# ramanakumars/patchGAN

Hardware: AMD Instinct MI355X
Metric: train images/sec (G+D step) at 256x256 bs=16 per GPU (higher is better)
Workload: dtype f32 (fp32 tensors and accumulation; polyphase Winograd GEMMs in bf16x3 split form: six bf16 MFMA products per fp32 product); 1 GPU; cfg2: 256x256x3->1 masks, bs 16/GPU, UNet nf=64 leakyrelu/sigmoid + PatchGAN ndf=64 n_layers=3, focal-Tversky*200 + BCE, Adam 1e-3, dropout off; global_batch=16, parallelism=dp1

## Files before the change

### include/patchgan_hip.h

```cpp
#ifndef PATCHGAN_HIP_H
#define PATCHGAN_HIP_H

#include <stddef.h>
#include <stdint.h>

#ifdef __cplusplus
extern "C" {
#endif

#define PG_OK 0
#define PG_EINVAL (-1)
#define PG_EWORKSPACE (-2)
#define PG_ELAUNCH (-3)

#define PG_ACT_NONE 0
#define PG_ACT_LEAKY 1
#define PG_ACT_RELU 2
#define PG_ACT_TANH 3
#define PG_ACT_SIGMOID 4

#define PG_ALGO_AUTO 0
#define PG_ALGO_DIRECT 1
#define PG_ALGO_MFMA 2
#define PG_ALGO_BF16 3

#define PG_ALGO_MASK 0xF
#define PG_TUNE_WINO2_ALL 0x010
#define PG_TUNE_WINO2_OFF 0x020
#define PG_TUNE_WINO2W_ALL 0x040
#define PG_TUNE_WINO2W_OFF 0x080
#define PG_TUNE_WINO_OFF 0x100
#define PG_TUNE_WINOW_OFF 0x200
#define PG_TUNE_WINO1_F2 0x400
#define PG_TUNE_WINO1_F3 0x800
#define PG_TUNE_WINO_DMA 0x1000
#define PG_TUNE_BF16X_OFF 0x2000
#define PG_TUNE_BF16X_RING 0x4000
#define PG_TUNE_BF16X_FLAT 0x8000
#define PG_TUNE_S3_OFF 0x40000

#define PG_IO_BIG_BF16 0x10000
#define PG_IO_SMALL_BF16 0x20000
#define PG_IO_MASK 0x30000

typedef struct pg_conv_geom {
    int N;
    int Hb, Wb;
    int Hs, Ws;
    int Ca;
    int Cb;
    int stride;
} pg_conv_geom;

int pg_version(void);

size_t pg_conv_max_tensor_bytes(void);

size_t pg_conv_workspace_bytes(const pg_conv_geom* g, int op);

int pg_conv_describe(const pg_conv_geom* g, int op, size_t ws_bytes, int* tile_id, int* split, long* workgroups);

int pg_conv_kernel(const pg_conv_geom* g, int op, size_t ws_bytes, char* name, size_t name_len, int* split, double* mfma_flops);

int pg_conv_kernel_flops(const pg_conv_geom* g, int op, size_t ws_bytes, double* executed, double* useful);

int pg_conv_time_next(void* ev_start, void* ev_stop);

int pg_conv4x4_big2small(const float* big, int ld_big, const float* P, const float* bias,
                         float* small, int ld_small, const pg_conv_geom* g, int act, int algo,
                         void* ws, size_t ws_bytes, void* stream);

int pg_conv4x4_small2big(const float* small, int ld_small, const float* P, const float* bias,
                         float* big, int ld_big, const pg_conv_geom* g, int act, int algo,
                         void* ws, size_t ws_bytes, void* stream);

int pg_conv4x4_wgrad(const float* small, int ld_small, const float* big, int ld_big,
                     float* dP, float* dbias, const pg_conv_geom* g, int algo,
                     void* ws, size_t ws_bytes, void* stream);

typedef struct pg_conv_extras {
    double* part;
    float* v_keep;
    const float* v_pre;
    float* u_cache;
    int u_valid;
    const void* mul_t;
    int mul_ld;
    int mul_act;
    long long v_stride;
    long long v_tile0;
} pg_conv_extras;
int pg_conv_batch_halves_same(const pg_conv_geom* g, int algo, size_t ws_bytes_n, size_t ws_bytes_2n);
int pg_conv_mul_ok(const pg_conv_geom* g, int algo, size_t ws_bytes);
int pg_conv_stats_chunks(const pg_conv_geom* g, int op, int algo, size_t ws_bytes);
size_t pg_conv_u_bytes(const pg_conv_geom* g, int op, int algo, size_t ws_bytes);
size_t pg_conv_v_bytes(const pg_conv_geom* g, int algo, size_t ws_bytes);
int pg_conv4x4_big2small_x(const float* big, int ld_big, const float* P, const float* bias, float* small, int ld_small,
                           const pg_conv_geom* g, int act, int algo, void* ws, size_t ws_bytes, void* stream,
                           const pg_conv_extras* x);
int pg_conv4x4_small2big_x(const float* small, int ld_small, const float* P, const float* bias, float* big, int ld_big,
                           const pg_conv_geom* g, int act, int algo, void* ws, size_t ws_bytes, void* stream,
                           const pg_conv_extras* x);
int pg_conv4x4_wgrad_x(const float* small, int ld_small, const float* big, int ld_big, float* dP, float* dbias,
                       const pg_conv_geom* g, int algo, void* ws, size_t ws_bytes, void* stream, const pg_conv_extras* x);
typedef struct pg_conv_prep_item {
    pg_conv_geom g;
    int op;
    int algo;
    size_t ws_bytes;
    const float* P;
    void* u;
} pg_conv_prep_item;
int pg_conv_prep_batch(int n, const pg_conv_prep_item* items, void* stream);
int pg_instnorm_act_fwd_parts(const float* y, int ld_y, float* out, int ld_out, float* stats, const double* part, int chunks,
                              int N, int HW, int C, int act, float eps, float drop_p, uint64_t seed, void* stream);

int pg_instnorm_act_fwd_t(const void* y, int ld_y, void* out, int ld_out, float* stats, int N, int HW, int C, int act, float eps,
                          float drop_p, uint64_t seed, void* ws, size_t ws_bytes, void* stream, int dt);
int pg_instnorm_act_fwd_parts_t(const void* y, int ld_y, void* out, int ld_out, float* stats, const double* part, int chunks,
                                int N, int HW, int C, int act, float eps, float drop_p, uint64_t seed, void* stream, int dt);
int pg_instnorm_act_bwd_t(const void* g1, int ld_g1, const void* g2, int ld_g2, const void* y, int ld_y, const float* stats,
                          void* dy, int ld_dy, int N, int HW, int C, int act, float drop_p, uint64_t seed, void* ws,
                          size_t ws_bytes, void* stream, int dt);
size_t pg_instnorm_affine_workspace_bytes(int N, int HW, int C);
int pg_instnorm_affine_act_fwd_t(const void* y, int ld_y, void* out, int ld_out, const float* gamma, const float* beta, float* stats,
                                 int N, int HW, int C, int act, float eps, float drop_p, uint64_t seed, void* ws, size_t ws_bytes,
                                 void* stream, int dt);
int pg_instnorm_affine_act_fwd_parts_t(const void* y, int ld_y, void* out, int ld_out, const float* gamma, const float* beta,
                                       float* stats, const double* part, int chunks, int N, int HW, int C, int act, float eps,
                                       float drop_p, uint64_t seed, void* stream, int dt);
int pg_instnorm_affine_act_bwd_t(const void* g1, int ld_g1, const void* g2, int ld_g2, const void* y, int ld_y, const float* gamma,
                                 const float* beta, const float* stats, void* dy, int ld_dy, float* dgamma, float* dbeta, int N,
                                 int HW, int C, int act, float drop_p, uint64_t seed, void* ws, size_t ws_bytes, void* stream,
                                 int dt);
int pg_act_fwd_t(const void* y, int ld_y, void* out, int ld_out, long npix, int C, int act, float drop_p, uint64_t seed,
                 void* stream, int dt);
int pg_act_bwd_t(const void* g1, int ld_g1, const void* g2, int ld_g2, const void* a, int ld_a, void* dy, int ld_dy, long npix,
                 int C, int act, float drop_p, uint64_t seed, void* stream, int dt);

int pg_conv4x4_bwd_big(const float* small, int ld_small, const float* big, int ld_big, const float* P, float* dP,
                       float* dsmall, int ld_dsmall, const pg_conv_geom* g, int algo, void* ws, size_t ws_bytes, void* stream);
int pg_conv4x4_bwd_big_x(const float* small, int ld_small, const float* big, int ld_big, const float* P, float* dP,
                         float* dsmall, int ld_dsmall, const pg_conv_geom* g, int algo, void* ws, size_t ws_bytes, void* stream,
                         const pg_conv_extras* x);

int pg_conv_time_next2(void* ev_start, void* ev_stop, void* ev_start2, void* ev_stop2);

int pg_instnorm_act_fwd(const float* y, int ld_y, float* out, int ld_out, float* stats,
                        int N, int HW, int C, int act, float eps,
                        float drop_p, uint64_t seed, void* ws, size_t ws_bytes, void* stream);

size_t pg_instnorm_workspace_bytes(int N, int HW, int C);

int pg_instnorm_act_bwd(const float* g1, int ld_g1, const float* g2, int ld_g2,
                        const float* y, int ld_y, const float* stats, float* dy, int ld_dy,
                        int N, int HW, int C, int act, float drop_p, uint64_t seed,
                        void* ws, size_t ws_bytes, void* stream);

int pg_act_bwd(const float* g1, int ld_g1, const float* g2, int ld_g2, const float* a, int ld_a,
               float* dy, int ld_dy, long npix, int C, int act, float drop_p, uint64_t seed, void* stream);

int pg_act_fwd(const float* y, int ld_y, float* out, int ld_out, long npix, int C, int act,
               float drop_p, uint64_t seed, void* stream);

int pg_softmax_fwd(const float* y, int ld_y, float* out, int ld_out, long npix, int C, void* stream);
int pg_softmax_bwd(const float* g1, int ld_g1, const float* g2, int ld_g2, const float* out, int ld_out,
                   float* dy, int ld_dy, long npix, int C, void* stream);

int pg_dropout_mask(float* mask, long nelem, float drop_p, uint64_t seed, void* stream);

size_t pg_batchnorm_workspace_bytes(int N, int HW, int C, int nseg);
int pg_batchnorm_act_fwd(const float* y, int ld_y, float* out, int ld_out, const float* weight, const float* bias, float* coef,
                         double* bstat, int N, int HW, int C, int nseg, int act, float eps, float drop_p, uint64_t seed, void* ws,
                         size_t ws_bytes, void* stream);
int pg_batchnorm_stats(const float* y, int ld_y, const double* part, int chunks, const float* weight, const float* bias, float* coef,
                       double* bstat, int N, int HW, int C, int nseg, float eps, void* ws, size_t ws_bytes, void* stream);
int pg_batchnorm_act_apply(const float* y, int ld_y, float* out, int ld_out, const float* coef, int N, int HW, int C, int nseg,
                           int act, float drop_p, uint64_t seed, void* stream);
int pg_batchnorm_eval_coef(const float* running_mean, const float* running_var, const float* weight, const float* bias, int C,
                           float eps, float* coef, void* stream);
int pg_batchnorm_act_bwd(const float* g1, int ld_g1, const float* g2, int ld_g2, const float* y, int ld_y, const float* coef,
                         float* dy, int ld_dy, float* dweight, float* dbias, int N, int HW, int C, int nseg, int train, int act,
                         float drop_p, uint64_t seed, void* ws, size_t ws_bytes, void* stream);
int pg_batchnorm_moments_fwd(const float* y, int ld_y, const double* part, int chunks, double* mom, int N, int HW, int C, int nseg,
                             void* ws, size_t ws_bytes, void* stream);
int pg_batchnorm_coef_from_moments(const double* mom, double count, const float* weight, const float* bias, float eps, float* coef,
                                   double* bstat, int C, int nseg, void* stream);
// ... 165 lines not shown
```

### patchgan_amd/_lib.py

```python
import ctypes
import os

_HERE = os.path.dirname(os.path.abspath(__file__))
LIB_PATH = os.environ.get('PATCHGAN_LIB') or os.path.join(_HERE, 'libpatchgan_hip.so')

ACT_NONE, ACT_LEAKY, ACT_RELU, ACT_TANH, ACT_SIGMOID = 0, 1, 2, 3, 4
ACT_CODES = {None: ACT_NONE, 'none': ACT_NONE, 'leakyrelu': ACT_LEAKY, 'relu': ACT_RELU, 'tanh': ACT_TANH,
             'sigmoid': ACT_SIGMOID}
ALGO_AUTO, ALGO_DIRECT, ALGO_MFMA, ALGO_BF16 = 0, 1, 2, 3
ALGO_MASK = 0xF
IO_BIG_BF16, IO_SMALL_BF16, IO_MASK = 0x10000, 0x20000, 0x30000
TUNE_WINO2_ALL, TUNE_WINO2_OFF, TUNE_WINO2W_ALL, TUNE_WINO2W_OFF = 0x010, 0x020, 0x040, 0x080
TUNE_WINO_OFF, TUNE_WINOW_OFF, TUNE_WINO1_F2, TUNE_WINO1_F3, TUNE_WINO_DMA = 0x100, 0x200, 0x400, 0x800, 0x1000
TUNE_BF16X_OFF, TUNE_BF16X_RING, TUNE_BF16X_FLAT = 0x2000, 0x4000, 0x8000
TUNE_S3_OFF = 0x40000
LOSS_TVERSKY, LOSS_WBCE, LOSS_MAE, LOSS_BCE = 0, 1, 2, 3
OP_BIG2SMALL, OP_SMALL2BIG, OP_WGRAD = 0, 1, 2
AUG_FLIP, AUG_TRANSLATION, AUG_CUTOUT = 1, 2, 4
ACC_BEGIN, ACC_ADD, ACC_CLOSE, ACC_CLOSE_ONLY = 0, 1, 2, 3
GAN_LSGAN, GAN_HINGE_D, GAN_HINGE_G, GAN_BCE_LOGITS = 0, 1, 2, 3
SEG_CE, SEG_FOCAL, SEG_DICE = 1, 2, 4
SEG_FOCAL_GAMMA_MAX, SEG_FOCAL_ALPHA_NONE = 8, -1.0

_ERR = {-1: 'PG_EINVAL (bad shape / null or misaligned pointer)', -2: 'PG_EWORKSPACE (workspace too small)',
        -3: 'PG_ELAUNCH (HIP launch failed)'}


class ConvGeom(ctypes.Structure):
    _fields_ = [('N', ctypes.c_int), ('Hb', ctypes.c_int), ('Wb', ctypes.c_int), ('Hs', ctypes.c_int),
                ('Ws', ctypes.c_int), ('Ca', ctypes.c_int), ('Cb', ctypes.c_int), ('stride', ctypes.c_int)]

    def key(self):
        return (self.N, self.Hb, self.Wb, self.Hs, self.Ws, self.Ca, self.Cb, self.stride)


_p = ctypes.c_void_p
_i = ctypes.c_int
_l = ctypes.c_long
_f = ctypes.c_float
_d = ctypes.c_double
_sz = ctypes.c_size_t
_u64 = ctypes.c_uint64
_G = ctypes.POINTER(ConvGeom)


class ConvExtras(ctypes.Structure):
    _fields_ = [('part', ctypes.c_void_p), ('v_keep', ctypes.c_void_p), ('v_pre', ctypes.c_void_p), ('u_cache', ctypes.c_void_p),
                ('u_valid', ctypes.c_int), ('mul_t', ctypes.c_void_p), ('mul_ld', ctypes.c_int), ('mul_act', ctypes.c_int),
                ('v_stride', ctypes.c_longlong), ('v_tile0', ctypes.c_longlong)]


_X = ctypes.POINTER(ConvExtras)


class BnUpdateItem(ctypes.Structure):
    _fields_ = [('bstat', ctypes.c_void_p), ('running_mean', ctypes.c_void_p), ('running_var', ctypes.c_void_p),
                ('num_batches_tracked', ctypes.c_void_p), ('C', ctypes.c_int)]


BN_MAX_LAYERS = 16


class ConvPrepItem(ctypes.Structure):
    _fields_ = [('g', ConvGeom), ('op', ctypes.c_int), ('algo', ctypes.c_int), ('ws_bytes', ctypes.c_size_t), ('P', ctypes.c_void_p),
                ('u', ctypes.c_void_p)]


class SpectralItem(ctypes.Structure):
    _fields_ = [('W', ctypes.c_void_p), ('w_hat', ctypes.c_void_p), ('u', ctypes.c_void_p), ('v', ctypes.c_void_p),
                ('sigma', ctypes.c_void_p), ('g_off', ctypes.c_long), ('Cout', ctypes.c_int), ('Cin', ctypes.c_int),
                ('iterate', ctypes.c_int)]


SN_MAX_LAYERS = 16


class GanTerm(ctypes.Structure):
    _fields_ = [('d', ctypes.c_void_p), ('g', ctypes.c_void_p), ('value', ctypes.c_void_p), ('scale', ctypes.c_double),
                ('n', ctypes.c_long), ('ld', ctypes.c_int), ('ld_g', ctypes.c_int), ('kind', ctypes.c_int), ('target', ctypes.c_float)]


GAN_MAX_TERMS = 4


SIGNATURES = {
    'pg_version': (_i, []),
    'pg_conv_max_tensor_bytes': (_sz, []),
    'pg_conv_workspace_bytes': (_sz, [_G, _i]),
    'pg_conv_describe': (_i, [_G, _i, _sz, ctypes.POINTER(_i), ctypes.POINTER(_i), ctypes.POINTER(_l)]),
    'pg_conv_mul_ok': (_i, [_G, _i, _sz]),
    'pg_conv_kernel': (_i, [_G, _i, _sz, ctypes.c_char_p, _sz, ctypes.POINTER(_i), ctypes.POINTER(ctypes.c_double)]),
    'pg_conv_kernel_flops': (_i, [_G, _i, _sz, ctypes.POINTER(ctypes.c_double), ctypes.POINTER(ctypes.c_double)]),
    'pg_conv_time_next': (_i, [_p, _p]),
    'pg_conv_time_next2': (_i, [_p, _p, _p, _p]),
    'pg_conv4x4_bwd_big': (_i, [_p, _i, _p, _i, _p, _p, _p, _i, _G, _i, _p, _sz, _p]),
    'pg_conv4x4_bwd_big_x': (_i, [_p, _i, _p, _i, _p, _p, _p, _i, _G, _i, _p, _sz, _p, _X]),
    'pg_conv4x4_big2small': (_i, [_p, _i, _p, _p, _p, _i, _G, _i, _i, _p, _sz, _p]),
    'pg_conv4x4_small2big': (_i, [_p, _i, _p, _p, _p, _i, _G, _i, _i, _p, _sz, _p]),
    'pg_conv4x4_wgrad': (_i, [_p, _i, _p, _i, _p, _p, _G, _i, _p, _sz, _p]),
    'pg_conv_stats_chunks': (_i, [_G, _i, _i, _sz]),
    'pg_conv_u_bytes': (_sz, [_G, _i, _i, _sz]),
    'pg_conv_v_bytes': (_sz, [_G, _i, _sz]),
    'pg_conv_batch_halves_same': (_i, [_G, _i, _sz, _sz]),
    'pg_conv4x4_big2small_x': (_i, [_p, _i, _p, _p, _p, _i, _G, _i, _i, _p, _sz, _p, _X]),
    'pg_conv4x4_small2big_x': (_i, [_p, _i, _p, _p, _p, _i, _G, _i, _i, _p, _sz, _p, _X]),
    'pg_conv4x4_wgrad_x': (_i, [_p, _i, _p, _i, _p, _p, _G, _i, _p, _sz, _p, _X]),
    'pg_conv_prep_batch': (_i, [_i, ctypes.POINTER(ConvPrepItem), _p]),
    'pg_instnorm_act_fwd_parts': (_i, [_p, _i, _p, _i, _p, _p, _i, _i, _i, _i, _i, _f, _f, _u64, _p]),
    'pg_instnorm_workspace_bytes': (_sz, [_i, _i, _i]),
    'pg_instnorm_act_fwd': (_i, [_p, _i, _p, _i, _p, _i, _i, _i, _i, _f, _f, _u64, _p, _sz, _p]),
    'pg_instnorm_act_bwd': (_i, [_p, _i, _p, _i, _p, _i, _p, _p, _i, _i, _i, _i, _i, _f, _u64, _p, _sz, _p]),
    'pg_act_bwd': (_i, [_p, _i, _p, _i, _p, _i, _p, _i, _l, _i, _i, _f, _u64, _p]),
    'pg_act_fwd': (_i, [_p, _i, _p, _i, _l, _i, _i, _f, _u64, _p]),
    'pg_instnorm_act_fwd_t': (_i, [_p, _i, _p, _i, _p, _i, _i, _i, _i, _f, _f, _u64, _p, _sz, _p, _i]),
    'pg_instnorm_act_fwd_parts_t': (_i, [_p, _i, _p, _i, _p, _p, _i, _i, _i, _i, _i, _f, _f, _u64, _p, _i]),
    'pg_instnorm_act_bwd_t': (_i, [_p, _i, _p, _i, _p, _i, _p, _p, _i, _i, _i, _i, _i, _f, _u64, _p, _sz, _p, _i]),
    'pg_instnorm_affine_workspace_bytes': (_sz, [_i, _i, _i]),
    'pg_instnorm_affine_act_fwd_t': (_i, [_p, _i, _p, _i, _p, _p, _p, _i, _i, _i, _i, _f, _f, _u64, _p, _sz, _p, _i]),
    'pg_instnorm_affine_act_fwd_parts_t': (_i, [_p, _i, _p, _i, _p, _p, _p, _p, _i, _i, _i, _i, _i, _f, _f, _u64, _p, _i]),
    'pg_instnorm_affine_act_bwd_t': (_i, [_p, _i, _p, _i, _p, _i, _p, _p, _p, _p, _i, _p, _p, _i, _i, _i, _i, _f, _u64, _p, _sz, _p,
                                          _i]),
    'pg_act_fwd_t': (_i, [_p, _i, _p, _i, _l, _i, _i, _f, _u64, _p, _i]),
    'pg_act_bwd_t': (_i, [_p, _i, _p, _i, _p, _i, _p, _i, _l, _i, _i, _f, _u64, _p, _i]),
    'pg_softmax_fwd': (_i, [_p, _i, _p, _i, _l, _i, _p]),
    'pg_softmax_bwd': (_i, [_p, _i, _p, _i, _p, _i, _p, _i, _l, _i, _p]),
    'pg_dropout_mask': (_i, [_p, _l, _f, _u64, _p]),
    'pg_batchnorm_workspace_bytes': (_sz, [_i, _i, _i, _i]),
    'pg_batchnorm_act_fwd': (_i, [_p, _i, _p, _i, _p, _p, _p, _p, _i, _i, _i, _i, _i, _f, _f, _u64, _p, _sz, _p]),
    'pg_batchnorm_stats': (_i, [_p, _i, _p, _i, _p, _p, _p, _p, _i, _i, _i, _i, _f, _p, _sz, _p]),
    'pg_batchnorm_act_apply': (_i, [_p, _i, _p, _i, _p, _i, _i, _i, _i, _i, _f, _u64, _p]),
    'pg_batchnorm_eval_coef': (_i, [_p, _p, _p, _p, _i, _f, _p, _p]),
    'pg_batchnorm_act_bwd': (_i, [_p, _i, _p, _i, _p, _i, _p, _p, _i, _p, _p, _i, _i, _i, _i, _i, _i, _f, _u64, _p, _sz, _p]),
    'pg_batchnorm_moments_fwd': (_i, [_p, _i, _p, _i, _p, _i, _i, _i, _i, _p, _sz, _p]),
    'pg_batchnorm_coef_from_moments': (_i, [_p, _d, _p, _p, _f, _p, _p, _i, _i, _p]),
    'pg_batchnorm_moments_bwd': (_i, [_p, _i, _p, _i, _p, _i, _p, _p, _p, _p, _i, _i, _i, _i, _i, _f, _u64, _p, _sz, _p]),
    'pg_batchnorm_bwd_apply': (_i, [_p, _i, _p, _i, _p, _i, _p, _p, _d, _p, _i, _i, _i, _i, _i, _i, _f, _u64, _p, _sz, _p]),
    'pg_batchnorm_update_running': (_i, [_i, ctypes.POINTER(BnUpdateItem), _i, _f, _p]),
    'pg_loss_reduce_doubles': (_l, [_i, _i, _i]),
    'pg_loss_fused_max_nc': (_i, []),
    'pg_loss_reduce': (_i, [_p, _i, _p, _i, _f, _i, _i, _i, _p, _p]),
    'pg_loss_prepare': (_i, [_p, _i, _i, _f, _p, _p]),
    'pg_loss_finalize': (_i, [_p, _p, _i, _i, _i, _i, _i, _f, _f, _f, _p, _p, _p]),
    'pg_loss_grad': (_i, [_p, _i, _p, _i, _f, _p, _p, _i, _i, _i, _i, _i, _p]),
    'pg_loss_reduce_parts': (_i, [_p, _i, _p, _i, _f, _i, _i, _i, _p, _p]),
    'pg_loss_value_grad': (_i, [_p, _i, _p, _p, _i, _i, _i, _i, _i, _f, _f, _f, _p, _i, _p, _i, _f, _p, _i, _p, _p]),
    'pg_seg_confusion_max_c': (_i, []),
    'pg_seg_confusion': (_i, [_p, _i, _p, _i, _i, _i, _i, _f, _p, _p]),
    'pg_seg_hist_max_words': (_i, []),
    'pg_seg_hist': (_i, [_p, _i, _p, _i, _i, _i, _i, _i, _p, _p]),
    'pg_adam_step': (_i, [_p, _p, _p, _p, _l, _f, _f, _f, _f, _f, _f, _p]),
    'pg_adam_step_dev': (_i, [_p, _p, _p, _p, _l, _f, _f, _f, _p, _p]),
    'pg_adam_ema_step': (_i, [_p, _p, _p, _p, _p, _l, _f, _f, _f, _f, _f, _f, _f, _p]),
    'pg_adam_ema_step_dev': (_i, [_p, _p, _p, _p, _p, _l, _f, _f, _f, _p, _f, _p]),
    'pg_grad_norm_workspace_bytes': (_l, [_l]),
    'pg_grad_norm': (_i, [_p, _l, _d, _p, _l, _p, _p]),
    'pg_adam_clip_step': (_i, [_p, _p, _p, _p, _p, _l, _f, _f, _f, _f, _f, _f, _f, _p, _p]),
    'pg_adam_clip_step_dev': (_i, [_p, _p, _p, _p, _p, _l, _f, _f, _f, _p, _f, _p, _p]),
    'pg_adamw_step': (_i, [_p, _p, _p, _p, _p, _l, _f, _f, _f, _f, _f, _f, _f, _f, _p, _p]),
    'pg_adamw_step_dev': (_i, [_p, _p, _p, _p, _p, _l, _f, _f, _f, _p, _f, _p, _p]),
    'pg_grad_accum': (_i, [_p, _p, _l, _i, _f, _p]),
    'pg_spectral_workspace_bytes': (_l, [_i, ctypes.POINTER(SpectralItem)]),
    'pg_spectral_fwd': (_i, [_i, ctypes.POINTER(SpectralItem), _p, _p, _l, _p, _l, _p]),
    'pg_spectral_bwd': (_i, [_i, ctypes.POINTER(SpectralItem), _p, _l, _p, _l, _p]),
    'pg_nchw_to_nhwc': (_i, [_p, _p, _i, _i, _i, _i, _i, _p]),
    'pg_nhwc_to_nchw': (_i, [_p, _i, _p, _i, _i, _i, _i, _p]),
    'pg_copy_channels': (_i, [_p, _i, _p, _i, _l, _i, _p]),
    'pg_fill': (_i, [_p, _l, _f, _p]),
    'pg_pad8_bf16': (_i, [_p, _i, _p, _l, _i, _p]),
    'pg_din_fill': (_i, [_p, _p, _p, _p, _i, _i, _i, _i, _i, _i, _p]),
    'pg_u8_to_f32': (_i, [_p, _p, _i, _l, _i, _f, _p]),
    'pg_labels_to_onehot': (_i, [_p, _p, _i, _l, _p, _i, _i, _p]),
    'pg_tiles_count': (_i, [_i, _i, _i]),
    'pg_tiles_gather': (_i, [_p, _i, _i, _i, _i, _i, _p, _i, _p]),
    'pg_tiles_blend': (_i, [_p, _i, _i, _i, _i, _i, _i, ctypes.c_double, _p, _p, _p]),
    'pg_tiles_tta_max': (_i, []),
    'pg_tiles_gather_tta': (_i, [_p, _i, _i, _i, _i, _i, _i, _p, _i, _p]),
    'pg_tiles_blend_win': (_i, [_p, _i, _i, _i, _i, _i, _i, _i, _p, ctypes.c_double, _p, _p, _p]),
    'pg_diffaug_params': (_i, [_u64, _p, _u64, _i, _l, _i, _i, _i, _p, _p]),
    'pg_diffaug_fwd': (_i, [_p, _i, _p, _i, _p, _i, _i, _i, _i, _p]),
    'pg_diffaug_bwd': (_i, [_p, _i, _p, _i, _p, _i, _i, _i, _i, _p]),
    'pg_gan_loss_max_terms': (_i, []),
    'pg_gan_loss_single_max': (_l, []),
    'pg_gan_loss_workspace_bytes': (_l, [_i, ctypes.POINTER(GanTerm)]),
    'pg_gan_loss': (_i, [_i, ctypes.POINTER(GanTerm), _p, _l, _p]),
    'pg_seg_loss_workspace_bytes': (_l, [_i, _i, _i]),
    'pg_seg_loss_slabs': (_i, [_i, _i]),
    'pg_seg_loss_reduce': (_i, [_p, _i, _p, _i, _i, _i, _i, _i, _i, _f, _p, _l, _p]),
    'pg_seg_loss_value_grad': (_i, [_p, _l, _p, _i, _p, _i, _i, _i, _i, _i, _i, _f, _f, _d, _d, _d, _p, _i, _p, _p]),
    'pg_seg_loss_value_grad_w': (_i, [_p, _l, _p, _i, _p, _i, _i, _i, _i, _i, _i, _f, _f, _d, _d, _d, _p, _p, _i, _p, _p]),
    'pg_seg_label_count': (_i, [_p, _i, _i, _i, _i, _p, _p]),
# ... 39 lines not shown
```

### patchgan_amd/csrc/conv_gemm.hip

```cpp
#include <hip/hip_runtime.h>
#include <stdio.h>
#include <stdint.h>
#include <stdlib.h>
#include <string.h>
#include <type_traits>
#include <vector>
#include "patchgan_hip.h"
#include "pg_common.h"
#include "conv_wino.h"
#include "conv_bf16.h"

namespace {

typedef float f32x4 __attribute__((ext_vector_type(4)));
typedef float f32x16 __attribute__((ext_vector_type(16)));

struct Geom {
    int N, Hb, Wb, Hs, Ws, Ca, Cb, s;
};

constexpr int KC = 32;
constexpr int LDK = KC + 4;

__device__ __forceinline__ f32x4 ld4(const float* p, bool ok) {
// ... 4234 lines not shown
                    hipLaunchKernelGGL((k_wgrad_tapn<PG_TILE(T), 2>), grid, dim3(256), 0, st, big, ld_big, small, ld_small, dst, q.out_elems, g, q.cps, q.tiles_n,
                                       p.vecn, 0);
            });
        }
    }
    if (hipGetLastError() != hipSuccess) return PG_ELAUNCH;
    return q.split == 1 ? PG_OK : reduce(dst, q.split);
}

int refusal(int rc, int op, const Views& v, const pg_conv_geom* gg, int algo_full, size_t ws_bytes) {
    if (rc != PG_EINVAL || !(algo_full & PG_IO_MASK)) return rc;
    const size_t full = pg_conv_workspace_bytes(gg, op);
    if (v.ws && ws_bytes >= full) return rc;
    Views w = v;
    if (!w.ws) w.ws = reinterpret_cast<void*>(uintptr_t(256));
    return plan_conv(gg, op, algo_full, tune_of(algo_full), full, &w).rc == PG_OK ? PG_EWORKSPACE : rc;
}

int run_conv(int op, const Views& v, const pg_conv_geom* gg, int algo_full, size_t ws_bytes, void* stream) {
    if (!v.ws) ws_bytes = 0;
    Call c{ConvPlan{}, v, to_geom(gg), algo_full & PG_ALGO_MASK, algo_full & PG_IO_MASK, tune_of(algo_full), ws_bytes, (hipStream_t)stream};
    c.p = plan_conv(gg, op, algo_full, c.tune, ws_bytes, &c.v);
    if (c.p.rc != PG_OK) return refusal(c.p.rc, op, v, gg, algo_full, ws_bytes);
    return op == 0 ? launch_b2s(c) : op == 1 ? launch_s2b(c) : launch_wgrad(c);
}

}

static bool hand_overs_sized(const pg_conv_geom* gg, int op, int algo, const void* ws, size_t ws_bytes, const pg_conv_extras& x) {
    const size_t wb = ws ? ws_bytes : 0;
    if (x.part && (op > 1 || pg_conv_stats_chunks(gg, op, algo, wb) == 0)) return false;
    if (x.u_cache && (op > 1 || pg_conv_u_bytes(gg, op, algo, wb) == 0)) return false;
    if ((x.v_keep || x.v_pre) && pg_conv_v_bytes(gg, algo, wb) == 0) return false;
    return true;
}

extern "C" {

int pg_conv4x4_big2small_x(const float* big, int ld_big, const float* P, const float* bias, float* small, int ld_small,
                           const pg_conv_geom* gg, int act, int algo, void* ws, size_t ws_bytes, void* stream, const pg_conv_extras* xp) {
    const pg_conv_extras& x = xp ? *xp : NO_EXTRAS;
    if ((x.u_cache && !aligned16(x.u_cache)) || (x.v_keep && !aligned16(x.v_keep)) || x.v_pre) return PG_EINVAL;
    if (!geom_ok(gg) || !big || !P || !small || ld_big < gg->Cb || ld_small < gg->Ca) return PG_EINVAL;
    if (act < PG_ACT_NONE || act > PG_ACT_SIGMOID) return PG_EINVAL;
    if ((algo & PG_IO_MASK) && (algo & PG_ALGO_MASK) != PG_ALGO_BF16) return PG_EINVAL;
    if (!hand_overs_sized(gg, 0, algo, ws, ws_bytes, x)) return PG_EINVAL;
    if (x.v_stride || x.v_tile0) {
        ConvPlan f;
        if (!x.v_keep || x.v_stride < 0 || x.v_tile0 < 0 || !query_plan(gg, 0, algo, ws ? ws_bytes : 0, OFFER_V, &f)) return PG_EINVAL;
        if (f.path != Path::Wino1 && f.path != Path::Wino2) return PG_EINVAL;
        const bool w1 = f.path == Path::Wino1;
        const long X = w1 ? 36 : 16, K = w1 ? gg->Cb : 4L * gg->Cb;
        const long T = w1 ? (long)gg->N * ((gg->Hs + 2) / 3) * ((gg->Ws + 2) / 3) : pg_wino2_tiles_b2s(gg->N, gg->Hs, gg->Ws);
        const long zs = x.v_stride ? (long)x.v_stride : T * K;
        if ((zs & 3) || (x.v_tile0 + T) * K > zs || (double)X * zs * 4 >= 1.5e9) return PG_EINVAL;
    }
    return run_conv(0, Views{small, big, ld_small, ld_big, P, bias, act, ws, &x}, gg, algo, ws_bytes, stream);
}

int pg_conv4x4_big2small(const float* big, int ld_big, const float* P, const float* bias, float* small,
                         int ld_small, const pg_conv_geom* gg, int act, int algo, void* ws, size_t ws_bytes,
                         void* stream) {
    return pg_conv4x4_big2small_x(big, ld_big, P, bias, small, ld_small, gg, act, algo, ws, ws_bytes, stream, nullptr);
}

int pg_conv4x4_small2big_x(const float* small, int ld_small, const float* P, const float* bias, float* big, int ld_big,
                           const pg_conv_geom* gg, int act, int algo, void* ws, size_t ws_bytes, void* stream, const pg_conv_extras* xp) {
    const pg_conv_extras& x = xp ? *xp : NO_EXTRAS;
    if ((x.u_cache && !aligned16(x.u_cache)) || x.v_keep || x.v_pre || x.v_stride || x.v_tile0) return PG_EINVAL;
    if (x.mul_t && (x.mul_ld < gg->Cb || x.mul_act < PG_ACT_NONE || x.mul_act > PG_ACT_SIGMOID || x.part)) return PG_EINVAL;
    if (!geom_ok(gg) || !big || !P || !small || ld_big < gg->Cb || ld_small < gg->Ca) return PG_EINVAL;
    if (act < PG_ACT_NONE || act > PG_ACT_SIGMOID) return PG_EINVAL;
    if ((algo & PG_IO_MASK) && (algo & PG_ALGO_MASK) != PG_ALGO_BF16) return PG_EINVAL;
    if (!hand_overs_sized(gg, 1, algo, ws, ws_bytes, x)) return PG_EINVAL;
    return run_conv(1, Views{small, big, ld_small, ld_big, P, bias, act, ws, &x}, gg, algo, ws_bytes, stream);
}

int pg_conv4x4_small2big(const float* small, int ld_small, const float* P, const float* bias, float* big,
                         int ld_big, const pg_conv_geom* gg, int act, int algo, void* ws, size_t ws_bytes,
                         void* stream) {
    return pg_conv4x4_small2big_x(small, ld_small, P, bias, big, ld_big, gg, act, algo, ws, ws_bytes, stream, nullptr);
}

static int wgrad_impl(const float* small, int ld_small, const float* big, int ld_big, float* dP, float* dbias,
                      const pg_conv_geom* gg, int algo, void* ws, size_t ws_bytes, void* stream, const float* v_pre) {
    if (!geom_ok(gg) || !big || !dP || !small || ld_big < gg->Cb || ld_small < gg->Ca) return PG_EINVAL;
    if (v_pre && !aligned16(v_pre)) return PG_EINVAL;
    hipStream_t st = (hipStream_t)stream;
    const Geom g = to_geom(gg);
    const int io = algo & PG_IO_MASK;
    if (io && ((algo & PG_ALGO_MASK) != PG_ALGO_BF16 || io != PG_IO_MASK)) return PG_EINVAL;
    if (io && dbias && !((g.Ca % 4 == 0) && (ld_small % 4 == 0) && aligned_io(small, true))) return PG_EINVAL;
    if (!ws) ws_bytes = 0;
    pg_conv_extras x = NO_EXTRAS;
    x.v_pre = v_pre;
    if (!hand_overs_sized(gg, 2, algo, ws, ws_bytes, x)) return PG_EINVAL;
    if (dbias) {
        if (ws_bytes < colsum_bytes(g.Ca)) return PG_EWORKSPACE;
        const Views vw{small, big, ld_small, ld_big, dP, dbias, PG_ACT_NONE, ws, &x};
        const int prc = plan_conv(gg, 2, algo, tune_of(algo), ws_bytes, &vw).rc;
        if (prc != PG_OK) return refusal(prc, 2, vw, gg, algo, ws_bytes);
        const long Kp = (long)g.N * g.Hs * g.Ws;
        float* part = (float*)ws;
        int chunks = (int)std::min<long>(COLSUM_CHUNKS, Kp);
        long rpc = (Kp + chunks - 1) / chunks;
        chunks = (int)((Kp + rpc - 1) / rpc);
        if (io)
            hipLaunchKernelGGL(k_colsum_partial4<true>, dim3(chunks, (g.Ca + 63) / 64), dim3(256), 0, st, small, ld_small, Kp, g.Ca,
                               rpc, part);
        else if ((g.Ca % 4 == 0) && (ld_small % 4 == 0) && aligned16(small) && aligned16(part))
            hipLaunchKernelGGL(k_colsum_partial4<false>, dim3(chunks, (g.Ca + 63) / 64), dim3(256), 0, st, small, ld_small, Kp, g.Ca,
                               rpc, part);
        else
            hipLaunchKernelGGL(k_colsum_partial, dim3(chunks, (g.Ca + 63) / 64), dim3(256), 0, st, small, ld_small, Kp, g.Ca,
                               rpc, part);
        if (hipGetLastError() != hipSuccess) return PG_ELAUNCH;
        int rc = launch_reduce(part, g.Ca, chunks, dbias, g.Ca, 1, g.Ca, nullptr, 0, st);
        if (rc != PG_OK) return rc;
    }
    return run_conv(2, Views{small, big, ld_small, ld_big, dP, dbias, PG_ACT_NONE, ws, &x}, gg, algo, ws_bytes, stream);
}

int pg_conv4x4_wgrad(const float* small, int ld_small, const float* big, int ld_big, float* dP, float* dbias,
                     const pg_conv_geom* gg, int algo, void* ws, size_t ws_bytes, void* stream) {
    return wgrad_impl(small, ld_small, big, ld_big, dP, dbias, gg, algo, ws, ws_bytes, stream, nullptr);
}

int pg_conv4x4_wgrad_x(const float* small, int ld_small, const float* big, int ld_big, float* dP, float* dbias,
                       const pg_conv_geom* gg, int algo, void* ws, size_t ws_bytes, void* stream, const pg_conv_extras* x) {
    if (x && (x->part || x->v_keep || x->u_cache || x->v_stride || x->v_tile0)) return PG_EINVAL;
    return wgrad_impl(small, ld_small, big, ld_big, dP, dbias, gg, algo, ws, ws_bytes, stream, x ? x->v_pre : nullptr);
}

int pg_conv4x4_bwd_big(const float* small, int ld_small, const float* big, int ld_big, const float* P, float* dP,
                       float* dsmall, int ld_dsmall, const pg_conv_geom* gg, int algo, void* ws, size_t ws_bytes, void* stream) {
    return pg_conv4x4_bwd_big_x(small, ld_small, big, ld_big, P, dP, dsmall, ld_dsmall, gg, algo, ws, ws_bytes, stream, nullptr);
}

int pg_conv4x4_bwd_big_x(const float* small, int ld_small, const float* big, int ld_big, const float* P, float* dP,
                         float* dsmall, int ld_dsmall, const pg_conv_geom* gg, int algo, void* ws, size_t ws_bytes, void* stream,
                         const pg_conv_extras* x) {
    if (!geom_ok(gg) || !small || !big || !P || !dP || !dsmall) return PG_EINVAL;
    if (x && (x->part || x->v_keep || x->v_pre || x->mul_t || x->v_stride || x->v_tile0)) return PG_EINVAL;
    float* const Uext = x ? x->u_cache : nullptr;
    const int u_valid = x ? x->u_valid : 0;
    if (Uext && !aligned16(Uext)) return PG_EINVAL;
    if (ld_small < gg->Ca || ld_big < gg->Cb || ld_dsmall < gg->Ca) return PG_EINVAL;
    if (Uext && pg_conv_u_bytes(gg, 0, algo, ws ? ws_bytes : 0) == 0) return PG_EINVAL;
    hipStream_t st = (hipStream_t)stream;
    const Geom g = to_geom(gg);
    const Tune tune = tune_of(algo);
    if (!ws) ws_bytes = 0;
    const bool views_ok = (ld_small % 4 == 0) && (ld_big % 4 == 0) && (ld_dsmall % 4 == 0) && aligned16(small) && aligned16(big) &&
                          aligned16(P) && aligned16(dP) && aligned16(dsmall) && aligned16(ws);
    hipEvent_t e0 = t_ev0, e1 = t_ev1, e2 = t_ev2, e3 = t_ev3;
    if (!plan_share_v(g, algo, tune, ws_bytes, views_ok, nullptr)) {
        t_ev2 = t_ev3 = nullptr;
        int rc = pg_conv4x4_wgrad(small, ld_small, big, ld_big, dP, nullptr, gg, algo, ws, ws_bytes, stream);
        if (rc != PG_OK) return rc;
        t_ev0 = e2;
        t_ev1 = e3;
        if (Uext) {
            pg_conv_extras xu{};
            xu.u_cache = Uext;
            xu.u_valid = u_valid;
            return pg_conv4x4_big2small_x(big, ld_big, P, nullptr, dsmall, ld_dsmall, gg, PG_ACT_NONE, algo, ws, ws_bytes, stream, &xu);
        }
        return pg_conv4x4_big2small(big, ld_big, P, nullptr, dsmall, ld_dsmall, gg, PG_ACT_NONE, algo, ws, ws_bytes, stream);
    }
    t_ev0 = t_ev1 = t_ev2 = t_ev3 = nullptr;
    float* V = (float*)ws;
    void* rest = (char*)ws + pg_wino2_v_bytes(g.N, g.Hs, g.Ws, g.Cb);
    int rc = pg_wino2_v(big, ld_big, V, g.N, g.Hb, g.Wb, g.Hs, g.Ws, g.Cb, st);
    if (rc != PG_OK) return rc;
    rc = pg_wino2_wgrad(small, ld_small, big, ld_big, dP, g.N, g.Hb, g.Wb, g.Hs, g.Ws, g.Ca, g.Cb, rest, st, e0, e1, V, tune.s3w);
    if (rc != PG_OK) return rc;
    return pg_wino2_b2s(big, ld_big, P, nullptr, dsmall, ld_dsmall, g.N, g.Hb, g.Wb, g.Hs, g.Ws, g.Ca, g.Cb, PG_ACT_NONE, rest, st, e2,
                        e3, V, nullptr, nullptr, Uext, u_valid, tune.s3);
}

}
```

### patchgan_amd/csrc/conv_wino.h

```cpp
#pragma once
#include <hip/hip_runtime.h>
#include <stddef.h>
#include "pg_common.h"


bool pg_wino_eligible(int N, int Hin, int Win, int Cin, int Hout, int Wout, int Cout, int ld_in, const void* in, int mo_forced);
bool pg_wino_geom_ok(int N, int Hout, int Wout, int Cin, int Cout, int mo_forced);
int pg_wino_mo(int N, int Hout, int Wout, int Cin, int Cout, int mo_forced);
bool pg_wino_small_tile(int N, int Hout, int Wout, int Cin, int Cout, int mo_forced);
size_t pg_wino_ws_bytes(int N, int Hout, int Wout, int Cin, int Cout, int mo_forced);
int pg_wino_prepare(const float* in, int ld_in, const float* P, int flip, int N, int Hin, int Win, int Cin, int Hout,
                    int Wout, int Cout, int pad, void* ws, hipStream_t st, int mo_forced, float* Uext, int u_valid, float* Vext = nullptr,
                    long v_stride = 0, long v_tile0 = 0);
size_t pg_wino_u_bytes(int N, int Hout, int Wout, int Cin, int Cout, int mo_forced);
size_t pg_wino2_u_bytes(int Ca, int Cb);
#define PG_WINO_PREP_MAX 24
struct pg_wino_prep {
    const float* P;
    float* U;
    int Ca, Cb, kind, mo, flip;
};
int pg_wino_prep_batch(int n, const pg_wino_prep* items, hipStream_t st);
int pg_wino_gemm_slices(int N, int Hout, int Wout, int Cin, int Cout, int mo_forced);
bool pg_wino_gemm_rows(int N, int Hout, int Wout, int Cin, int Cout, int mo_forced, int dma_mode, const float* out, int ld_out,
                       const float* bias, pg_epi_mul mul);
bool pg_wino_row_on();
float* pg_wino_gemm_slabs(void* ws, int N, int Hout, int Wout, int Cin, int Cout, int mo_forced);
int pg_wino_dma_mode();
int pg_wino_gemm(const float* bias, float* out, int ld_out, int N, int Cin, int Hout, int Wout, int Cout, int act,
                 void* ws, hipStream_t st, int mo_forced, int dma_mode, const float* Uext, pg_epi_mul mul = pg_epi_mul{nullptr, 0, 0},
                 const float* Vext = nullptr, int s3 = 0, long v_stride = 0, long v_tile0 = 0);

bool pg_wino_wgrad_geom_ok(int N, int Hs, int Ws, int Ca, int Cb);
int pg_wino_wgrad_r(int N, int Hs, int Ws);
double pg_wino_wgrad_flops(int N, int Hs, int Ws, int Ca, int Cb);
int pg_wino_wgrad_slices(int N, int Hs, int Ws, int Ca, int Cb, int s3);
bool pg_wino_wgrad_tile64(int Ca, int Cb, int s3);
size_t pg_wino_wgrad_ws_bytes(int N, int Hs, int Ws, int Ca, int Cb);
int pg_wino_wgrad(const float* small, int ld_small, const float* big, int ld_big, float* dP, int N, int Hb, int Wb, int Hs,
                  int Ws, int Ca, int Cb, void* ws, hipStream_t st, hipEvent_t ev0, hipEvent_t ev1, const float* Vpre = nullptr, int s3 = 0);
size_t pg_wino_wgrad_v_bytes(int N, int Hs, int Ws, int Ca, int Cb, int fwd_mo_forced);

int pg_wino2_mo();
long pg_wino2_tiles_b2s(int N, int Hs, int Ws);
long pg_wino2_tiles_s2b(int N, int Hb, int Wb);
int pg_wino2_b2s_zb(int N, int Hs, int Ws, int Ca);
int pg_wino2_s2b_zb(int N, int Hb, int Wb, int Cb);
bool pg_wino2_geom_ok(int N, int Hs, int Ws, int Ca, int Cb);
size_t pg_wino2_ws_bytes(int N, int Hs, int Ws, int Ca, int Cb);
int pg_wino2_b2s(const float* big, int ld_big, const float* P, const float* bias, float* small, int ld_small, int N, int Hb,
                 int Wb, int Hs, int Ws, int Ca, int Cb, int act, void* ws, hipStream_t st, hipEvent_t ev0, hipEvent_t ev1,
                 const float* Vpre, double* part, float* Vkeep, float* Uext, int u_valid, int s3, long v_stride = 0, long v_tile0 = 0);
int pg_wino2_b2s_stats_chunks(int N, int Hs, int Ws, int Ca);
int pg_wino2_s2b_stats_chunks(int N, int Hb, int Wb, int Cb);
size_t pg_wino2_v_bytes(int N, int Hs, int Ws, int Cb);
int pg_wino2_v(const float* big, int ld_big, float* V, int N, int Hb, int Wb, int Hs, int Ws, int Cb, hipStream_t st);

bool pg_wino2c_geom_ok(int N, int Hb, int Wb, int Ca, int Cb);
size_t pg_wino2c_ws_bytes(int N, int Hb, int Wb, int Ca, int Cb);
int pg_wino2_s2b(const float* small, int ld_small, const float* P, const float* bias, float* big, int ld_big, int N, int Hb,
                 int Wb, int Hs, int Ws, int Ca, int Cb, int act, void* ws, hipStream_t st, hipEvent_t ev0, hipEvent_t ev1,
                 double* part, float* Uext, int u_valid, pg_epi_mul mul, int s3);

bool pg_wino2_wgrad_geom_ok(int N, int Hs, int Ws, int Ca, int Cb);
int pg_wino2_wgrad_slices(int N, int Hs, int Ws, int Ca, int Cb, int s3);
bool pg_wino2_wgrad_tile64(int Ca, int Cb, int s3);
size_t pg_wino2_wgrad_ws_bytes(int N, int Hs, int Ws, int Ca, int Cb);
int pg_wino2_wgrad(const float* small, int ld_small, const float* big, int ld_big, float* dP, int N, int Hb, int Wb, int Hs,
                   int Ws, int Ca, int Cb, void* ws, hipStream_t st, hipEvent_t ev0, hipEvent_t ev1, const float* Vpre, int s3 = 0);
```

### patchgan_amd/csrc/conv_wino.hip

```cpp
#include <hip/hip_runtime.h>
#include <stdint.h>
#include <stdlib.h>
#include "patchgan_hip.h"
#include "pg_common.h"
#include "conv_wino.h"

namespace {

typedef float f32x4 __attribute__((ext_vector_type(4)));
typedef float f32x16 __attribute__((ext_vector_type(16)));
typedef unsigned int u32x4 __attribute__((ext_vector_type(4)));

constexpr int KC = 32;
constexpr int LDK = KC + 4;


__device__ __constant__ float c_BT[5][5] = {{2, -1, -2, 1, 0}, {0, -2, -1, 1, 0}, {0, 2, -3, 1, 0}, {0, -1, 0, 1, 0},
                                            {0, 2, -1, -2, 1}};
__device__ __constant__ float c_G[5][4] = {{0.5f, 0, 0, 0},
                                           {-0.5f, -0.5f, -0.5f, -0.5f},
                                           {-1.f / 6, 1.f / 6, -1.f / 6, 1.f / 6},
                                           {1.f / 6, 1.f / 3, 2.f / 3, 4.f / 3},
                                           {0, 0, 0, 1}};

// ... 1104 lines not shown
            for (int j = 0; j < NR; ++j)
#pragma unroll
                for (int p = 0; p < 3; ++p)
                    fb[j][p] = *reinterpret_cast<const s3_bf16x8*>(&buf[(BM + (wn * NR + j) * 32 + lrow) * S3_LDR + p * S3_KC + lh * 8]);
#pragma unroll
            for (int i = 0; i < MR; ++i)
#pragma unroll
                for (int p = 0; p < 3; ++p)
                    fa[i][p] = *reinterpret_cast<const s3_bf16x8*>(&buf[((wm * MR + i) * 32 + lrow) * S3_LDR + p * S3_KC + lh * 8]);
        };
        auto mm = [&](const s3_bf16x8 (&fa)[MR][3], const s3_bf16x8 (&fb)[NR][3]) {
#define S3_MM(pa, pb)                                                                       \
    _Pragma("unroll") for (int i = 0; i < MR; ++i) _Pragma("unroll") for (int j = 0; j < NR; ++j) \
        acc[i][j] = __builtin_amdgcn_mfma_f32_32x32x16_bf16(fa[i][pa], fb[j][pb], acc[i][j], 0, 0, 0)
            S3_MM(0, 0); S3_MM(0, 1); S3_MM(1, 0); S3_MM(1, 1); S3_MM(0, 2); S3_MM(2, 0);
#undef S3_MM
        };
        auto mix = [&]() {
            constexpr int NM = 6 * MR * NR, NRD = 3 * (MR + NR), NWR = 3 * (AI + BI), NLD = AI + BI;
#pragma unroll
            for (int t = 0; t < NM; ++t) {
                __builtin_amdgcn_sched_group_barrier(0x008, 1, 0);
                if (t < NLD) __builtin_amdgcn_sched_group_barrier(0x020, 1, 0);
                if (t < NRD) __builtin_amdgcn_sched_group_barrier(0x100, 1, 0);
                __builtin_amdgcn_sched_group_barrier(0x002, 4, 0);
                if (t >= NM - NWR) __builtin_amdgcn_sched_group_barrier(0x200, 1, 0);
            }
        };
        issue_loads(ra0, rb0, 0);
        issue_loads(ra1, rb1, 1);
        stage(ra0, rb0, buf0);
        issue_loads(ra0, rb0, 2);
        __syncthreads();
        rd(fa0, fb0, buf0);
        stage(ra1, rb1, buf1);
        issue_loads(ra1, rb1, 3);
        __syncthreads();
        for (int c = 0; c < nch; c += 2) {
            mm(fa0, fb0);
            rd(fa1, fb1, buf1);
            stage(ra0, rb0, buf0);
            issue_loads(ra0, rb0, c + 4);
            mix();
            __syncthreads();
            mm(fa1, fb1);
            rd(fa0, fb0, buf0);
            stage(ra1, rb1, buf1);
            issue_loads(ra1, rb1, c + 5);
            mix();
            __syncthreads();
        }
    } else {
    issue_loads(ra0, rb0, 0);
    issue_loads(ra1, rb1, 1);
    stage(ra0, rb0, buf0);
    issue_loads(ra0, rb0, 2);
    __syncthreads();
    for (int c = 0; c < nch; c += 2) {
        stage(ra1, rb1, buf1);
        compute(buf0);
        issue_loads(ra1, rb1, c + 3);
        __syncthreads();
        stage(ra0, rb0, buf0);
        compute(buf1);
        issue_loads(ra0, rb0, c + 4);
        __syncthreads();
    }
    }
    float* o = C + (long)z * Mrows * Ncols;
#pragma unroll
    for (int i = 0; i < MR; ++i)
#pragma unroll
        for (int j = 0; j < NR; ++j) {
            const int col = n0 + (wn * NR + j) * 32 + lrow;
#pragma unroll
            for (int r = 0; r < 16; ++r) {
                const int row = (r & 3) + 8 * (r >> 2) + 4 * lh;
                const int m = m0 + (wm * MR + i) * 32 + row;
                if (m < Mrows && col < Ncols) o[(long)m * Ncols + col] = acc[i][j][r];
            }
        }
}

template <int MR, int NR, int WM, int WN, int KS, int WPE>
__global__ __launch_bounds__(256) __attribute__((amdgpu_waves_per_eu(WPE, WPE))) void k_wino_wgrad_gemm_s3(const float* __restrict__ DY, const float* __restrict__ V,
                                                         float* __restrict__ S, int T, int Ca, int Cb, int chunks_per_slice,
                                                         int tilesA, int tilesB, int NX, int dy_bytes, int v_bytes) {
    constexpr int BM = WM * MR * 32, BN = WN * NR * 32, KCH = 16 * KS, ROW = KS * 48 + 8, BUF = (BM + BN) * ROW;
    static_assert((BM + BN) * KS == 256, "one 4 x 4 block per staging thread");
    __shared__ __attribute__((aligned(16))) __bf16 smem[2 * BUF];
    const int tid = threadIdx.x, lane = tid & 63, wave = tid >> 6;
    const int wm = wave / WN, wn = wave % WN;
    const int lrow = lane & 31, lh = lane >> 5;
    int w = pg_xcd_remap(blockIdx.x, gridDim.x);
    const int tile_b = w % tilesB;
    w /= tilesB;
    const int tile_a = w % tilesA;
    w /= tilesA;
    const int xi = w % NX, slice = w / NX;
    const int m0 = tile_a * BM, n0 = tile_b * BN;
    const int k_begin = slice * chunks_per_slice * KC, k_end = min(T, k_begin + chunks_per_slice * KC);
    const int nch = (max(k_end - k_begin, 0) + KCH - 1) / KCH;
    const bool is_a = __builtin_amdgcn_readfirstlane(tid >> 6) < BM * KS / 64;
    const int it = is_a ? tid : tid - BM * KS, BX = is_a ? BM : BN;
    const int kg = it & 3, mq = (it >> 2) % (BX / 4), ks = it / BX;
    const int ld = is_a ? Ca : Cb, c0 = (is_a ? m0 : n0) + mq * 4;
    const bool c_in = c0 < ld;
    const __amdgpu_buffer_rsrc_t rS = is_a ? __builtin_amdgcn_make_buffer_rsrc((void*)DY, 0, dy_bytes, 0x00020000)
                                           : __builtin_amdgcn_make_buffer_rsrc((void*)V, 0, v_bytes, 0x00020000);
    const int base = xi * T * ld + c0;
    const int krow = ks * 16 + kg * 4;
    const int wr_off = ((is_a ? 0 : BM) + mq * 4) * ROW + ks * 48 + kg * 4;
    auto issue_loads = [&](f32x4 (&r)[4], int c) {
#pragma unroll
        for (int j = 0; j < 4; ++j) {
            const int k = k_begin + c * KCH + krow + j;
            r[j] = bload4(rS, voff(base + k * ld, c < nch && c_in && k < k_end));
        }
    };
    auto stage = [&](const f32x4 (&r)[4], __bf16* buf) {
#pragma unroll
        for (int e = 0; e < 4; ++e) {
            const f32x4 v = {r[0][e], r[1][e], r[2][e], r[3][e]};
            s3_bf16x4 h, m, l;
            s3_split(v, h, m, l);
            __bf16* row = &buf[wr_off + e * ROW];
            *reinterpret_cast<s3_bf16x4*>(row) = h;
            *reinterpret_cast<s3_bf16x4*>(row + 16) = m;
            *reinterpret_cast<s3_bf16x4*>(row + 32) = l;
        }
    };
    f32x16 acc[MR][NR];
#pragma unroll
    for (int i = 0; i < MR; ++i)
#pragma unroll
        for (int j = 0; j < NR; ++j)
#pragma unroll
            for (int r = 0; r < 16; ++r) acc[i][j][r] = 0.f;
    auto compute = [&](const __bf16* buf) {
#pragma unroll
        for (int s = 0; s < KS; ++s) {
            s3_bf16x8 bf[NR][3], af[MR][3];
#pragma unroll
            for (int j = 0; j < NR; ++j)
#pragma unroll
                for (int p = 0; p < 3; ++p)
                    bf[j][p] = *reinterpret_cast<const s3_bf16x8*>(&buf[(BM + (wn * NR + j) * 32 + lrow) * ROW + s * 48 + p * 16 + lh * 8]);
#pragma unroll
            for (int i = 0; i < MR; ++i)
#pragma unroll
                for (int p = 0; p < 3; ++p)
                    af[i][p] = *reinterpret_cast<const s3_bf16x8*>(&buf[((wm * MR + i) * 32 + lrow) * ROW + s * 48 + p * 16 + lh * 8]);
#pragma unroll
            for (int i = 0; i < MR; ++i)
#pragma unroll
                for (int j = 0; j < NR; ++j) {
#define S3_MM(pa, pb) acc[i][j] = __builtin_amdgcn_mfma_f32_32x32x16_bf16(af[i][pa], bf[j][pb], acc[i][j], 0, 0, 0)
                    S3_MM(0, 0); S3_MM(0, 1); S3_MM(1, 0); S3_MM(1, 1); S3_MM(0, 2); S3_MM(2, 0);
#undef S3_MM
                }
        }
    };
    __bf16* const buf0 = smem;
    __bf16* const buf1 = smem + BUF;
    f32x4 r0[4], r1[4];
    issue_loads(r0, 0);
    issue_loads(r1, 1);
    stage(r0, buf0);
    issue_loads(r0, 2);
    __syncthreads();
    for (int c = 0; c < nch; c += 2) {
        stage(r1, buf1);
        compute(buf0);
        issue_loads(r1, c + 3);
        __syncthreads();
        stage(r0, buf0);
        compute(buf1);
        issue_loads(r0, c + 4);
        __syncthreads();
    }
    float* o = S + ((long)slice * NX + xi) * Ca * Cb;
#pragma unroll
    for (int i = 0; i < MR; ++i)
#pragma unroll
        for (int j = 0; j < NR; ++j) {
            const int col = n0 + (wn * NR + j) * 32 + lrow;
#pragma unroll
            for (int r = 0; r < 16; ++r) {
                const int row = (r & 3) + 8 * (r >> 2) + 4 * lh;
                const int a = m0 + (wm * MR + i) * 32 + row;
                if (a < Ca && col < Cb) o[(long)a * Cb + col] = acc[i][j][r];
            }
        }
}

template <int WPE>
__global__ __launch_bounds__(256) __attribute__((amdgpu_waves_per_eu(WPE, WPE))) void k_wino_gemm_row_s3(
    const float* __restrict__ V, const float* __restrict__ U, float* __restrict__ Tout, int T, int Ci, int Co, int v_bytes, int u_bytes,
    int tiles_n, int v_xi) {
    constexpr int NP = 6, BM = 128, BN = 64, MR = 2, BUF = (BM + BN) * S3_LDR;
    __shared__ __attribute__((aligned(16))) __bf16 smem[2 * BUF];
    const __amdgpu_buffer_rsrc_t rV = __builtin_amdgcn_make_buffer_rsrc((void*)V, 0, v_bytes, 0x00020000);
    const __amdgpu_buffer_rsrc_t rU = __builtin_amdgcn_make_buffer_rsrc((void*)U, 0, u_bytes, 0x00020000);
    const int tid = threadIdx.x, lane = tid & 63, wave = tid >> 6;
    const int wm = wave >> 1, wn = wave & 1;
    const int lrow = lane & 31, lh = lane >> 5;
    int w = pg_xcd_remap(blockIdx.x, gridDim.x);
    const int n0 = (w % tiles_n) * BN;
    w /= tiles_n;
    const int tiles_m = (T + BM - 1) / BM;
    const int xrow = w / tiles_m;
    const int m0 = (w % tiles_m) * BM;
    const int nch = Ci / S3_KC, total = NP * nch;
    const int kq = tid & 3, r0 = tid >> 2;
    int a_off[2], b_off;
    bool a_ok[2];
#pragma unroll
    for (int i = 0; i < 2; ++i) {
        const int m = m0 + r0 + 64 * i;
        a_ok[i] = m < T;
        a_off[i] = min(m, T - 1) * Ci + kq * 4;
    }
    {
        const int co = n0 + r0;
        b_off = (co < Co) ? co * Ci + kq * 4 : 0x10000000;
    }
    const int u_xi = Co * Ci;
    int ld_j = 0, ld_ch = 0;
    auto issue_loads = [&](f32x4 (&ra)[2], f32x4& rb) {
        const bool on = ld_j < NP;
        const int xi = xrow * NP + ld_j;
        const int av = xi * v_xi + ld_ch * S3_KC, bu = xi * u_xi + ld_ch * S3_KC;
#pragma unroll
        for (int i = 0; i < 2; ++i) ra[i] = bload4(rV, voff(a_off[i] + av, on && a_ok[i]));
        rb = bload4(rU, voff(b_off + bu, on));
        const bool wrap = ld_ch + 1 >= nch;
        ld_ch = wrap ? 0 : ld_ch + 1;
        ld_j = wrap ? ld_j + 1 : ld_j;
    };
    auto stage = [&](const f32x4 (&ra)[2], const f32x4& rb, __bf16* buf) {
#pragma unroll
        for (int i = 0; i < 2; ++i) {
            s3_bf16x4 h, m, l;
            s3_split(ra[i], h, m, l);
            __bf16* row = &buf[(r0 + 64 * i) * S3_LDR + kq * 4];
            *reinterpret_cast<s3_bf16x4*>(row) = h;
            *reinterpret_cast<s3_bf16x4*>(row + S3_KC) = m;
            *reinterpret_cast<s3_bf16x4*>(row + 2 * S3_KC) = l;
        }
        s3_bf16x4 h, m, l;
        s3_split(rb, h, m, l);
        __bf16* row = &buf[(BM + r0) * S3_LDR + kq * 4];
        *reinterpret_cast<s3_bf16x4*>(row) = h;
        *reinterpret_cast<s3_bf16x4*>(row + S3_KC) = m;
        *reinterpret_cast<s3_bf16x4*>(row + 2 * S3_KC) = l;
    };
    f32x16 accm[MR], acct[3][MR];
#pragma unroll
    for (int i = 0; i < MR; ++i)
#pragma unroll
        for (int r = 0; r < 16; ++r) {
            accm[i][r] = 0.f;
#pragma unroll
            for (int c = 0; c < 3; ++c) acct[c][i][r] = 0.f;
        }
    int j = 0, ch = 0;
    auto compute = [&](const __bf16* buf) {
        s3_bf16x8 bf[3], af[MR][3];
#pragma unroll
        for (int p = 0; p < 3; ++p) bf[p] = *reinterpret_cast<const s3_bf16x8*>(&buf[(BM + wn * 32 + lrow) * S3_LDR + p * S3_KC + lh * 8]);
#pragma unroll
        for (int i = 0; i < MR; ++i)
#pragma unroll
            for (int p = 0; p < 3; ++p)
                af[i][p] = *reinterpret_cast<const s3_bf16x8*>(&buf[((wm * MR + i) * 32 + lrow) * S3_LDR + p * S3_KC + lh * 8]);
#pragma unroll
// ... 664 lines not shown
                           TW, Hout, Wout, act, v_bytes, u_bytes, tn, mul, 1, 0L);
    } else if (small_tile && dma_mode == 2) {
        dim3 grid((unsigned)(((T + 63) / 64) * tn));
        hipLaunchKernelGGL((k_wino_gemm_dma<2, 3, 3>), grid, dim3(256), 0, st, V, U, bias, out, ld_out, (int)T, Cin, Cout, TH, TW,
                           Hout, Wout, act, v_bytes, u_bytes, tn);
    } else if (small_tile) {
        dim3 grid((unsigned)(((T + 63) / 64) * tn));
        hipLaunchKernelGGL((k_wino_gemm<1, 1, 2, 2, 4, 2>), grid, dim3(256), 0, st, V, U, bias, out, ld_out, (int)T, Cin, Cout, TH,
                           TW, Hout, Wout, act, v_bytes, u_bytes, tn, mul, 1, 0L);
    } else {
        dim3 grid((unsigned)(((T + 127) / 128) * tn));
        hipLaunchKernelGGL((k_wino_gemm<2, 1, 2, 2, 2, 2>), grid, dim3(256), 0, st, V, U, bias, out, ld_out, (int)T, Cin, Cout, TH,
                           TW, Hout, Wout, act, v_bytes, u_bytes, tn, mul, 1, 0L);
    }
    return hipGetLastError() == hipSuccess ? PG_OK : PG_ELAUNCH;
}

static long wgrad_s3_fill(int s3, int tile) {
    static const int forced = [] {
        const char* e = pg_exp_env("PATCHGAN_S3W_FILL");
        return e ? atoi(e) : 0;
    }();
    if (s3 && tile == 128) return forced ? forced : 128;
    return 768;
}
int pg_wino_wgrad_r(int N, int Hs, int Ws) {
    static const int forced = [] {
        const char* e = pg_exp_env("PATCHGAN_WINOW_R");
        return e ? atoi(e) : 0;
    }();
    if (forced == 2 || forced == 3) return forced;
    return (long)N * ((Hs + 2) / 3) * ((Ws + 2) / 3) >= 1024 ? 3 : 2;
}
static long wgrad_tiles(int N, int Hs, int Ws) {
    const int r = pg_wino_wgrad_r(N, Hs, Ws);
    return (long)N * ((Hs + r - 1) / r) * ((Ws + r - 1) / r);
}
static int wgrad_nxi(int N, int Hs, int Ws) {
    const int np = pg_wino_wgrad_r(N, Hs, Ws) + 3;
    return np * np;
}
double pg_wino_wgrad_flops(int N, int Hs, int Ws, int Ca, int Cb) {
    return 2.0 * wgrad_nxi(N, Hs, Ws) * wgrad_tiles(N, Hs, Ws) * Ca * Cb;
}
bool pg_wino_wgrad_geom_ok(int N, int Hs, int Ws, int Ca, int Cb) {
    if (Ca % 4 != 0 || Cb % 4 != 0 || Ca < 64 || Cb < 64) return false;
    if ((long)N * ((Hs + 1) / 2) * ((Ws + 1) / 2) < 2048) return false;
    const double xt = (double)wgrad_nxi(N, Hs, Ws) * wgrad_tiles(N, Hs, Ws);
    if (xt * Ca * 4 >= 1.5e9 || xt * Cb * 4 >= 1.5e9) return false;
    return true;
}

bool pg_wino_wgrad_tile64(int Ca, int Cb, int s3) {
    static const int forced = [] {
        const char* e = pg_exp_env("PATCHGAN_WINOW_TILE");
        return e ? atoi(e) : 0;
    }();
    if (forced) return forced == 64;
    if (s3 && Ca % 128 == 0 && Cb % 128 == 0) return false;
    return 25L * ((Ca + 127) / 128) * ((Cb + 127) / 128) < 768;
}
int pg_wino_wgrad_slices(int N, int Hs, int Ws, int Ca, int Cb, int s3) {
    const long T = wgrad_tiles(N, Hs, Ws);
    const int tt = pg_wino_wgrad_tile64(Ca, Cb, s3) ? 64 : 128;
    const long wgs = (long)wgrad_nxi(N, Hs, Ws) * ((Ca + tt - 1) / tt) * ((Cb + tt - 1) / tt);
    const long fill = wgrad_s3_fill(s3, tt);
    long s = (fill + wgs - 1) / wgs;
    const long nchunks = (T + KC - 1) / KC;
    if (s > nchunks / 16) s = nchunks / 16;
    return (int)(s < 1 ? 1 : s);
}

size_t pg_wino_wgrad_ws_bytes(int N, int Hs, int Ws, int Ca, int Cb) {
    const long T = wgrad_tiles(N, Hs, Ws), X = wgrad_nxi(N, Hs, Ws);
    const int sl = std::max(pg_wino_wgrad_slices(N, Hs, Ws, Ca, Cb, 0), pg_wino_wgrad_slices(N, Hs, Ws, Ca, Cb, 1));
    return align256((size_t)X * T * Cb * 4) + align256((size_t)X * T * Ca * 4) + align256((size_t)sl * X * Ca * Cb * 4);
}

size_t pg_wino_wgrad_v_bytes(int N, int Hs, int Ws, int Ca, int Cb, int fwd_forced) {
    if (pg_wino_wgrad_r(N, Hs, Ws) != 3 || pg_wino_mo(N, Hs, Ws, Cb, Ca, fwd_forced) != 3) return 0;
    return align256((size_t)36 * wgrad_tiles(N, Hs, Ws) * Cb * 4);
}

int pg_wino_wgrad(const float* small, int ld_small, const float* big, int ld_big, float* dP, int N, int Hb, int Wb, int Hs,
                  int Ws, int Ca, int Cb, void* ws, hipStream_t st, hipEvent_t ev0, hipEvent_t ev1, const float* Vpre, int s3) {
    const int R = pg_wino_wgrad_r(N, Hs, Ws), X = (R + 3) * (R + 3);
    const int TH = (Hs + R - 1) / R, TW = (Ws + R - 1) / R;
    const long T = (long)N * TH * TW;
    if (Vpre && R != 3) return PG_EINVAL;
    const float* V = Vpre ? Vpre : (const float*)ws;
    float* DY = (float*)((char*)ws + align256((size_t)X * T * Cb * 4));
    float* S = (float*)((char*)DY + align256((size_t)X * T * Ca * 4));
    const dim3 gv((unsigned)((T * (Cb / 4) + 255) / 256)), gd((unsigned)((T * (Ca / 4) + 255) / 256));
    if (R == 3) {
        if (!Vpre) hipLaunchKernelGGL(k_wino_v<3>, gv, dim3(256), 0, st, big, ld_big, (float*)ws, N, Hb, Wb, Cb, TH, TW, 1, T * Cb, 0L);
        if (hipGetLastError() != hipSuccess) return PG_ELAUNCH;
        hipLaunchKernelGGL(k_wino_dy<3>, gd, dim3(256), 0, st, small, ld_small, DY, N, Hs, Ws, Ca, TH, TW);
    } else {
        hipLaunchKernelGGL(k_wino_v<2>, gv, dim3(256), 0, st, big, ld_big, (float*)ws, N, Hb, Wb, Cb, TH, TW, 1, T * Cb, 0L);
        if (hipGetLastError() != hipSuccess) return PG_ELAUNCH;
        hipLaunchKernelGGL(k_wino_dy<2>, gd, dim3(256), 0, st, small, ld_small, DY, N, Hs, Ws, Ca, TH, TW);
    }
    if (hipGetLastError() != hipSuccess) return PG_ELAUNCH;
    const int slices = pg_wino_wgrad_slices(N, Hs, Ws, Ca, Cb, s3);
    const int nchunks = (int)((T + KC - 1) / KC);
    const int cps = (nchunks + slices - 1) / slices;
    if (ev0) (void)hipEventRecord(ev0, st);
    if (pg_wino_wgrad_tile64(Ca, Cb, s3)) {
        const int tilesA = (Ca + 63) / 64, tilesB = (Cb + 63) / 64;
        if (s3)
            hipLaunchKernelGGL((k_wino_wgrad_gemm_s3<1, 1, 2, 2, 2, 3>), dim3(tilesA * tilesB * X * slices), dim3(256), 0, st, DY, V, S, (int)T,
                               Ca, Cb, cps, tilesA, tilesB, X, (int)((long)X * T * Ca * 4), (int)((long)X * T * Cb * 4));
        else
            hipLaunchKernelGGL((k_wino_wgrad_gemm<1, 1, 2, 2>), dim3(tilesA * tilesB * X * slices), dim3(256), 0, st, DY, V, S, (int)T, Ca,
                               Cb, cps, tilesA, tilesB, X, (int)((long)X * T * Ca * 4), (int)((long)X * T * Cb * 4));
    } else {
        const int tilesA = (Ca + 127) / 128, tilesB = (Cb + 127) / 128;
        if (s3)
            hipLaunchKernelGGL((k_wino_wgrad_gemm_s3<2, 2, 2, 2, 1, 2>), dim3(tilesA * tilesB * X * slices), dim3(256), 0, st, DY, V, S, (int)T,
                               Ca, Cb, cps, tilesA, tilesB, X, (int)((long)X * T * Ca * 4), (int)((long)X * T * Cb * 4));
        else
            hipLaunchKernelGGL((k_wino_wgrad_gemm<2, 2, 2, 2>), dim3(tilesA * tilesB * X * slices), dim3(256), 0, st, DY, V, S, (int)T, Ca,
                               Cb, cps, tilesA, tilesB, X, (int)((long)X * T * Ca * 4), (int)((long)X * T * Cb * 4));
    }
    if (ev1) (void)hipEventRecord(ev1, st);
    if (hipGetLastError() != hipSuccess) return PG_ELAUNCH;
    const dim3 go((unsigned)(((long)Ca * Cb + 255) / 256));
    if (R == 3)
        hipLaunchKernelGGL(k_wino_wgrad_out<3>, go, dim3(256), 0, st, S, slices, dP, Ca, Cb);
    else
        hipLaunchKernelGGL(k_wino_wgrad_out<2>, go, dim3(256), 0, st, S, slices, dP, Ca, Cb);
    return hipGetLastError() == hipSuccess ? PG_OK : PG_ELAUNCH;
}

static void bgemm_s3_launch(int big_rows, dim3 grid, hipStream_t st, const float* A, const float* B, float* C, int Mrows, int Ncols, int K,
                            int a_bytes, int b_bytes, int tm, int tn, int a_zs) {
    static const int var = [] {
        const char* e = pg_exp_env("PATCHGAN_S3_VAR");
        return e ? atoi(e) : 1;
    }();
    static const int pipe = [] {
        const char* e = pg_exp_env("PATCHGAN_S3_PIPE");
        return e ? atoi(e) : 0;
    }();
    static const int big = [] {
        const char* e = pg_exp_env("PATCHGAN_S3_BIG");
        return e ? atoi(e) : 0;
    }();
    if (var == 1 && big && big_rows && Mrows >= big) {
        const int X = (int)grid.x / (tm * tn), tm2 = (Mrows + 255) / 256;
        hipLaunchKernelGGL((k_wino_bgemm_s3<2, 2, 4, 2, 2, 1, false>), dim3(tm2 * tn * X), dim3(512), 0, st, A, B, C, Mrows, Ncols, K, a_bytes, b_bytes,
                           tm2, tn, a_zs);
        return;
    }
    if (var == 1 && pipe) {
        if (big_rows)
            hipLaunchKernelGGL((k_wino_bgemm_s3<2, 2, 2, 2, 2, 1, true>), grid, dim3(256), 0, st, A, B, C, Mrows, Ncols, K, a_bytes, b_bytes, tm, tn, a_zs);
        else
            hipLaunchKernelGGL((k_wino_bgemm_s3<1, 2, 2, 2, 3, 1, true>), grid, dim3(256), 0, st, A, B, C, Mrows, Ncols, K, a_bytes, b_bytes, tm, tn, a_zs);
        return;
    }
#define S3_GO(MR, WPE, VAR) hipLaunchKernelGGL((k_wino_bgemm_s3<MR, 2, 2, 2, WPE, VAR>), grid, dim3(256), 0, st, A, B, C, Mrows, Ncols, K, a_bytes, b_bytes, tm, tn, a_zs)
    if (var == 0) { if (big_rows) S3_GO(2, 2, 0); else S3_GO(1, 3, 0); }
    else if (var == 2) { if (big_rows) S3_GO(2, 2, 2); else S3_GO(1, 3, 2); }
    else if (var == 3) { if (big_rows) S3_GO(2, 2, 3); else S3_GO(1, 3, 3); }
    else if (big_rows) S3_GO(2, 2, 1);
    else S3_GO(1, 3, 1);
#undef S3_GO
}
static int bgemm_zb(long tiles_mn, int X) {
    static const bool on = [] {
        const char* e = pg_exp_env("PATCHGAN_BGEMM_MZ");
        return e && e[0] == '1';
    }();
    if (!on) return 1;
    int zb = 1;
    for (int d = 2; d <= X; ++d)
        if (X % d == 0 && tiles_mn * (X / d) >= 768) zb = d;
    return zb;
}

int pg_wino2_mo() {
    static const int mo = [] {
        const char* e = pg_exp_env("PATCHGAN_WINO2_TILE");
        return (e && atoi(e) == 4) ? 4 : 3;
    }();
    return mo;
}
static long wino2_tiles(int N, int H, int W) {
    const int mo = pg_wino2_mo();
    return (long)N * ((H + mo - 1) / mo) * ((W + mo - 1) / mo);
}
static long wino2_nxi() { return (long)(pg_wino2_mo() + 1) * (pg_wino2_mo() + 1); }

long pg_wino2_tiles_b2s(int N, int Hs, int Ws) { return wino2_tiles(N, Hs, Ws); }
long pg_wino2_tiles_s2b(int N, int Hb, int Wb) { return wino2_tiles(N, (Hb + 1) / 2 + 1, (Wb + 1) / 2 + 1); }

bool pg_wino2_geom_ok(int N, int Hs, int Ws, int Ca, int Cb) {
    if (Cb % 8 != 0 || Ca % 4 != 0 || Cb < 32 || Ca < 64) return false;
    const long T = wino2_tiles(N, Hs, Ws), X = wino2_nxi();
    if (T < 64) return false;
    if ((double)X * T * 4 * Cb * 4 >= 1.5e9 || (double)X * Ca * 4 * Cb * 4 >= 1.5e9 || (double)X * T * Ca * 4 >= 1.5e9) return false;
    return true;
}

size_t pg_wino2_ws_bytes(int N, int Hs, int Ws, int Ca, int Cb) {
    const long T = wino2_tiles(N, Hs, Ws), X = wino2_nxi();
    return align256((size_t)X * Ca * 4 * Cb * 4) + align256((size_t)X * T * 4 * Cb * 4) + align256((size_t)X * T * Ca * 4);
}

template <int MO>
static int wino2_b2s_run(const float* big, int ld_big, const float* P, const float* bias, float* small, int ld_small, int N,
                         int Hb, int Wb, int Hs, int Ws, int Ca, int Cb, int act, void* ws, hipStream_t st, hipEvent_t ev0,
                         hipEvent_t ev1, const float* Vpre, double* part, float* Vkeep, float* Uext, int u_valid, int s3, long v_stride,
                         long v_tile0) {
// ... 148 lines not shown
    float* M = (float*)((char*)V + align256((size_t)X * T * Ca * 4));
    if (!(Uext && u_valid)) {
        hipLaunchKernelGGL(k_wino2c_u<MO>, dim3((Cb + 15) / 16, (Ca + 15) / 16), dim3(256), 0, st, P, U, Ca, Cb);
        if (hipGetLastError() != hipSuccess) return PG_ELAUNCH;
    }
    hipLaunchKernelGGL(k_wino2c_v<MO>, dim3((unsigned)((T * (Ca / 4) + 255) / 256)), dim3(256), 0, st, small, ld_small, V, N, Hs, Ws,
                       Ca, TH, TW);
    if (hipGetLastError() != hipSuccess) return PG_ELAUNCH;
    if (ev0) (void)hipEventRecord(ev0, st);
    const int a_bytes = (int)((long)X * T * Ca * 4), b_bytes = (int)((long)X * NC * Ca * 4);
    {
        const int big_rows = T >= 1024;
        const int tm = (int)(big_rows ? (T + 127) / 128 : (T + 63) / 64), tn = (NC + 127) / 128;
        const int zb = s3 ? 1 : bgemm_zb((long)tm * tn, X);
        const dim3 grid((unsigned)(tm * tn * (X / zb)));
        if (s3)
            bgemm_s3_launch(big_rows, grid, st, V, U, M, (int)T, NC, Ca, a_bytes, b_bytes, tm, tn, (int)T * Ca);
        else if (big_rows && zb > 1)
            hipLaunchKernelGGL((k_wino_bgemm_mz<2, 2, 2, 2>), grid, dim3(256), 0, st, V, U, M, (int)T, NC, Ca, zb, a_bytes, b_bytes, tm, tn, (int)T * Ca);
        else if (big_rows)
            hipLaunchKernelGGL((k_wino_bgemm<2, 2, 2, 2>), grid, dim3(256), 0, st, V, U, M, (int)T, NC, Ca, a_bytes, b_bytes, tm, tn, (int)T * Ca);
        else if (zb > 1)
            hipLaunchKernelGGL((k_wino_bgemm_mz<1, 2, 2, 2>), grid, dim3(256), 0, st, V, U, M, (int)T, NC, Ca, zb, a_bytes, b_bytes, tm, tn, (int)T * Ca);
        else
            hipLaunchKernelGGL((k_wino_bgemm<1, 2, 2, 2>), grid, dim3(256), 0, st, V, U, M, (int)T, NC, Ca, a_bytes, b_bytes, tm, tn, (int)T * Ca);
    }
    if (ev1) (void)hipEventRecord(ev1, st);
    if (hipGetLastError() != hipSuccess) return PG_ELAUNCH;
    if (part)
        hipLaunchKernelGGL(k_wino2c_out_stats<MO>, dim3((unsigned)pg_wino2_s2b_stats_chunks(N, Hb, Wb, Cb), N), dim3(256), 0, st, M, bias,
                           big, ld_big, N, Hb, Wb, Cb, TH, TW, act, part);
    else
        hipLaunchKernelGGL(k_wino2c_out<MO>, dim3((unsigned)((T * Cb + 255) / 256)), dim3(256), 0, st, M, bias, big, ld_big, N, Hb,
                           Wb, Cb, TH, TW, act, mul);
    return hipGetLastError() == hipSuccess ? PG_OK : PG_ELAUNCH;
}

int pg_wino2_s2b(const float* small, int ld_small, const float* P, const float* bias, float* big, int ld_big, int N, int Hb,
                 int Wb, int Hs, int Ws, int Ca, int Cb, int act, void* ws, hipStream_t st, hipEvent_t ev0, hipEvent_t ev1,
                 double* part, float* Uext, int u_valid, pg_epi_mul mul, int s3) {
    if (part && mul.t) return PG_EINVAL;
    if (pg_wino2_mo() == 4)
        return wino2_s2b_run<4>(small, ld_small, P, bias, big, ld_big, N, Hb, Wb, Hs, Ws, Ca, Cb, act, ws, st, ev0, ev1, part, Uext, u_valid, mul, s3);
    return wino2_s2b_run<3>(small, ld_small, P, bias, big, ld_big, N, Hb, Wb, Hs, Ws, Ca, Cb, act, ws, st, ev0, ev1, part, Uext, u_valid, mul, s3);
}

static long wino2w_tiles(int N, int Hs, int Ws) { return (long)N * ((Hs + 2) / 3) * ((Ws + 2) / 3); }

bool pg_wino2_wgrad_geom_ok(int N, int Hs, int Ws, int Ca, int Cb) {
    if (Ca % 4 != 0 || Cb % 4 != 0 || Ca < 64 || Cb < 32) return false;
    const long T = wino2w_tiles(N, Hs, Ws);
    if (T < 512) return false;
    if (16.0 * T * Ca * 4 >= 1.5e9 || 16.0 * T * 4 * Cb * 4 >= 1.5e9) return false;
    return true;
}

bool pg_wino2_wgrad_tile64(int Ca, int Cb, int s3) {
    static const int forced = [] {
        const char* e = pg_exp_env("PATCHGAN_WINO2W_TILE");
        return e ? atoi(e) : 0;
    }();
    if (forced) return forced == 64;
    if (s3 && Ca % 128 == 0 && (4 * Cb) % 128 == 0) return false;
    return 16L * ((Ca + 127) / 128) * ((4 * Cb + 127) / 128) < 768;
}

int pg_wino2_wgrad_slices(int N, int Hs, int Ws, int Ca, int Cb, int s3) {
    const long T = wino2w_tiles(N, Hs, Ws);
    const int t = pg_wino2_wgrad_tile64(Ca, Cb, s3) ? 64 : 128;
    const long wgs = 16L * ((Ca + t - 1) / t) * ((4 * Cb + t - 1) / t);
    const long fill = wgrad_s3_fill(s3, t);
    long s = (fill + wgs - 1) / wgs;
    const long nchunks = (T + KC - 1) / KC;
    if (s > nchunks / 8) s = nchunks / 8;
    return (int)(s < 1 ? 1 : s);
}

size_t pg_wino2_wgrad_ws_bytes(int N, int Hs, int Ws, int Ca, int Cb) {
    const long T = wino2w_tiles(N, Hs, Ws);
    const int sl = std::max(pg_wino2_wgrad_slices(N, Hs, Ws, Ca, Cb, 0), pg_wino2_wgrad_slices(N, Hs, Ws, Ca, Cb, 1));
    return align256((size_t)16 * T * 4 * Cb * 4) + align256((size_t)16 * T * Ca * 4) + align256((size_t)sl * 16 * Ca * 4 * Cb * 4);
}

int pg_wino2_wgrad(const float* small, int ld_small, const float* big, int ld_big, float* dP, int N, int Hb, int Wb, int Hs,
                   int Ws, int Ca, int Cb, void* ws, hipStream_t st, hipEvent_t ev0, hipEvent_t ev1, const float* Vpre, int s3) {
    const int TH = (Hs + 2) / 3, TW = (Ws + 2) / 3, K = 4 * Cb;
    const long T = (long)N * TH * TW;
    float* Vown = (float*)ws;
    float* DY = Vpre ? Vown : (float*)((char*)ws + align256((size_t)16 * T * K * 4));
    float* S = (float*)((char*)DY + align256((size_t)16 * T * Ca * 4));
    const float* V = Vpre ? Vpre : Vown;
    if (!Vpre) {
        hipLaunchKernelGGL(k_wino2_v<3>, dim3((unsigned)((T * Cb + 255) / 256)), dim3(256), 0, st, big, ld_big, Vown, N, Hb, Wb, Cb, TH,
                           TW, T * K, 0L);
        if (hipGetLastError() != hipSuccess) return PG_ELAUNCH;
    }
    hipLaunchKernelGGL(k_wino2_dy, dim3((unsigned)((T * (Ca / 4) + 255) / 256)), dim3(256), 0, st, small, ld_small, DY, N, Hs, Ws,
                       Ca, TH, TW);
    if (hipGetLastError() != hipSuccess) return PG_ELAUNCH;
    const int slices = pg_wino2_wgrad_slices(N, Hs, Ws, Ca, Cb, s3);
    const int nchunks = (int)((T + KC - 1) / KC);
    const int cps = (nchunks + slices - 1) / slices;
    if (ev0) (void)hipEventRecord(ev0, st);
    if (pg_wino2_wgrad_tile64(Ca, Cb, s3)) {
        const int tilesA = (Ca + 63) / 64, tilesB = (K + 63) / 64;
        if (s3)
            hipLaunchKernelGGL((k_wino_wgrad_gemm_s3<1, 1, 2, 2, 2, 3>), dim3(tilesA * tilesB * 16 * slices), dim3(256), 0, st, DY, V, S, (int)T,
                               Ca, K, cps, tilesA, tilesB, 16, (int)(16L * T * Ca * 4), (int)(16L * T * K * 4));
        else
            hipLaunchKernelGGL((k_wino_wgrad_gemm<1, 1, 2, 2>), dim3(tilesA * tilesB * 16 * slices), dim3(256), 0, st, DY, V, S, (int)T, Ca,
                               K, cps, tilesA, tilesB, 16, (int)(16L * T * Ca * 4), (int)(16L * T * K * 4));
    } else {
        const int tilesA = (Ca + 127) / 128, tilesB = (K + 127) / 128;
        if (s3)
            hipLaunchKernelGGL((k_wino_wgrad_gemm_s3<2, 2, 2, 2, 1, 2>), dim3(tilesA * tilesB * 16 * slices), dim3(256), 0, st, DY, V, S, (int)T,
                               Ca, K, cps, tilesA, tilesB, 16, (int)(16L * T * Ca * 4), (int)(16L * T * K * 4));
        else
            hipLaunchKernelGGL((k_wino_wgrad_gemm<2, 2, 2, 2>), dim3(tilesA * tilesB * 16 * slices), dim3(256), 0, st, DY, V, S, (int)T, Ca,
                               K, cps, tilesA, tilesB, 16, (int)(16L * T * Ca * 4), (int)(16L * T * K * 4));
    }
    if (ev1) (void)hipEventRecord(ev1, st);
    if (hipGetLastError() != hipSuccess) return PG_ELAUNCH;
    hipLaunchKernelGGL(k_wino2_wgrad_out, dim3((unsigned)(((long)Ca * Cb + 255) / 256)), dim3(256), 0, st, S, slices, dP, Ca, Cb);
    return hipGetLastError() == hipSuccess ? PG_OK : PG_ELAUNCH;
}

int pg_wino2_b2s_zb(int N, int Hs, int Ws, int Ca) {
    const long T = wino2_tiles(N, Hs, Ws);
    const long tm = (T >= 1024) ? (T + 127) / 128 : (T + 63) / 64;
    return bgemm_zb(tm * ((Ca + 127) / 128), (int)wino2_nxi());
}
int pg_wino2_s2b_zb(int N, int Hb, int Wb, int Cb) {
    const long T = pg_wino2_tiles_s2b(N, Hb, Wb);
    const long tm = (T >= 1024) ? (T + 127) / 128 : (T + 63) / 64;
    return bgemm_zb(tm * ((4 * Cb + 127) / 128), (int)wino2_nxi());
}

#ifdef PG_TRACE_R
extern "C" int pg_debug_trace_set_w(void* buf) {
    unsigned long long* p = (unsigned long long*)buf;
    return hipMemcpyToSymbol(HIP_SYMBOL(pg_trace_buf_w), &p, sizeof(p)) == hipSuccess ? 0 : -1;
}
#endif
```

### patchgan_amd/engine.py

```python
import ctypes
import os
import functools
import math
import threading

import numpy as np

import torch
from torch import nn

from . import _lib as L

_MASK64 = (1 << 64) - 1
DEFAULT_ALGO = {'direct': L.ALGO_DIRECT, 'mfma': L.ALGO_MFMA, 'bf16': L.ALGO_BF16}.get(__import__('os').environ.get('PATCHGAN_ALGO', ''), L.ALGO_AUTO)


_raw_stream = getattr(torch._C, '_cuda_getCurrentRawStream', None)


def _stream():
    if _raw_stream is not None:
        return _raw_stream(torch.cuda.current_device())
    return torch.cuda.current_stream().cuda_stream

# ... 16 lines not shown
        assert not self.bf and self.C <= 8
        t = torch.empty(self.npix * 8, dtype=torch.bfloat16, device=self.t.device)
        L.check(L.load().pg_pad8_bf16(self.ptr(), self.ld, t.data_ptr(), self.npix, self.C, _stream()), 'pg_pad8_bf16')
        return View(t, 0, 8, self.N, self.H, self.W, self.C, True)

    def channels(self, c0, c):
        assert 0 <= c0 and c0 + c <= self.C
        return View(self.t, self.off + c0, self.ld, self.N, self.H, self.W, c, self.bf)

    def samples(self, n0, n):
        assert 0 <= n0 and n0 + n <= self.N
        return View(self.t, self.off + n0 * self.H * self.W * self.ld, self.ld, n, self.H, self.W, self.C, self.bf)

    def converted(self, bf):
        if self.bf == bf:
            return self
        out = View.alloc(self.N, self.H, self.W, self.C, self.t.device, bf=bf)
        L.check(L.load().pg_act_fwd_t(self.ptr(), self.ld, out.ptr(), out.ld, self.npix, self.C, L.ACT_NONE, 0.0, 0, _stream(),
                                      (1 if self.bf else 0) | (2 if bf else 0)), 'pg_act_fwd_t')
        return out

    @property
    def HW(self):
        return self.H * self.W

    @property
    def extent_bytes(self):
        return self.npix * self.ld * (2 if self.bf else 4)

    @property
    def npix(self):
        return self.N * self.H * self.W

    def to_nchw(self):
        if self.bf:
            return self.converted(False).to_nchw()
        out = torch.empty(self.N, self.C, self.H, self.W, dtype=torch.float32, device=self.t.device)
        L.check(L.load().pg_nhwc_to_nchw(self.ptr(), self.ld, out.data_ptr(), self.N, self.C, self.H, self.W,
                                         _stream()), 'pg_nhwc_to_nchw')
        return out

    def from_nchw(self, src):
        assert tuple(src.shape) == (self.N, self.C, self.H, self.W), (tuple(src.shape), (self.N, self.C, self.H, self.W))
        assert not self.bf, 'API-edge layout kernels write fp32 views'
        src = src.contiguous()
        L.check(L.load().pg_nchw_to_nhwc(src.data_ptr(), self.ptr(), self.ld, self.N, self.C, self.H, self.W,
                                         _stream()), 'pg_nchw_to_nhwc')
        return self

    def from_u8(self, src, div=255.0):
        assert src.dtype == torch.uint8 and tuple(src.shape) == (self.N, self.H, self.W, self.C), tuple(src.shape)
        src = src.contiguous()
        L.check(L.load().pg_u8_to_f32(src.data_ptr(), self.ptr(), self.ld, self.npix, self.C, div, _stream()), 'pg_u8_to_f32')
        return self

    def from_labels(self, src, labels, add=1):
        assert src.dtype == torch.uint8 and tuple(src.shape) == (self.N, self.H, self.W), tuple(src.shape)
        assert len(labels) == self.C, (len(labels), self.C)
        src = src.contiguous()
        arr = (ctypes.c_int * len(labels))(*[int(v) for v in labels])
        L.check(L.load().pg_labels_to_onehot(src.data_ptr(), self.ptr(), self.ld, self.npix, arr, len(labels), add, _stream()),
                'pg_labels_to_onehot')
        return self


def din_fill(x, y, real, fake):
    N, Cx, H, W = x.shape
    Cy = y.shape[1]
    assert tuple(y.shape) == (N, Cy, H, W) and (real.N, real.H, real.W, real.C) == (N, H, W, Cx + Cy) == (fake.N, fake.H, fake.W, fake.C)
    assert real.ld == fake.ld and not real.bf and not fake.bf
    x, y = x.contiguous(), y.contiguous()
    L.check(L.load().pg_din_fill(x.data_ptr(), y.data_ptr(), real.ptr(), fake.ptr(), real.ld, N, Cx, Cy, H, W, _stream()), 'pg_din_fill')




class Exec:

    def __init__(self, device=None):
        self.device = torch.device(device) if device is not None else None
        self.enabled = self.allow = self.inside = self.pending = False
        self.stream = None
        self.keep = []
        self.keep_ptrs = set()
        self.keep_bytes = 0
        self.ws = {}
        self.ws_gen = 0
        self._prev = []

    def side_stream(self):
        if self.stream is None:
            dev = self.device if self.device is not None else torch.device('cuda', torch.cuda.current_device())
            st = _SECOND_STREAMS.get(dev.index)
            if st is None:
                st = _SECOND_STREAMS[dev.index] = torch.cuda.Stream(device=dev)
            self.stream = st
        return self.stream

    def workspace(self, nbytes, device):
        if self.device is not None and device != self.device:
            raise RuntimeError(f'patchgan_amd: engine call on {device} under an execution state bound to {self.device}')
        ws = self.ws.get(self.inside)
        if ws is None or ws.numel() < nbytes:
            ws = self.ws[self.inside] = torch.empty(max(nbytes, 1 << 20), dtype=torch.uint8, device=device)
            self.ws_gen += 1
        return ws

    def buffers(self):
        return list(self.ws.values())

    def release(self):
        if self.stream is not None and (self.keep or self.pending):
            torch.cuda.current_stream(self.device).wait_stream(self.stream)
        self.keep.clear()
        self.keep_ptrs.clear()
        self.keep_bytes = 0
        self.pending = self.allow = self.inside = False
        self.ws.clear()
        self.ws_gen += 1

    def __enter__(self):
        self._prev.append(getattr(_TLS, 'cur', None))
        _TLS.cur = self
        return self

    def __exit__(self, *exc):
        _TLS.cur = self._prev.pop()
        return False


_TLS = threading.local()
_SECOND_STREAMS = {}
_DEFAULT_EXEC = {}


def cur_exec(device=None):
    ex = getattr(_TLS, 'cur', None)
    if ex is not None:
        return ex
    if device is None:
        device = torch.device('cuda', torch.cuda.current_device())
    ex = _DEFAULT_EXEC.get(device.index)
    if ex is None:
        ex = _DEFAULT_EXEC[device.index] = Exec(device)
    return ex


def release_workspaces():
    for ex in _DEFAULT_EXEC.values():
        ex.release()
    _DEFAULT_EXEC.clear()


KEEP_LIMIT_BYTES = 3 << 30


class on_side:
    def __enter__(self):
        ex = self._ex = cur_exec()
        side = ex.side_stream()
        side.wait_stream(torch.cuda.current_stream())
        self._ctx = torch.cuda.stream(side)
        self._ctx.__enter__()
        self._was = ex.inside
        ex.inside = ex.pending = True
        return side

    def __exit__(self, *exc):
        self._ex.inside = self._was
        return self._ctx.__exit__(*exc)


def _side_begin(allow):
    ex = cur_exec()
    ex.allow = (bool(allow) and ex.enabled and not ex.inside and WGRAD_SIDE and PROFILER is None
                and not torch.cuda.is_current_stream_capturing())


def side_join():
    _side_join(True)


def _side_join(explicit=False):
    ex = cur_exec()
    ex.allow = False
    if ex.keep or (explicit and ex.pending):
        torch.cuda.current_stream().wait_stream(ex.stream)
        ex.keep.clear()
        ex.keep_ptrs.clear()
        ex.keep_bytes = 0
        ex.pending = False


def side_producers():
    ex = cur_exec()
    return [ex.stream] if (ex.stream is not None and (ex.keep or ex.pending)) else []


def _workspace(nbytes, device):
    return cur_exec(device).workspace(nbytes, device)


class LaunchProfiler:
    def __init__(self, only=None):
        self.records = []
        self.only = only
        self.limit = None
        self._pool = []

    def reserve(self, n):
        for _ in range(n):
            self._pool.append(self._new_event())

    def _new_event(self):
        e = torch.cuda.Event(enable_timing=True)
        e.record()
        return e

    def launch(self, op, opcode, fn, io=0):
        if op.algo & L.ALGO_MASK == L.ALGO_DIRECT:
            return fn()
        sym, split = op.describe(opcode, io)
        if (self.only is not None and sym != self.only) or (self.limit is not None and len(self.records) >= self.limit):
            return fn()
        e0, e1 = self._event(), self._event()
        L.check(L.load().pg_conv_time_next(e0.cuda_event, e1.cuda_event), 'pg_conv_time_next')
        fn()
        self.records.append((sym, split, op.flops, op.kernel_flops(opcode, io), op.useful_flops(opcode, io), e0, e1))

    def launch2(self, op, opcodes, fn, io=0):
        if op.algo & L.ALGO_MASK == L.ALGO_DIRECT:
            return fn()
        syms = [op.describe(oc, io)[0] for oc in opcodes]
        if (self.only is not None and self.only not in syms) or (self.limit is not None and len(self.records) >= self.limit):
            return fn()
        ev = [self._event() for _ in range(4)]
        L.check(L.load().pg_conv_time_next2(*[e.cuda_event for e in ev]), 'pg_conv_time_next2')
        fn()
        for i, oc in enumerate(opcodes):
            if self.only is None or syms[i] == self.only:
                self.records.append((syms[i], op.describe(oc, io)[1], op.flops, op.kernel_flops(oc, io), op.useful_flops(oc, io), ev[2 * i], ev[2 * i + 1]))

    def _event(self):
        if self._pool:
            return self._pool.pop()
        return self._new_event()

    def summary(self):
        out = {}
        for sym, split, flops, kflops, uflops, e0, e1 in self.records:
            ms = e0.elapsed_time(e1)
            d = out.setdefault(sym, dict(launches=0, ms=0.0, flops=0.0, kflops=0.0, uflops=0.0))
            d['launches'] += 1
            d['ms'] += ms
            d['flops'] += flops
            d['kflops'] += kflops
            d['uflops'] += uflops
        return out


PROFILER = None
_MAX_TENSOR_BYTES = None


class ConvOp:

    def __init__(self, N, Hb, Wb, Ca, Cb, stride, algo=L.ALGO_AUTO):
        Hs = (Hb - 2) // stride + 1
        Ws = (Wb - 2) // stride + 1
        if Hb < 2 or Wb < 2 or Hs < 1 or Ws < 1:
            raise RuntimeError(f"Kernel size can't be greater than actual input size ({Hb}x{Wb}, 4x4 kernel, pad 1)")
        self.g = L.ConvGeom(N, Hb, Wb, Hs, Ws, Ca, Cb, stride)
        self.N, self.Hb, self.Wb, self.Hs, self.Ws, self.Ca, self.Cb, self.stride = N, Hb, Wb, Hs, Ws, Ca, Cb, stride
        self.algo = algo
        lib = L.load()
        self.ws_bytes = max(int(lib.pg_conv_workspace_bytes(ctypes.byref(self.g), op)) for op in (0, 1, 2, 3))
        self._desc = {}

    @property
    def ws_arg(self):
        return max(self.ws_bytes, 1 << 20)

    def _ws(self, device):
        ws = _workspace(self.ws_bytes, device)
        return ws.data_ptr(), self.ws_arg

    @property
    def flops(self):
        return 2.0 * self.N * self.Hs * self.Ws * 16 * self.Ca * self.Cb

    def kernel_flops(self, opcode, io=0):
        return self._describe(opcode, io)[2]

    def useful_flops(self, opcode, io=0):
        ex, us = ctypes.c_double(0), ctypes.c_double(0)
        L.check(L.load().pg_conv_kernel_flops(ctypes.byref(self.g), opcode + 16 * (self.algo | io), self.ws_arg, ctypes.byref(ex),
                                              ctypes.byref(us)), 'pg_conv_kernel_flops')
        return us.value

    def describe(self, opcode, io=0):
        return self._describe(opcode, io)[:2]

    def _describe(self, opcode, io=0):
        key = (opcode, io)
        if key not in self._desc:
            name = ctypes.create_string_buffer(128)
            s, fl = ctypes.c_int(0), ctypes.c_double(0)
            L.check(L.load().pg_conv_kernel(ctypes.byref(self.g), opcode + 16 * (self.algo | io), self.ws_arg, name, 128,
                                            ctypes.byref(s), ctypes.byref(fl)), 'pg_conv_kernel')
            self._desc[key] = (name.value.decode(), s.value, fl.value)
        return self._desc[key]

    @staticmethod
    def _aligned(*views):
        return all(v.ld % 4 == 0 and v.ptr() % 16 == 0 and not v.bf for v in views)

    @staticmethod
    def fits(*views):
        global _MAX_TENSOR_BYTES
        if _MAX_TENSOR_BYTES is None:
            _MAX_TENSOR_BYTES = int(L.load().pg_conv_max_tensor_bytes())
        return all(v.extent_bytes < _MAX_TENSOR_BYTES for v in views)

    @staticmethod
    def _io(big, small):
        return (L.IO_BIG_BF16 if big.bf else 0) | (L.IO_SMALL_BF16 if small.bf else 0)

    def _query(self, key, fn):
        if key not in self._desc:
            self._desc[key] = int(fn())
        return self._desc[key]

    def stats_chunks(self, opcode, view_in, view_out):
        big, small = (view_in, view_out) if opcode == 0 else (view_out, view_in)
        io = self._io(big, small)
        if not self.fits(view_in, view_out):
            return 0
        if io:
            if io != L.IO_MASK or not all(v.ptr() % 16 == 0 and v.ld % 8 == 0 for v in (view_in, view_out)):
                return 0
        elif not self._aligned(view_out) or (not self._aligned(view_in) and not (opcode == 0 and self.Cb <= 3)):
            return 0
        return self._query(('chunks', opcode, io), lambda: L.load().pg_conv_stats_chunks(ctypes.byref(self.g), opcode, self.algo | io,
                                                                                        self.ws_arg))

    def u_bytes(self, opcode, io=0):
        return self._query(('u', opcode, io), lambda: L.load().pg_conv_u_bytes(ctypes.byref(self.g), opcode, self.algo | io,
                                                                               self.ws_arg))

    def v_bytes(self):
        return self._query(('v',), lambda: L.load().pg_conv_v_bytes(ctypes.byref(self.g), self.algo, self.ws_arg))

    def keep_v(self, want, *views):
        vb = self.v_bytes() if (want and KEEP_V and self._aligned(*views) and self.fits(*views)) else 0
        return torch.empty(vb, dtype=torch.uint8, device=views[0].t.device) if vb else None

    def halves_same(self, whole):
        assert whole.g.key()[1:] == self.g.key()[1:] and whole.N == 2 * self.N and whole.algo == self.algo
        return bool(self._query(('halves', whole.ws_arg), lambda: L.load().pg_conv_batch_halves_same(
            ctypes.byref(self.g), self.algo, self.ws_arg, whole.ws_arg)))

    def v_part(self, whole, n0):
        points, k = (16, 4 * self.Cb) if self.stride == 2 else (36, self.Cb)
        stride = whole.v_bytes() // (4 * points)
        return stride, n0 * (stride // k) // whole.N

    @staticmethod
    def _extras(part=None, v_keep=None, v_pre=None, u_cache=None, u_valid=False, mul=None, v_part=(0, 0)):
        if part is None and v_keep is None and v_pre is None and u_cache is None and mul is None:
            return None
        p = lambda t: t.data_ptr() if t is not None else None
        mt, ml, ma = (mul[0].ptr(), mul[0].ld, mul[1]) if mul is not None else (None, 0, 0)
        return L.ConvExtras(p(part), p(v_keep), p(v_pre), p(u_cache), 1 if u_valid else 0, mt, ml, ma, v_part[0], v_part[1])

    def mul_ok(self, small, big, t):
        if t.bf != big.bf or (t.N, t.H, t.W, t.C) != (big.N, big.H, big.W, big.C) or not self.fits(small, big, t):
            return False
        need = (big, t) if self.Ca == 1 else (small, big, t)
        if not all(v.ptr() % 16 == 0 and v.ld % (8 if v.bf else 4) == 0 for v in need):
            return False
        io = self._io(big, small)
        return bool(self._query(('mul', io), lambda: L.load().pg_conv_mul_ok(ctypes.byref(self.g), self.algo | io,
                                                                              self.ws_arg)))

    def big2small(self, big, P, p_off, bias, b_off, small, act=L.ACT_NONE, part=None, v_keep=None, u_cache=None, u_valid=False,
                  v_part=(0, 0)):
        assert (big.N, big.H, big.W, big.C) == (self.N, self.Hb, self.Wb, self.Cb), 'big view mismatch'
        assert (small.N, small.H, small.W, small.C) == (self.N, self.Hs, self.Ws, self.Ca), 'small view mismatch'
        wp, wn = self._ws(P.device)
        args = (big.ptr(), big.ld, L.ptr(P, p_off), L.ptr(bias, b_off) if bias is not None else None, small.ptr(), small.ld,
                ctypes.byref(self.g), act, self.algo | self._io(big, small), wp, wn, _stream())
        x = self._extras(part=part, v_keep=v_keep, u_cache=u_cache, u_valid=u_valid, v_part=v_part if v_keep is not None else (0, 0))

        def go():
            if x is None:
                L.check(L.load().pg_conv4x4_big2small(*args), 'pg_conv4x4_big2small')
            else:
                L.check(L.load().pg_conv4x4_big2small_x(*args, ctypes.byref(x)), 'pg_conv4x4_big2small_x')
        PROFILER.launch(self, 0, go, self._io(big, small)) if PROFILER is not None else go()

    def small2big(self, small, P, p_off, bias, b_off, big, act=L.ACT_NONE, part=None, u_cache=None, u_valid=False, mul=None):
        assert (big.N, big.H, big.W, big.C) == (self.N, self.Hb, self.Wb, self.Cb), 'big view mismatch'
        assert (small.N, small.H, small.W, small.C) == (self.N, self.Hs, self.Ws, self.Ca), 'small view mismatch'
        wp, wn = self._ws(P.device)
        args = (small.ptr(), small.ld, L.ptr(P, p_off), L.ptr(bias, b_off) if bias is not None else None, big.ptr(), big.ld,
                ctypes.byref(self.g), act, self.algo | self._io(big, small), wp, wn, _stream())
        x = self._extras(part=part, u_cache=u_cache, u_valid=u_valid, mul=mul)

        def go():
            if x is None:
                L.check(L.load().pg_conv4x4_small2big(*args), 'pg_conv4x4_small2big')
            else:
                L.check(L.load().pg_conv4x4_small2big_x(*args, ctypes.byref(x)), 'pg_conv4x4_small2big_x')
        PROFILER.launch(self, 1, go, self._io(big, small)) if PROFILER is not None else go()

    def wgrad(self, small, big, dP, p_off, dbias=None, b_off=0, v_pre=None):
        assert (big.N, big.H, big.W, big.C) == (self.N, self.Hb, self.Wb, self.Cb), 'big view mismatch'
        assert (small.N, small.H, small.W, small.C) == (self.N, self.Hs, self.Ws, self.Ca), 'small view mismatch'
        wp, wn = self._ws(dP.device)
        args = (small.ptr(), small.ld, big.ptr(), big.ld, L.ptr(dP, p_off), L.ptr(dbias, b_off) if dbias is not None else None,
                ctypes.byref(self.g), self.algo | self._io(big, small), wp, wn, _stream())
        x = self._extras(v_pre=v_pre)

        def go():
            if x is None:
                L.check(L.load().pg_conv4x4_wgrad(*args), 'pg_conv4x4_wgrad')
            else:
                L.check(L.load().pg_conv4x4_wgrad_x(*args, ctypes.byref(x)), 'pg_conv4x4_wgrad_x')
        ex = cur_exec(dP.device)
        if ex.allow:
            side = ex.side_stream()
            side.wait_stream(torch.cuda.current_stream())
            ex.keep.append((small.t, big.t, v_pre, dP))
            for t in (small.t, big.t, v_pre):
                if t is not None and t.data_ptr() not in ex.keep_ptrs:
                    ex.keep_ptrs.add(t.data_ptr())
                    ex.keep_bytes += t.numel() * t.element_size()
            was, ex.inside = ex.inside, True
            try:
                with torch.cuda.stream(side):
                    wp2, wn2 = self._ws(dP.device)
                    args = args[:8] + (wp2, wn2, _stream())
                    go()
            finally:
                ex.inside = was
            if ex.keep_bytes > KEEP_LIMIT_BYTES:
                torch.cuda.current_stream().wait_stream(side)
                ex.keep.clear()
                ex.keep_ptrs.clear()
                ex.keep_bytes = 0
            return
        PROFILER.launch(self, 2, go, self._io(big, small)) if PROFILER is not None else go()

    def bwd_big(self, small, big, P, dP, p_off, dsmall, u_cache=None, u_valid=False):
        assert (big.N, big.H, big.W, big.C) == (self.N, self.Hb, self.Wb, self.Cb), 'big view mismatch'
        assert (small.N, small.H, small.W, small.C) == (self.N, self.Hs, self.Ws, self.Ca), 'small view mismatch'
        assert (dsmall.N, dsmall.H, dsmall.W, dsmall.C) == (self.N, self.Hs, self.Ws, self.Ca), 'dsmall view mismatch'
        wp, wn = self._ws(P.device)

        def go():
            assert small.bf == big.bf == dsmall.bf, 'bwd_big: one storage type for the three activation tensors'
            args = (small.ptr(), small.ld, big.ptr(), big.ld, L.ptr(P, p_off), L.ptr(dP, p_off), dsmall.ptr(), dsmall.ld,
                    ctypes.byref(self.g), self.algo | self._io(big, small), wp, wn, _stream())
            if u_cache is None:
                L.check(L.load().pg_conv4x4_bwd_big(*args), 'pg_conv4x4_bwd_big')
            else:
                x = self._extras(u_cache=u_cache, u_valid=u_valid)
                L.check(L.load().pg_conv4x4_bwd_big_x(*args, ctypes.byref(x)), 'pg_conv4x4_bwd_big_x')
        PROFILER.launch2(self, (2, 0), go, self._io(big, small)) if PROFILER is not None else go()


def _bf16_tensors_ok(ops, ld_mult=1):
    if _MAX_TENSOR_BYTES is None:
        ConvOp.fits()
    for op in ops:
        if max(op.N * op.Hb * op.Wb * op.Cb, op.N * op.Hs * op.Ws * op.Ca) * ld_mult * 2 >= _MAX_TENSOR_BYTES:
            return False
    return all('bf16' in op.describe(oc, L.IO_MASK)[0] for op in ops for oc in (0, 1, 2))


class UCache(dict):

    def __init__(self, pool=None):
        super().__init__()
        self.log = []
        self.pool = pool if pool is not None else {}

    def buffer(self, key, nb, dev):
        buf = self.pool.get(key)
        if buf is None or buf.numel() != nb or buf.device != dev:
            buf = self.pool[key] = torch.empty(nb, dtype=torch.uint8, device=dev)
        return buf


def _ucache(ucache, li, opcode, op, dev, src, dst, p_off=None):
    if ucache is None or not CACHE_U or not ConvOp.fits(src, dst):
        return None, False
    big, small = (src, dst) if opcode == 0 else (dst, src)
    io = ConvOp._io(big, small)
    if io:
        if not all(v.ptr() % 16 == 0 and v.ld % (8 if v.bf else 4) == 0 for v in (src, dst)):
            return None, False
    elif not ConvOp._aligned(src, dst):
        return None, False
    nb = op.u_bytes(opcode, io)
    if not nb:
        return None, False
    shared = (io == L.IO_MASK and op.Cb > 8 and not (op.algo & L.TUNE_BF16X_RING)
              and not op.describe(0, io)[0].startswith('k_conv_bf16r') and not op.describe(1, io)[0].startswith('k_conv_bf16r'))
    key = (li, 'w', nb) if shared else (li, opcode, nb)
    if key in ucache:
        return ucache[key], True
    if isinstance(ucache, UCache):
        ucache[key] = ucache.buffer(key, nb, dev)
        if p_off is not None:
            ucache.log.append((key, op, opcode, io, p_off, nb))
    else:
        ucache[key] = torch.empty(nb, dtype=torch.uint8, device=dev)
    return ucache[key], False


def prefill_ucache(plan, flat, dev, pool=None):
    uc = UCache(pool)
    if not plan or not PREP_BATCH:
        return uc
    items = (L.ConvPrepItem * len(plan))()
    for it, (key, op, opcode, io, p_off, nb) in zip(items, plan):
        buf = uc[key] = uc.buffer(key, nb, dev)
        it.g, it.op, it.algo, it.ws_bytes = op.g, opcode, op.algo | io, op.ws_arg
        it.P, it.u = L.ptr(flat, p_off), buf.data_ptr()
    uc.log = list(plan)
    L.check(L.load().pg_conv_prep_batch(len(plan), items, _stream()), 'pg_conv_prep_batch')
    return uc


# ... 61 lines not shown
    bstat = L.ptr(bn.scratch, l.bs_off + bn.slot * y.C * 2)
    L.check(lib.pg_batchnorm_coef_from_moments(mom.data_ptr(), count, w, b, BN_EPS, coef.data_ptr(), bstat, y.C, bn.nseg, st),
            'pg_batchnorm_coef_from_moments')
    L.check(lib.pg_batchnorm_act_apply(y.ptr(), y.ld, out.ptr(), out.ld, coef.data_ptr(), y.N, y.HW, y.C, bn.nseg, act, drop_p,
                                       seed & _MASK64, st), 'pg_batchnorm_act_apply')
    return coef


def batchnorm_act_fwd(l, bn, flat, y, out, act, drop_p=0.0, seed=0, part=None, chunks=0):
    lib = L.load()
    coef = torch.empty(bn.nseg * y.C * 4, dtype=torch.float32, device=y.t.device)
    w, b = L.ptr(flat, l.g_off), L.ptr(flat, l.be_off)
    st = _stream()
    if not bn.train:
        L.check(lib.pg_batchnorm_eval_coef(L.ptr(bn.bufs, l.rm_off), L.ptr(bn.bufs, l.rv_off), w, b, y.C, BN_EPS, coef.data_ptr(), st),
                'pg_batchnorm_eval_coef')
        L.check(lib.pg_batchnorm_act_apply(y.ptr(), y.ld, out.ptr(), out.ld, coef.data_ptr(), y.N, y.HW, y.C, 1, act, drop_p,
                                           seed & _MASK64, st), 'pg_batchnorm_act_apply')
        return coef
    _bn_check(y, bn.nseg, bn.world)
    if bn.dist is not None:
        return _bn_sync_fwd(lib, l, bn, flat, y, out, act, drop_p, seed, part, chunks, coef, st)
    bstat = L.ptr(bn.scratch, l.bs_off + bn.slot * y.C * 2)
    if part is not None:
        L.check(lib.pg_batchnorm_stats(None, y.ld, part.data_ptr(), chunks, w, b, coef.data_ptr(), bstat, y.N, y.HW, y.C, bn.nseg,
                                       BN_EPS, None, 0, st), 'pg_batchnorm_stats')
        L.check(lib.pg_batchnorm_act_apply(y.ptr(), y.ld, out.ptr(), out.ld, coef.data_ptr(), y.N, y.HW, y.C, bn.nseg, act, drop_p,
                                           seed & _MASK64, st), 'pg_batchnorm_act_apply')
        return coef
    ws = _workspace(int(lib.pg_batchnorm_workspace_bytes(y.N, y.HW, y.C, bn.nseg)), y.t.device)
    L.check(lib.pg_batchnorm_act_fwd(y.ptr(), y.ld, out.ptr(), out.ld, w, b, coef.data_ptr(), bstat, y.N, y.HW, y.C, bn.nseg, act,
                                     BN_EPS, drop_p, seed & _MASK64, ws.data_ptr(), ws.numel(), st), 'pg_batchnorm_act_fwd')
    return coef


def batchnorm_act_bwd(l, train, nseg, gflat, g1, g2, y, coef, dy, act, drop_p=0.0, seed=0, dist=None):
    lib = L.load()
    nseg = nseg if train else 1
    ws = _workspace(int(lib.pg_batchnorm_workspace_bytes(y.N, y.HW, y.C, nseg)), y.t.device)
    dw, db = (L.ptr(gflat, l.g_off), L.ptr(gflat, l.be_off)) if gflat is not None else (None, None)
    if train and dist is not None:
        st = _stream()
        g2p, g2l = _pl(g2)
        mom = torch.empty(nseg * y.C * 2, dtype=torch.float64, device=y.t.device)
        L.check(lib.pg_batchnorm_moments_bwd(g1.ptr(), g1.ld, g2p, g2l, y.ptr(), y.ld, coef.data_ptr(), mom.data_ptr(), dw, db, y.N, y.HW,
                                             y.C, nseg, act, drop_p, seed & _MASK64, ws.data_ptr(), ws.numel(), st),
                'pg_batchnorm_moments_bwd')
        _bn_allreduce(dist, mom)
        count = float((y.N // nseg) * dist.world * y.HW)
        L.check(lib.pg_batchnorm_bwd_apply(g1.ptr(), g1.ld, g2p, g2l, y.ptr(), y.ld, coef.data_ptr(), mom.data_ptr(), count, dy.ptr(),
                                           dy.ld, y.N, y.HW, y.C, nseg, act, drop_p, seed & _MASK64, ws.data_ptr(), ws.numel(), st),
                'pg_batchnorm_bwd_apply')
        return
    L.check(lib.pg_batchnorm_act_bwd(g1.ptr(), g1.ld, *_pl(g2), y.ptr(), y.ld, coef.data_ptr(), dy.ptr(), dy.ld, dw, db, y.N, y.HW, y.C,
                                     nseg, 1 if train else 0, act, drop_p, seed & _MASK64, ws.data_ptr(), ws.numel(), _stream()),
            'pg_batchnorm_act_bwd')


def bn_update_running(layers, bufs, counters, scratch, nslots):
    bl = [l for l in layers if l.bn]
    if not bl:
        return
    items = (L.BnUpdateItem * len(bl))()
    for it, l in zip(items, bl):
        it.bstat, it.C = L.ptr(scratch, l.bs_off), l.cout
        it.running_mean, it.running_var = L.ptr(bufs, l.rm_off), L.ptr(bufs, l.rv_off)
        it.num_batches_tracked = L.ptr(counters, l.bn_idx)
    L.check(L.load().pg_batchnorm_update_running(len(bl), items, nslots, BN_MOMENTUM, _stream()), 'pg_batchnorm_update_running')


def _exp_env(name, default='1'):
    return os.environ.get(name, default) if 'PATCHGAN_EXPERIMENT' in os.environ else default


FUSE_IN_STATS = _exp_env('PATCHGAN_FUSE_IN_STATS') != '0'
KEEP_V = _exp_env('PATCHGAN_KEEP_V') != '0'
CACHE_U = _exp_env('PATCHGAN_CACHE_U') != '0'
PREP_BATCH = _exp_env('PATCHGAN_PREP_BATCH') != '0'
FUSE_ACT_BWD = _exp_env('PATCHGAN_FUSE_ACT_BWD') != '0'
SEAM8 = _exp_env('PATCHGAN_SEAM8') != '0'
WGRAD_SIDE = _exp_env('PATCHGAN_WGRAD_SIDE') != '0'
BF16_WGRAD_SIDE = _exp_env('PATCHGAN_BF16_WGRAD_SIDE') != '0'
SHARE_DY_V = _exp_env('PATCHGAN_SHARE_DY_V') != '0'
SPLIT_BWD_BIG = _exp_env('PATCHGAN_SPLIT_BWD_BIG') != '0'


def instnorm_act_bwd(g1, g2, y, stats, dy, act, drop_p=0.0, seed=0):
    ws = _workspace(int(L.load().pg_instnorm_workspace_bytes(y.N, y.HW, y.C)), y.t.device)
    L.check(L.load().pg_instnorm_act_bwd_t(g1.ptr(), g1.ld, *_pl(g2), y.ptr(), y.ld, stats.data_ptr(), dy.ptr(), dy.ld,
                                           y.N, y.HW, y.C, act, drop_p, seed & _MASK64, ws.data_ptr(), ws.numel(), _stream(),
                                           _dt(g1, g2, y, dy)), 'pg_instnorm_act_bwd')


def instnorm_affine_act_fwd(y, out, stats, flat, g_off, be_off, act, drop_p=0.0, seed=0, part=None, chunks=0):
    _in_check(y)
    lib = L.load()
    w, b = L.ptr(flat, g_off), L.ptr(flat, be_off)
    if part is not None:
        L.check(lib.pg_instnorm_affine_act_fwd_parts_t(y.ptr(), y.ld, out.ptr(), out.ld, w, b, stats.data_ptr(), part.data_ptr(), chunks,
                                                       y.N, y.HW, y.C, act, 1e-5, drop_p, seed & _MASK64, _stream(), _dt(y, out)),
                'pg_instnorm_affine_act_fwd_parts')
        return
    ws = _workspace(int(lib.pg_instnorm_affine_workspace_bytes(y.N, y.HW, y.C)), y.t.device)
    L.check(lib.pg_instnorm_affine_act_fwd_t(y.ptr(), y.ld, out.ptr(), out.ld, w, b, stats.data_ptr(), y.N, y.HW, y.C, act, 1e-5, drop_p,
                                             seed & _MASK64, ws.data_ptr(), ws.numel(), _stream(), _dt(y, out)),
            'pg_instnorm_affine_act_fwd')


def instnorm_affine_act_bwd(g1, g2, y, stats, dy, flat, gflat, g_off, be_off, act, drop_p=0.0, seed=0):
    lib = L.load()
    ws = _workspace(int(lib.pg_instnorm_affine_workspace_bytes(y.N, y.HW, y.C)), y.t.device)
    dw, db = (L.ptr(gflat, g_off), L.ptr(gflat, be_off)) if gflat is not None else (None, None)
    L.check(lib.pg_instnorm_affine_act_bwd_t(g1.ptr(), g1.ld, *_pl(g2), y.ptr(), y.ld, L.ptr(flat, g_off), L.ptr(flat, be_off),
                                             stats.data_ptr(), dy.ptr(), dy.ld, dw, db, y.N, y.HW, y.C, act, drop_p, seed & _MASK64,
                                             ws.data_ptr(), ws.numel(), _stream(), _dt(g1, g2, y, dy)), 'pg_instnorm_affine_act_bwd')


def act_bwd(g1, g2, a, dy, act):
    L.check(L.load().pg_act_bwd_t(g1.ptr(), g1.ld, *_pl(g2), *_pl(a), dy.ptr(), dy.ld, dy.npix, dy.C, act, 0.0, 0, _stream(),
                                  _dt(g1, g2, a, dy)), 'pg_act_bwd')


def softmax_fwd(y, out):
    L.check(L.load().pg_softmax_fwd(y.ptr(), y.ld, out.ptr(), out.ld, y.npix, y.C, _stream()), 'pg_softmax_fwd')


def softmax_bwd(g1, g2, out, dy):
    L.check(L.load().pg_softmax_bwd(g1.ptr(), g1.ld, *_pl(g2), out.ptr(), out.ld, dy.ptr(), dy.ld, dy.npix, dy.C, _stream()),
            'pg_softmax_bwd')


def adam_scalars(step, lr, beta1=0.9, beta2=0.999, weight_decay=None):
    bc1 = np.float32(1.0 - beta1 ** step)
    sc = np.float32(lr) / bc1, np.float32(math.sqrt(1.0 - beta2 ** step))
    return sc if weight_decay is None else sc + (np.float32(decay_mul(lr, weight_decay)),)


def _is_number(x):
    return not isinstance(x, bool) and isinstance(x, (int, float, np.floating, np.integer))


def _one_or_pair(value, one, msg):
    if value is None:
        return None, None
    if isinstance(value, (tuple, list)):
        if len(value) != 2:
            raise ValueError(msg)
        return tuple(None if x is None else one(x) for x in value)
    x = one(value)
    return x, x


def check_ema_decay(decay):
    if not _is_number(decay):
        raise ValueError(f"ema_decay must be None or a float in [0, 1), not {decay!r}")
    d = float(decay)
    if not (0.0 <= d < 1.0) or not (float(np.float32(d)) < 1.0):
        raise ValueError(f"ema_decay must be None or a float in [0, 1), not {decay!r}")
    return d


def check_clip_norm(value):
    msg = f"clip_grad_norm must be None, a positive float or a pair of them (members may be None), not {value!r}"

    def one(x):
        if not _is_number(x) or not float(x) > 0.0:
# ... 672 lines not shown
                    raise ValueError(f"Expected more than 1 spatial element when training, got input size "
                                     f"torch.Size([{N}, {l.a}, {h}, {w}])")
            sizes = [(op.Hs, op.Ws) for op in enc_ops]
            for i, l in enumerate(self.dec):
                op = ConvOp(N, 2 * h, 2 * w, l.a, l.b, 2, self.algo)
                assert (op.Hs, op.Ws) == (h, w)
                dec_ops.append(op)
                h, w = 2 * h, 2 * w
                if i < 6:
                    sh, sw = sizes[5 - i]
                    if (sh, sw) != (h, w):
                        raise RuntimeError(f"Sizes of tensors must match except in dimension 1. Expected size {h} but got "
                                           f"size {sh} for the skip connection of decoder block {i + 1} (input {H}x{W}: "
                                           "H and W must be multiples of 128)")
            self._ops[key] = (enc_ops, dec_ops)
        return self._ops[key]

    def forward(self, flat, xin, gen_out, train, seed=0, sample0=0, keep_v=False, ucache=None, bn=None):
        assert bn is not None or not self.has_bn, 'a BatchNorm generator pass needs its BNRun'
        N, H, W = xin.N, xin.H, xin.W
        dev = flat.device
        enc_ops, dec_ops = self.ops(N, H, W)
        F = [l.a for l in self.enc]
        c = GenContext()
        c.N, c.H, c.W, c.xin, c.gen_out = N, H, W, xin, gen_out
        norm = c.norm = norm_pass(bn, train=train, seed=seed, sample0=sample0)
        bf = c.bf = bool(self.act_bf) and self._storage_ok((N, H, W), enc_ops[1:] + dec_ops[:6])
        seam8 = c.seam8 = (bf and SEAM8 and self.nf % 64 == 0 and self.input_nc <= 8 and self.output_nc <= 8
                           and enc_ops[0].describe(0, L.IO_MASK)[0].startswith('k_conv_bf16x'))
        c.xin8 = xin.padded8() if seam8 else None
        c.cat = [None] * 7
        for i in range(1, 7):
            op = dec_ops[i]
            c.cat[i] = View.alloc(N, op.Hs, op.Ws, self.dec[i].a, dev, bf=bf)
        c.hidden = View.alloc(N, enc_ops[6].Hs, enc_ops[6].Ws, F[6], dev, bf=bf)
        c.y, c.stats, c.enc_out, c.v = [], [], [], []
        act = L.ACT_CODES[self.activation]
        src = c.xin8 if seam8 else xin
        for i, (l, op) in enumerate(zip(self.enc, enc_ops)):
            y = View.alloc(N, op.Hs, op.Ws, l.a, dev, bf=bf and (i > 0 or seam8))
            if i < 6:
                cat = c.cat[6 - i]
                out = cat.channels(cat.C - l.a, l.a)
            else:
                out = c.hidden
            vk = op.keep_v(keep_v, src, y)
            u, uv = _ucache(ucache, ('e', i), 0, op, dev, src, y, l.p_off)
            c.stats.append(norm.conv_norm_act(op, 0, src, flat, l, (1, i), y, out, act, v_keep=vk, u_cache=u, u_valid=uv))
            c.v.append(vk)
            c.y.append(y)
            c.enc_out.append(out)
            src = out
        c.yd, c.statsd = [None] * 7, [None] * 7
        src = c.hidden
        for i, (l, op) in enumerate(zip(self.dec, dec_ops)):
            if i == 6:
                src = c.cat6_f32 = src if seam8 else src.converted(False)
                if self.final_act == 'softmax':
                    c.gen_raw = View.alloc(N, op.Hb, op.Wb, l.b, dev)
                    op.small2big(src, flat, l.p_off, None, 0, c.gen_raw)
                    softmax_fwd(c.gen_raw, gen_out)
                else:
                    op.small2big(src, flat, l.p_off, None, 0, gen_out, L.ACT_CODES[self.final_act])
                break
            cat = c.cat[i + 1]
            out = cat.channels(0, l.b)
            if l.norm:
                yd = View.alloc(N, op.Hb, op.Wb, l.b, dev, bf=bf)
                u, uv = _ucache(ucache, ('d', i), 1, op, dev, src, yd, l.p_off)
                c.yd[i], c.statsd[i] = yd, norm.conv_norm_act(op, 1, src, flat, l, (2, i), yd, out, act, u_cache=u, u_valid=uv)
            else:
                op.small2big(src, flat, l.p_off, None, 0, out, act)
            src = cat
        return c

    def backward(self, flat, gflat, c, g1, g2=None, need_dx=False, on_ready=None, ucache=None, defer_join=False):
        def done(l):
            if on_ready is not None:
                on_ready(l.p_off, l.be_off + (l.cout + 3) // 4 * 4 if l.norm_params else l.p_off + 16 * l.a * l.b)
        _side_begin(not self.act_bf or BF16_WGRAD_SIDE)
        ok = False
        try:
            r = self._backward(flat, gflat, c, g1, g2, need_dx, done, ucache)
            ok = True
            return r
        finally:
            if not (ok and defer_join):
                _side_join()
            else:
                cur_exec().allow = False

    def _backward(self, flat, gflat, c, g1, g2, need_dx, done, ucache):
        N, dev = c.N, flat.device
        enc_ops, dec_ops = self.ops(c.N, c.H, c.W)
        act = L.ACT_CODES[self.activation]
        l, op = self.dec[6], dec_ops[6]
        dy = View.alloc(N, op.Hb, op.Wb, l.b, dev)
        if self.final_act == 'softmax':
            softmax_bwd(g1, g2, c.gen_out, dy)
        else:
            act_bwd(g1, g2, c.gen_out, dy, L.ACT_CODES[self.final_act])
        bf = c.bf
        if c.seam8:
            dy = dy.padded8()
        dcat = View.alloc(N, op.Hs, op.Ws, l.a, dev, bf=c.seam8)
        op.bwd_big(c.cat6_f32, dy, flat, gflat, l.p_off, dcat)
        done(l)
        dskip = [None] * 7
        for i in range(5, -1, -1):
            l, op = self.dec[i], dec_ops[i]
            g = dcat.channels(0, l.b)
            dskip[5 - i] = dcat.channels(l.b, dcat.C - l.b)
            dy = View.alloc(N, op.Hb, op.Wb, l.b, dev, bf=bf)
            if l.norm:
                c.norm.backward(l, gflat, g, None, c.yd[i], c.statsd[i], dy, act, key=(2, i))
            else:
                act_bwd(g, None, c.cat[i + 1].channels(0, l.b), dy, act)
            src = c.hidden if i == 0 else c.cat[i]
            dsrc = View.alloc(N, op.Hs, op.Ws, l.a, dev, bf=bf)
            u, uv = _ucache(ucache, ('d', i), 0, op, dev, dy, dsrc, l.p_off)
            if (u is not None and bf) or (SPLIT_BWD_BIG and cur_exec().allow):
                vk = op.keep_v(SHARE_DY_V and not bf, dy, dsrc, src)
                if vk is not None:
                    op.big2small(dy, flat, l.p_off, None, 0, dsrc, u_cache=u, u_valid=uv, v_keep=vk)
                    op.wgrad(src, dy, gflat, l.p_off, v_pre=vk)
                else:
                    op.wgrad(src, dy, gflat, l.p_off)
                    op.big2small(dy, flat, l.p_off, None, 0, dsrc, u_cache=u, u_valid=uv)
            else:
                op.bwd_big(src, dy, flat, gflat, l.p_off, dsrc, u_cache=u, u_valid=uv)
            done(l)
            dcat = dsrc
        g_main = dcat
        dx = None
        for j in range(6, -1, -1):
            l, op = self.enc[j], enc_ops[j]
            dy = View.alloc(N, op.Hs, op.Ws, l.a, dev, bf=bf and (j > 0 or c.seam8))
            c.norm.backward(l, gflat, g_main, dskip[j] if j < 6 else None, c.y[j], c.stats[j], dy, act, key=(1, j))
            src = (c.xin8 if c.seam8 else c.xin) if j == 0 else c.enc_out[j - 1]
            op.wgrad(dy, src, gflat, l.p_off, v_pre=c.v[j] if ConvOp._aligned(dy, src) else None)
            done(l)
            if j > 0 or need_dx:
                dsrc = View.alloc(N, op.Hb, op.Wb, l.b, dev, bf=bf and j > 0)
                u, uv = _ucache(ucache, ('e', j), 1, op, dev, dy, dsrc, l.p_off)
                op.small2big(dy, flat, l.p_off, None, 0, dsrc, u_cache=u, u_valid=uv)
                if j == 0:
                    dx = dsrc
                g_main = dsrc
        return dx




DISC_FINAL_ACTS = ('sigmoid', 'none')


def disc_layers(input_nc, ndf, n_layers, norm, norm_kind='instance', spectral=False, final_act='sigmoid'):
    if final_act not in DISC_FINAL_ACTS:
        raise ValueError(f"final_act must be one of {' | '.join(DISC_FINAL_ACTS)}, got {final_act!r}")
    layers = []
    idx = 0
    layers.append(LayerSpec(f'model.{idx}.weight', ndf, input_nc, 2, False, 'leakyrelu', False, bias_key=f'model.{idx}.bias'))
    idx += 2
    mult = 1
    for n in range(1, n_layers):
        prev, mult = mult, min(2 ** n, 8)
        layers.append(LayerSpec(f'model.{idx}.weight', ndf * mult, ndf * prev, 2, False, 'tanh', norm, norm_kind=norm_kind,
                                norm_key=f'model.{idx + 2}'))
        idx += 3 if norm else 2
    prev, mult = mult, min(2 ** n_layers, 8)
    layers.append(LayerSpec(f'model.{idx}.weight', ndf * mult, ndf * prev, 1, False, 'tanh', norm, norm_kind=norm_kind,
                            norm_key=f'model.{idx + 2}'))
    idx += 3 if norm else 2
    layers.append(LayerSpec(f'model.{idx}.weight', 1, ndf * mult, 1, False, final_act, False, bias_key=f'model.{idx}.bias'))
    if spectral:
        for l in layers:
            l.key, l.sn = l.key + '_orig', True
    return layers


class DiscContext:
    def samples(self, n0, n):
        assert not self.bf and not any(s is not None for s in self.stats), 'sample views: fp32 contexts without a norm layer'
        c = DiscContext()
        c.N, c.H, c.W = n, self.H, self.W
        c.norm, c.bf, c.seam8 = self.norm, self.bf, self.seam8
        c.din = self.din.samples(n0, n)
        c.t, c.a, c.src = ([v.samples(n0, n) for v in vs] for vs in (self.t, self.a, self.src))
        c.stats, c.v = list(self.stats), [None] * len(self.v)
        c.out = c.a[-1]
        return c


class DiscriminatorEngine(_WeightPrep):
    _LD_MULT = 1

    def __init__(self, input_nc, ndf, n_layers, norm, algo=None, norm_kind='instance', spectral=False, final_act='sigmoid'):
        self.input_nc, self.ndf, self.n_layers, self.norm = input_nc, ndf, n_layers, norm
        self._init_network(disc_layers(input_nc, ndf, n_layers, norm, layer_kind(norm_kind), spectral, final_act), norm_kind, algo)
        self.final_act = final_act
        self.spectral = bool(spectral)
        self.nsn = assign_spectral(self.layers)
        if self.spectral and len(self.layers) > L.SN_MAX_LAYERS:
            raise NotImplementedError(f"patchgan_amd: spectral_norm takes at most {L.SN_MAX_LAYERS} conv layers (n_layers <= "
                                      f"{L.SN_MAX_LAYERS - 2}), got n_layers = {n_layers}")

    def bf16_storage_ok(self):
        return self.ndf % 4 == 0 and self.ndf >= 32

    def ops(self, N, H, W):
        key = (N, H, W)
        if key not in self._ops:
            ops = []
            h, w = H, W
            for l in self.layers:
                op = ConvOp(N, h, w, l.a, l.b, l.stride, self.algo)
                ops.append(op)
                h, w = op.Hs, op.Ws
            self._ops[key] = ops
        return self._ops[key]

    def out_shape(self, N, H, W):
        op = self.ops(N, H, W)[-1]
        return (N, 1, op.Hs, op.Ws)

    def halves_ok(self, N, H, W):
        key = ('halves', N, H, W)
        if key not in self._ops:
            ok = not self.norm and not self.act_bf and (self.algo & L.ALGO_MASK) in (L.ALGO_AUTO, L.ALGO_MFMA, L.ALGO_DIRECT)
            if ok:
                half, whole = self.ops(N, H, W), self.ops(2 * N, H, W)
                ok = all(h.halves_same(w) and (N * h.Hs * h.Ws * h.Ca * 4) % 16 == 0 for h, w in zip(half, whole))
            self._ops[key] = ok
        return self._ops[key]

    def context(self, flat, din, keep_v=False):
        ops = self.ops(din.N, din.H, din.W)
        dev = flat.device
        c = DiscContext()
        c.din, c.N, c.H, c.W = din, din.N, din.H, din.W
        c.norm, c.bf, c.seam8 = norm_pass(None), False, False
        c.t, c.stats, c.a, c.v, c.src = [], [], [], [], []
        src = din
        for l, op in zip(self.layers, ops):
            c.src.append(src)
            t = View.alloc(din.N, op.Hs, op.Ws, l.a, dev)
            c.v.append(op.keep_v(keep_v, src, t))
            c.t.append(t)
            c.stats.append(None)
            c.a.append(t)
            src = t
        c.out = src
        return c

    def forward_part(self, flat, c, n0, n, ucache=None):
        whole = self.ops(c.N, c.H, c.W)
        dev = flat.device
        for li, (l, op) in enumerate(zip(self.layers, self.ops(n, c.H, c.W))):
            src, t = c.src[li].samples(n0, n), c.t[li].samples(n0, n)
            bias = flat if l.bias_key is not None else None
            u, uv = _ucache(ucache, li, 0, op, dev, src, t, l.p_off)
            vk = c.v[li]
            op.big2small(src, flat, l.p_off, bias, l.b_off, t, L.ACT_CODES[l.act], v_keep=vk, u_cache=u, u_valid=uv,
                         v_part=op.v_part(whole[li], n0) if vk is not None else (0, 0))

    def forward(self, flat, din, ucache=None, keep_v=False, bn=None):
        assert bn is not None or not self.has_bn, 'a BatchNorm discriminator pass needs its BNRun'
        ops = self.ops(din.N, din.H, din.W)
        dev = flat.device
        c = DiscContext()
        c.din, c.N, c.H, c.W = din, din.N, din.H, din.W
        norm = c.norm = norm_pass(bn)
        c.t, c.stats, c.a, c.v, c.src = [], [], [], [], []
        last = len(self.layers) - 1
        bf = c.bf = bool(self.act_bf) and self._storage_ok((din.N, din.H, din.W), ops[1:last])
        seam8 = c.seam8 = (bf and SEAM8 and self.ndf % 64 == 0 and self.input_nc <= 8 and last > 0
                           and ops[0].describe(0, L.IO_MASK)[0].startswith('k_conv_bf16x'))

        src = din.padded8() if seam8 else din
        for li, (l, op) in enumerate(zip(self.layers, ops)):
            if li == last:
                src = src.converted(False)
            c.src.append(src)
            t = View.alloc(din.N, op.Hs, op.Ws, l.a, dev, bf=bf and (0 < li < last or (li == 0 and seam8)))
            bias = flat if l.bias_key is not None else None
            u, uv = _ucache(ucache, li, 0, op, dev, src, t, l.p_off)
            vk = op.keep_v(keep_v, src, t)
            c.v.append(vk)
            op.big2small(src, flat, l.p_off, bias, l.b_off, t, L.ACT_CODES[l.act], v_keep=vk, u_cache=u, u_valid=uv)
            if l.norm:
                a = View.alloc(din.N, op.Hs, op.Ws, l.a, dev, bf=bf and li < last)
                stats = norm.norm_act(l, flat, t, a, L.ACT_NONE)
            else:
                if bf and li == 0 and not seam8:
                    t = t.converted(True)
                a, stats = t, None
            c.t.append(t)
            c.stats.append(stats)
            c.a.append(a)
            src = a
        c.out = src
        return c

    def backward(self, flat, gflat, c, gout, need_wgrad=True, need_dx=False, ucache=None):
        _side_begin(need_wgrad and (not self.act_bf or BF16_WGRAD_SIDE))
        try:
            return self._backward(flat, gflat, c, gout, need_wgrad, need_dx, ucache)
        finally:
            _side_join()

    def _backward(self, flat, gflat, c, gout, need_wgrad, need_dx, ucache):
        ops = self.ops(c.N, c.H, c.W)
        dev = flat.device
        g = gout
        dx = None
        bf, last = c.bf, len(self.layers) - 1
        inner_of = lambda i: bf and (0 < i < last or (i == 0 and c.seam8))
        fused = None
        for li in range(last, -1, -1):
            l, op = self.layers[li], ops[li]
            inner = inner_of(li)
            if fused is not None:
                dy, fused = fused, None
            else:
                if l.norm:
                    dt = View.alloc(c.N, op.Hs, op.Ws, l.a, dev, bf=inner)
                    c.norm.backward(l, gflat if need_wgrad else None, g, None, c.t[li], c.stats[li], dt, L.ACT_NONE)
                    g = dt
                if li == last and not l.norm and L.ACT_CODES[l.act] == L.ACT_NONE:
                    dy = g
                else:
                    dy = View.alloc(c.N, op.Hs, op.Ws, l.a, dev, bf=inner)
                    act_bwd(g, None, c.t[li], dy, L.ACT_CODES[l.act])
            src = c.src[li]
            if need_wgrad:
                op.wgrad(dy, src, gflat, l.p_off, gflat if l.bias_key is not None else None, l.b_off,
                         v_pre=c.v[li] if ConvOp._aligned(dy, src) else None)
            if li > 0 or need_dx:
                below = self.layers[li - 1] if li > 0 else None
                dsrc = None
                if FUSE_ACT_BWD and below is not None and not below.norm:
                    cand = View.alloc(c.N, op.Hb, op.Wb, l.b, dev, bf=inner_of(li - 1))
                    if op.mul_ok(dy, cand, c.t[li - 1]):
                        dsrc = fused = cand
                if dsrc is None:
                    dsrc = View.alloc(c.N, op.Hb, op.Wb, l.b, dev, bf=bf and 0 < li < last)
                u, uv = _ucache(ucache, li, 1, op, dev, dy, dsrc, l.p_off)
                if fused is not None:
                    op.small2big(dy, flat, l.p_off, None, 0, dsrc, u_cache=u, u_valid=uv, mul=(c.t[li - 1], L.ACT_CODES[below.act]))
                else:
                    op.small2big(dy, flat, l.p_off, None, 0, dsrc, u_cache=u, u_valid=uv)
                g = dsrc
                if li == 0:
                    dx = dsrc
        return dx




class LossBuffers:

    def __init__(self, N, C, device, HW=1):
        self.S = torch.empty(int(L.load().pg_loss_reduce_doubles(N, HW, C)), dtype=torch.float64, device=device)
        self.sums = torch.empty(2, dtype=torch.float64, device=device)
        self.coef = torch.empty(N * C * 2, dtype=torch.float32, device=device)


class PendingLoss:
    __slots__ = ('buf', 'wait', 'args', 'nsplit', 'sums')


def _fused_loss_max_nc():
    global _FUSED_LOSS_MAX_NC
    if _FUSED_LOSS_MAX_NC is None:
        _FUSED_LOSS_MAX_NC = int(L.load().pg_loss_fused_max_nc())
    return _FUSED_LOSS_MAX_NC


_FUSED_LOSS_MAX_NC = None


def loss_begin(p, y, tconst, beta=0.75, allreduce=None, need_sums=True):
    lib = L.load()
    buf = LossBuffers(p.N, p.C, p.t.device, p.HW)
    st = _stream()
    h = PendingLoss()
    h.buf, h.args, h.wait, h.sums = buf, (p, y, tconst, beta), None, None
    yp, yl = _pl(y)
    exchange = allreduce is not None and need_sums
    if not exchange and p.N * p.C <= _fused_loss_max_nc():
        h.nsplit = int(lib.pg_loss_reduce_parts(p.ptr(), p.ld, yp, yl, float(tconst), p.N, p.HW, p.C, buf.S.data_ptr(), st))
        if h.nsplit < 1:
            L.check(h.nsplit, 'pg_loss_reduce_parts')
        return h
    h.nsplit = 0
    L.check(lib.pg_loss_reduce(p.ptr(), p.ld, yp, yl, float(tconst), p.N, p.HW, p.C, buf.S.data_ptr(), st), 'pg_loss_reduce')
    if need_sums:
        L.check(lib.pg_loss_prepare(buf.S.data_ptr(), p.N, p.C, beta, buf.sums.data_ptr(), st), 'pg_loss_prepare')
        h.sums = buf.sums
    if exchange:
        h.wait = allreduce(buf.sums)
    return h


def loss_finish(h, mode, alpha, grad_out, loss_out, loss_slot, bglobal, gamma=0.75):
    lib = L.load()
    p, y, tconst, beta = h.args
    buf = h.buf
    if h.wait is not None:
        h.wait()
    st = _stream()
    yp, yl = _pl(y)
    sums = h.sums.data_ptr() if h.sums is not None else None
    if p.N * p.C <= _fused_loss_max_nc():
        gp, gl = _pl(grad_out)
        L.check(lib.pg_loss_value_grad(buf.S.data_ptr(), max(h.nsplit, 1), None, sums, mode, p.N, p.C, p.HW, bglobal, alpha, beta, gamma,
                                       p.ptr(), p.ld, yp, yl, float(tconst), gp, gl, L.ptr(loss_out, loss_slot), st), 'pg_loss_value_grad')
        return buf
    L.check(lib.pg_loss_finalize(buf.S.data_ptr(), sums, mode, p.N, p.C, p.HW, bglobal, alpha, beta, gamma,
                                 buf.coef.data_ptr(), L.ptr(loss_out, loss_slot), st), 'pg_loss_finalize')
# ... 236 lines not shown
```

Before: 2237 images/sec.

## Group small Winograd weight-gradient GEMMs of adjacent layers into one launch

Adds a grouped wgrad entry point that plans several conv weight-gradient problems and runs their Winograd s3 GEMMs in a single kernel. Workgroups are partitioned across members in rounds. On the Python side, a layer's wgrad is held back and fused with the next layer's when the planner judges that the combined workgroup count is small enough to pay off. Held calls are flushed before the backward pass ends or before non-grouped paths run. This targets under-filled GPU launches for the small deep layers, at the cost of extra planning, workspace slicing and a deferred ordering of the done callbacks.

```diff
diff --git a/include/patchgan_hip.h b/include/patchgan_hip.h
--- a/include/patchgan_hip.h
+++ b/include/patchgan_hip.h
@@ -103,6 +103,22 @@
                            const pg_conv_extras* x);
 int pg_conv4x4_wgrad_x(const float* small, int ld_small, const float* big, int ld_big, float* dP, float* dbias,
                        const pg_conv_geom* g, int algo, void* ws, size_t ws_bytes, void* stream, const pg_conv_extras* x);
+#define PG_WGRAD_GROUP_MAX 4
+typedef struct pg_wgrad_problem {
+    const float* small;
+    int ld_small;
+    const float* big;
+    int ld_big;
+    float* dP;
+    float* dbias;
+    pg_conv_geom g;
+    int algo;
+    size_t ws_bytes;
+    const float* v_pre;
+} pg_wgrad_problem;
+size_t pg_conv4x4_wgrad_group_workspace_bytes(int n, const pg_wgrad_problem* problems);
+int pg_conv4x4_wgrad_group_plan(int n, const pg_wgrad_problem* problems, int* workgroups, int* pays);
+int pg_conv4x4_wgrad_group(int n, const pg_wgrad_problem* problems, void* ws, size_t ws_bytes, void* stream);
 typedef struct pg_conv_prep_item {
     pg_conv_geom g;
     int op;
diff --git a/patchgan_amd/_lib.py b/patchgan_amd/_lib.py
--- a/patchgan_amd/_lib.py
+++ b/patchgan_amd/_lib.py
@@ -64,6 +64,15 @@
 class ConvPrepItem(ctypes.Structure):
     _fields_ = [('g', ConvGeom), ('op', ctypes.c_int), ('algo', ctypes.c_int), ('ws_bytes', ctypes.c_size_t), ('P', ctypes.c_void_p),
                 ('u', ctypes.c_void_p)]
+
+
+class WgradProblem(ctypes.Structure):
+    _fields_ = [('small', ctypes.c_void_p), ('ld_small', ctypes.c_int), ('big', ctypes.c_void_p), ('ld_big', ctypes.c_int),
+                ('dP', ctypes.c_void_p), ('dbias', ctypes.c_void_p), ('g', ConvGeom), ('algo', ctypes.c_int),
+                ('ws_bytes', ctypes.c_size_t), ('v_pre', ctypes.c_void_p)]
+
+
+WGRAD_GROUP_MAX = 4
 
 
 class SpectralItem(ctypes.Structure):
@@ -106,6 +115,9 @@
     'pg_conv4x4_small2big_x': (_i, [_p, _i, _p, _p, _p, _i, _G, _i, _i, _p, _sz, _p, _X]),
     'pg_conv4x4_wgrad_x': (_i, [_p, _i, _p, _i, _p, _p, _G, _i, _p, _sz, _p, _X]),
     'pg_conv_prep_batch': (_i, [_i, ctypes.POINTER(ConvPrepItem), _p]),
+    'pg_conv4x4_wgrad_group_workspace_bytes': (_sz, [_i, ctypes.POINTER(WgradProblem)]),
+    'pg_conv4x4_wgrad_group_plan': (_i, [_i, ctypes.POINTER(WgradProblem), ctypes.POINTER(_i), ctypes.POINTER(_i)]),
+    'pg_conv4x4_wgrad_group': (_i, [_i, ctypes.POINTER(WgradProblem), _p, _sz, _p]),
     'pg_instnorm_act_fwd_parts': (_i, [_p, _i, _p, _i, _p, _p, _i, _i, _i, _i, _i, _f, _f, _u64, _p]),
     'pg_instnorm_workspace_bytes': (_sz, [_i, _i, _i]),
     'pg_instnorm_act_fwd': (_i, [_p, _i, _p, _i, _p, _i, _i, _i, _i, _f, _f, _u64, _p, _sz, _p]),
diff --git a/patchgan_amd/csrc/conv_gemm.hip b/patchgan_amd/csrc/conv_gemm.hip
--- a/patchgan_amd/csrc/conv_gemm.hip
+++ b/patchgan_amd/csrc/conv_gemm.hip
@@ -4340,43 +4340,50 @@
     return pg_conv4x4_small2big_x(small, ld_small, P, bias, big, ld_big, gg, act, algo, ws, ws_bytes, stream, nullptr);
 }
 
-static int wgrad_impl(const float* small, int ld_small, const float* big, int ld_big, float* dP, float* dbias,
-                      const pg_conv_geom* gg, int algo, void* ws, size_t ws_bytes, void* stream, const float* v_pre) {
+static int bias_colsum(const Geom& g, int io, const float* small, int ld_small, float* part, float* dbias, hipStream_t st) {
+    const long Kp = (long)g.N * g.Hs * g.Ws;
+    int chunks = (int)std::min<long>(COLSUM_CHUNKS, Kp);
+    long rpc = (Kp + chunks - 1) / chunks;
+    chunks = (int)((Kp + rpc - 1) / rpc);
+    if (io)
+        hipLaunchKernelGGL(k_colsum_partial4<true>, dim3(chunks, (g.Ca + 63) / 64), dim3(256), 0, st, small, ld_small, Kp, g.Ca,
+                           rpc, part);
+    else if ((g.Ca % 4 == 0) && (ld_small % 4 == 0) && aligned16(small) && aligned16(part))
+        hipLaunchKernelGGL(k_colsum_partial4<false>, dim3(chunks, (g.Ca + 63) / 64), dim3(256), 0, st, small, ld_small, Kp, g.Ca,
+                           rpc, part);
+    else
+        hipLaunchKernelGGL(k_colsum_partial, dim3(chunks, (g.Ca + 63) / 64), dim3(256), 0, st, small, ld_small, Kp, g.Ca,
+                           rpc, part);
+    if (hipGetLastError() != hipSuccess) return PG_ELAUNCH;
+    return launch_reduce(part, g.Ca, chunks, dbias, g.Ca, 1, g.Ca, nullptr, 0, st);
+}
+
+static int wgrad_plan(const float* small, int ld_small, const float* big, int ld_big, float* dP, float* dbias, const pg_conv_geom* gg,
+                      int algo, void* ws, size_t ws_bytes, void* stream, const pg_conv_extras* x, Call* c) {
     if (!geom_ok(gg) || !big || !dP || !small || ld_big < gg->Cb || ld_small < gg->Ca) return PG_EINVAL;
-    if (v_pre && !aligned16(v_pre)) return PG_EINVAL;
-    hipStream_t st = (hipStream_t)stream;
+    if (x->v_pre && !aligned16(x->v_pre)) return PG_EINVAL;
     const Geom g = to_geom(gg);
     const int io = algo & PG_IO_MASK;
     if (io && ((algo & PG_ALGO_MASK) != PG_ALGO_BF16 || io != PG_IO_MASK)) return PG_EINVAL;
     if (io && dbias && !((g.Ca % 4 == 0) && (ld_small % 4 == 0) && aligned_io(small, true))) return PG_EINVAL;
     if (!ws) ws_bytes = 0;
+    if (!hand_overs_sized(gg, 2, algo, ws, ws_bytes, *x)) return PG_EINVAL;
+    if (dbias && ws_bytes < colsum_bytes(g.Ca)) return PG_EWORKSPACE;
+    *c = Call{ConvPlan{}, Views{small, big, ld_small, ld_big, dP, dbias, PG_ACT_NONE, ws, x}, g, algo & PG_ALGO_MASK, io, tune_of(algo), ws_bytes,
+              (hipStream_t)stream};
+    c->p = plan_conv(gg, 2, algo, c->tune, ws_bytes, &c->v);
+    return c->p.rc != PG_OK ? refusal(c->p.rc, 2, c->v, gg, algo, ws_bytes) : PG_OK;
+}
+
+static int wgrad_impl(const float* small, int ld_small, const float* big, int ld_big, float* dP, float* dbias,
+                      const pg_conv_geom* gg, int algo, void* ws, size_t ws_bytes, void* stream, const float* v_pre) {
     pg_conv_extras x = NO_EXTRAS;
     x.v_pre = v_pre;
-    if (!hand_overs_sized(gg, 2, algo, ws, ws_bytes, x)) return PG_EINVAL;
-    if (dbias) {
-        if (ws_bytes < colsum_bytes(g.Ca)) return PG_EWORKSPACE;
-        const Views vw{small, big, ld_small, ld_big, dP, dbias, PG_ACT_NONE, ws, &x};
-        const int prc = plan_conv(gg, 2, algo, tune_of(algo), ws_bytes, &vw).rc;
-        if (prc != PG_OK) return refusal(prc, 2, vw, gg, algo, ws_bytes);
-        const long Kp = (long)g.N * g.Hs * g.Ws;
-        float* part = (float*)ws;
-        int chunks = (int)std::min<long>(COLSUM_CHUNKS, Kp);
-        long rpc = (Kp + chunks - 1) / chunks;
-        chunks = (int)((Kp + rpc - 1) / rpc);
-        if (io)
-            hipLaunchKernelGGL(k_colsum_partial4<true>, dim3(chunks, (g.Ca + 63) / 64), dim3(256), 0, st, small, ld_small, Kp, g.Ca,
-                               rpc, part);
-        else if ((g.Ca % 4 == 0) && (ld_small % 4 == 0) && aligned16(small) && aligned16(part))
-            hipLaunchKernelGGL(k_colsum_partial4<false>, dim3(chunks, (g.Ca + 63) / 64), dim3(256), 0, st, small, ld_small, Kp, g.Ca,
-                               rpc, part);
-        else
-            hipLaunchKernelGGL(k_colsum_partial, dim3(chunks, (g.Ca + 63) / 64), dim3(256), 0, st, small, ld_small, Kp, g.Ca,
-                               rpc, part);
-        if (hipGetLastError() != hipSuccess) return PG_ELAUNCH;
-        int rc = launch_reduce(part, g.Ca, chunks, dbias, g.Ca, 1, g.Ca, nullptr, 0, st);
-        if (rc != PG_OK) return rc;
-    }
-    return run_conv(2, Views{small, big, ld_small, ld_big, dP, dbias, PG_ACT_NONE, ws, &x}, gg, algo, ws_bytes, stream);
+    Call c;
+    int rc = wgrad_plan(small, ld_small, big, ld_big, dP, dbias, gg, algo, ws, ws_bytes, stream, &x, &c);
+    if (rc != PG_OK) return rc;
+    if (dbias && (rc = bias_colsum(c.g, c.io, small, ld_small, (float*)ws, dbias, c.st)) != PG_OK) return rc;
+    return launch_wgrad(c);
 }
 
 int pg_conv4x4_wgrad(const float* small, int ld_small, const float* big, int ld_big, float* dP, float* dbias,
@@ -4388,6 +4395,97 @@
                        const pg_conv_geom* gg, int algo, void* ws, size_t ws_bytes, void* stream, const pg_conv_extras* x) {
     if (x && (x->part || x->v_keep || x->u_cache || x->v_stride || x->v_tile0)) return PG_EINVAL;
     return wgrad_impl(small, ld_small, big, ld_big, dP, dbias, gg, algo, ws, ws_bytes, stream, x ? x->v_pre : nullptr);
+}
+
+static size_t group_slice(const pg_wgrad_problem& p) { return ((p.ws_bytes ? p.ws_bytes : pg_conv_workspace_bytes(&p.g, 2)) + 255) & ~(size_t)255; }
+static long group_wgs(const ConvPlan& p, const Geom& g, const Tune& t) {
+    if (p.rc != PG_OK || (p.path != Path::WinoWgrad && p.path != Path::Wino2Wgrad)) return 0;
+    return pg_wino_wgrad_group_wgs(p.path == Path::Wino2Wgrad, g.N, g.Hs, g.Ws, g.Ca, g.Cb, t.s3w);
+}
+static bool group_pays(int n, int fused, const long* wgs) {
+    static const long cap = pg_exp_env("PATCHGAN_WGRAD_GROUP_WGS") ? atol(pg_exp_env("PATCHGAN_WGRAD_GROUP_WGS")) : 256;
+    if (fused != n || n < 2) return false;
+    long sum = 0, least = wgs[0];
+    for (int i = 0; i < n; ++i) sum += wgs[i], least = std::min(least, wgs[i]);
+    return least <= 128 && sum <= cap;
+}
+
+size_t pg_conv4x4_wgrad_group_workspace_bytes(int n, const pg_wgrad_problem* pr) {
+    if (n < 1 || n > PG_WGRAD_GROUP_MAX || !pr) return 0;
+    size_t sum = 0;
+    for (int i = 0; i < n; ++i) {
+        if (!geom_ok(&pr[i].g)) return 0;
+        sum += group_slice(pr[i]);
+    }
+    return sum;
+}
+
+int pg_conv4x4_wgrad_group_plan(int n, const pg_wgrad_problem* pr, int* workgroups, int* pays) {
+    if (workgroups) *workgroups = 0;
+    if (pays) *pays = 0;
+    if (n < 1 || n > PG_WGRAD_GROUP_MAX || !pr) return 0;
+    long wgs[PG_WGRAD_GROUP_MAX], sum = 0;
+    int fused = 0;
+    for (int i = 0; i < n; ++i) {
+        ConvPlan p;
+        const size_t wb = group_slice(pr[i]);
+        if (!query_plan(&pr[i].g, 2, pr[i].algo, pr[i].ws_bytes ? pr[i].ws_bytes : wb, pr[i].v_pre ? OFFER_V : 0, &p)) return 0;
+        wgs[i] = group_wgs(p, to_geom(&pr[i].g), tune_of(pr[i].algo));
+        if (wgs[i]) ++fused, sum += wgs[i];
+    }
+    if (fused < 2) return 0;
+    if (workgroups) *workgroups = (int)sum;
+    if (pays) *pays = group_pays(n, fused, wgs) ? 1 : 0;
+    return fused;
+}
+
+int pg_conv4x4_wgrad_group(int n, const pg_wgrad_problem* pr, void* ws, size_t ws_bytes, void* stream) {
+    if (n < 1 || n > PG_WGRAD_GROUP_MAX || !pr) return PG_EINVAL;
+    t_ev0 = t_ev1 = t_ev2 = t_ev3 = nullptr;
+    if (!ws) ws_bytes = 0;
+    Call c[PG_WGRAD_GROUP_MAX];
+    pg_conv_extras x[PG_WGRAD_GROUP_MAX];
+    long wgs[PG_WGRAD_GROUP_MAX];
+    size_t off = 0;
+    int fused = 0;
+    for (int i = 0; i < n; ++i) {
+        const pg_wgrad_problem& p = pr[i];
+        if (!geom_ok(&p.g)) return PG_EINVAL;
+        const size_t mine = group_slice(p);
+        if (off + mine > ws_bytes) return PG_EWORKSPACE;
+        x[i] = NO_EXTRAS;
+        x[i].v_pre = p.v_pre;
+        const int rc = wgrad_plan(p.small, p.ld_small, p.big, p.ld_big, p.dP, p.dbias, &p.g, p.algo, (char*)ws + off, p.ws_bytes ? p.ws_bytes : mine, stream, &x[i],
+                                  &c[i]);
+        if (rc != PG_OK) return rc;
+        wgs[i] = group_wgs(c[i].p, c[i].g, c[i].tune);
+        if (wgs[i]) ++fused;
+        off += mine;
+    }
+    hipStream_t st = (hipStream_t)stream;
+    pg_wino_wgrad_item items[PG_WGRAD_GROUP_MAX];
+    int m = 0;
+    for (int i = 0; i < n; ++i) {
+        const Call& k = c[i];
+        if (fused < 2 || !wgs[i]) {
+            int rc = PG_OK;
+            if (k.v.bias && (rc = bias_colsum(k.g, k.io, (const float*)k.v.small, k.v.ld_small, (float*)k.v.ws, const_cast<float*>(k.v.bias), st)) != PG_OK) return rc;
+            if ((rc = launch_wgrad(k)) != PG_OK) return rc;
+            continue;
+        }
+        items[m++] = pg_wino_wgrad_item{k.p.path == Path::Wino2Wgrad, (const float*)k.v.small, k.v.ld_small, (const float*)k.v.big, k.v.ld_big,
+                                        const_cast<float*>(k.v.P), k.g.N, k.g.Hb, k.g.Wb, k.g.Hs, k.g.Ws, k.g.Ca, k.g.Cb, (char*)k.v.ws + k.p.reserved,
+                                        x[i].v_pre, k.tune.s3w};
+    }
+    if (!m) return PG_OK;
+    int rc = pg_wino_wgrad_group(m, items, st);
+    if (rc != PG_OK) return rc;
+    for (int i = 0; i < n; ++i) {
+        const Call& k = c[i];
+        if (wgs[i] && k.v.bias && (rc = bias_colsum(k.g, k.io, (const float*)k.v.small, k.v.ld_small, (float*)k.v.ws, const_cast<float*>(k.v.bias), st)) != PG_OK)
+            return rc;
+    }
+    return PG_OK;
 }
 
 int pg_conv4x4_bwd_big(const float* small, int ld_small, const float* big, int ld_big, const float* P, float* dP,
diff --git a/patchgan_amd/csrc/conv_wino.h b/patchgan_amd/csrc/conv_wino.h
--- a/patchgan_amd/csrc/conv_wino.h
+++ b/patchgan_amd/csrc/conv_wino.h
@@ -68,3 +68,19 @@
 size_t pg_wino2_wgrad_ws_bytes(int N, int Hs, int Ws, int Ca, int Cb);
 int pg_wino2_wgrad(const float* small, int ld_small, const float* big, int ld_big, float* dP, int N, int Hb, int Wb, int Hs,
                    int Ws, int Ca, int Cb, void* ws, hipStream_t st, hipEvent_t ev0, hipEvent_t ev1, const float* Vpre, int s3 = 0);
+
+#define PG_WINO_WGRAD_GROUP_MAX 4
+struct pg_wino_wgrad_item {
+    int polyphase;
+    const float* small;
+    int ld_small;
+    const float* big;
+    int ld_big;
+    float* dP;
+    int N, Hb, Wb, Hs, Ws, Ca, Cb;
+    void* ws;
+    const float* Vpre;
+    int s3;
+};
+int pg_wino_wgrad_group(int n, const pg_wino_wgrad_item* items, hipStream_t st);
+long pg_wino_wgrad_group_wgs(int polyphase, int N, int Hs, int Ws, int Ca, int Cb, int s3);
diff --git a/patchgan_amd/csrc/conv_wino.hip b/patchgan_amd/csrc/conv_wino.hip
--- a/patchgan_amd/csrc/conv_wino.hip
+++ b/patchgan_amd/csrc/conv_wino.hip
@@ -1210,17 +1210,16 @@
         }
 }
 
-template <int MR, int NR, int WM, int WN, int KS, int WPE>
-__global__ __launch_bounds__(256) __attribute__((amdgpu_waves_per_eu(WPE, WPE))) void k_wino_wgrad_gemm_s3(const float* __restrict__ DY, const float* __restrict__ V,
-                                                         float* __restrict__ S, int T, int Ca, int Cb, int chunks_per_slice,
-                                                         int tilesA, int tilesB, int NX, int dy_bytes, int v_bytes) {
+template <int MR, int NR, int WM, int WN, int KS>
+__device__ __forceinline__ void wino_wgrad_s3_body(const float* __restrict__ DY, const float* __restrict__ V, float* __restrict__ S, int T,
+                                                   int Ca, int Cb, int chunks_per_slice, int tilesA, int tilesB, int NX, int dy_bytes,
+                                                   int v_bytes, int bid, int nblk, __bf16* smem) {
     constexpr int BM = WM * MR * 32, BN = WN * NR * 32, KCH = 16 * KS, ROW = KS * 48 + 8, BUF = (BM + BN) * ROW;
     static_assert((BM + BN) * KS == 256, "one 4 x 4 block per staging thread");
-    __shared__ __attribute__((aligned(16))) __bf16 smem[2 * BUF];
     const int tid = threadIdx.x, lane = tid & 63, wave = tid >> 6;
     const int wm = wave / WN, wn = wave % WN;
     const int lrow = lane & 31, lh = lane >> 5;
-    int w = pg_xcd_remap(blockIdx.x, gridDim.x);
+    int w = pg_xcd_remap(bid, nblk);
     const int tile_b = w % tilesB;
     w /= tilesB;
     const int tile_a = w % tilesA;
@@ -1320,6 +1319,62 @@
                 if (a < Ca && col < Cb) o[(long)a * Cb + col] = acc[i][j][r];
             }
         }
+}
+
+template <int MR, int NR, int WM, int WN, int KS, int WPE>
+__global__ __launch_bounds__(256) __attribute__((amdgpu_waves_per_eu(WPE, WPE))) void k_wino_wgrad_gemm_s3(const float* __restrict__ DY, const float* __restrict__ V,
+                                                         float* __restrict__ S, int T, int Ca, int Cb, int chunks_per_slice,
+                                                         int tilesA, int tilesB, int NX, int dy_bytes, int v_bytes) {
+    __shared__ __attribute__((aligned(16))) __bf16 smem[2 * (WM * MR * 32 + WN * NR * 32) * (KS * 48 + 8)];
+    wino_wgrad_s3_body<MR, NR, WM, WN, KS>(DY, V, S, T, Ca, Cb, chunks_per_slice, tilesA, tilesB, NX, dy_bytes, v_bytes, blockIdx.x, gridDim.x, smem);
+}
+
+struct WinoWgradMember {
+    const float *DY, *V;
+    float* S;
+    int T, Ca, Cb, chunks_per_slice, tilesA, tilesB, NX, dy_bytes, v_bytes, wgs;
+};
+struct WinoWgradGroup {
+    int n;
+    WinoWgradMember m[PG_WINO_WGRAD_GROUP_MAX];
+};
+template <int MR, int NR, int WM, int WN, int KS, int WPE>
+__global__ __launch_bounds__(256) __attribute__((amdgpu_waves_per_eu(WPE, WPE))) void k_wino_wgrad_gemm_s3_group(const WinoWgradGroup g) {
+    __shared__ __attribute__((aligned(16))) __bf16 smem[2 * (WM * MR * 32 + WN * NR * 32) * (KS * 48 + 8)];
+    int units[PG_WINO_WGRAD_GROUP_MAX];
+#pragma unroll
+    for (int i = 0; i < PG_WINO_WGRAD_GROUP_MAX; ++i) units[i] = i < g.n ? (g.m[i].wgs + 7) >> 3 : 0;
+    int rem = blockIdx.x >> 3, lo = 0, mi = -1, round = 0;
+    for (int phase = 0; phase < PG_WINO_WGRAD_GROUP_MAX && mi < 0; ++phase) {
+        int active = 0, next = 0x7fffffff;
+#pragma unroll
+        for (int i = 0; i < PG_WINO_WGRAD_GROUP_MAX; ++i)
+            if (units[i] > lo) {
+                ++active;
+                next = min(next, units[i]);
+            }
+        if (active == 0) return;
+        const int span = (next - lo) * active;
+        if (rem < span) {
+            round = lo + rem / active;
+            int k = rem % active;
+#pragma unroll
+            for (int i = 0; i < PG_WINO_WGRAD_GROUP_MAX; ++i)
+                if (units[i] > lo && mi < 0) {
+                    if (k == 0) mi = i;
+                    --k;
+                }
+        } else {
+            rem -= span;
+            lo = next;
+        }
+    }
+    if (mi < 0) return;
+    const WinoWgradMember& t = g.m[mi];
+    const int local = round * 8 + (blockIdx.x & 7);
+    if (local >= t.wgs) return;
+    wino_wgrad_s3_body<MR, NR, WM, WN, KS>(t.DY, t.V, t.S, t.T, t.Ca, t.Cb, t.chunks_per_slice, t.tilesA, t.tilesB, t.NX, t.dy_bytes, t.v_bytes,
+                                           local, t.wgs, smem);
 }
 
 template <int WPE>
@@ -2150,8 +2205,49 @@
     return align256((size_t)36 * wgrad_tiles(N, Hs, Ws) * Cb * 4);
 }
 
-int pg_wino_wgrad(const float* small, int ld_small, const float* big, int ld_big, float* dP, int N, int Hb, int Wb, int Hs,
-                  int Ws, int Ca, int Cb, void* ws, hipStream_t st, hipEvent_t ev0, hipEvent_t ev1, const float* Vpre, int s3) {
+struct WgradGemm {
+    const float *DY, *V;
+    float* S;
+    long T;
+    int Ca, K, X, slices, cps, tilesA, tilesB, R;
+    bool tile64, s3;
+    int wgs() const { return tilesA * tilesB * X * slices; }
+    bool groupable() const { return s3 && !tile64; }
+};
+
+static int wgrad_gemm(const WgradGemm& j, hipStream_t st) {
+    const dim3 grid(j.wgs());
+    const int T = (int)j.T, dyb = (int)((long)j.X * j.T * j.Ca * 4), vb = (int)((long)j.X * j.T * j.K * 4);
+    if (j.tile64) {
+        if (j.s3)
+            hipLaunchKernelGGL((k_wino_wgrad_gemm_s3<1, 1, 2, 2, 2, 3>), grid, dim3(256), 0, st, j.DY, j.V, j.S, T, j.Ca, j.K, j.cps, j.tilesA, j.tilesB,
+                               j.X, dyb, vb);
+        else
+            hipLaunchKernelGGL((k_wino_wgrad_gemm<1, 1, 2, 2>), grid, dim3(256), 0, st, j.DY, j.V, j.S, T, j.Ca, j.K, j.cps, j.tilesA, j.tilesB, j.X, dyb,
+                               vb);
+    } else {
+        if (j.s3)
+            hipLaunchKernelGGL((k_wino_wgrad_gemm_s3<2, 2, 2, 2, 1, 2>), grid, dim3(256), 0, st, j.DY, j.V, j.S, T, j.Ca, j.K, j.cps, j.tilesA, j.tilesB,
+                               j.X, dyb, vb);
+        else
+            hipLaunchKernelGGL((k_wino_wgrad_gemm<2, 2, 2, 2>), grid, dim3(256), 0, st, j.DY, j.V, j.S, T, j.Ca, j.K, j.cps, j.tilesA, j.tilesB, j.X, dyb,
+                               vb);
+    }
+    return hipGetLastError() == hipSuccess ? PG_OK : PG_ELAUNCH;
+}
+
+static void wgrad_split(WgradGemm& j, int slices, bool tile64, int s3) {
+    const int nchunks = (int)((j.T + KC - 1) / KC), tt = tile64 ? 64 : 128;
+    j.slices = slices;
+    j.cps = (nchunks + slices - 1) / slices;
+    j.tile64 = tile64;
+    j.s3 = s3 != 0;
+    j.tilesA = (j.Ca + tt - 1) / tt;
+    j.tilesB = (j.K + tt - 1) / tt;
+}
+
+static int wino_wgrad_prep(const float* small, int ld_small, const float* big, int ld_big, int N, int Hb, int Wb, int Hs, int Ws, int Ca,
+                           int Cb, void* ws, hipStream_t st, const float* Vpre, int s3, WgradGemm* j) {
     const int R = pg_wino_wgrad_r(N, Hs, Ws), X = (R + 3) * (R + 3);
     const int TH = (Hs + R - 1) / R, TW = (Ws + R - 1) / R;
     const long T = (long)N * TH * TW;
@@ -2170,35 +2266,32 @@
         hipLaunchKernelGGL(k_wino_dy<2>, gd, dim3(256), 0, st, small, ld_small, DY, N, Hs, Ws, Ca, TH, TW);
     }
     if (hipGetLastError() != hipSuccess) return PG_ELAUNCH;
-    const int slices = pg_wino_wgrad_slices(N, Hs, Ws, Ca, Cb, s3);
-    const int nchunks = (int)((T + KC - 1) / KC);
-    const int cps = (nchunks + slices - 1) / slices;
+    *j = WgradGemm{DY, V, S, T, Ca, Cb, X, 0, 0, 0, 0, R, false, false};
+    wgrad_split(*j, pg_wino_wgrad_slices(N, Hs, Ws, Ca, Cb, s3), pg_wino_wgrad_tile64(Ca, Cb, s3), s3);
+    return PG_OK;
+}
+
+static int wgrad_finish(const WgradGemm& j, float* dP, int Cb, hipStream_t st) {
+    const dim3 go((unsigned)(((long)j.Ca * Cb + 255) / 256));
+    if (j.R == 3)
+        hipLaunchKernelGGL(k_wino_wgrad_out<3>, go, dim3(256), 0, st, j.S, j.slices, dP, j.Ca, Cb);
+    else if (j.R == 2)
+        hipLaunchKernelGGL(k_wino_wgrad_out<2>, go, dim3(256), 0, st, j.S, j.slices, dP, j.Ca, Cb);
+    else
+        hipLaunchKernelGGL(k_wino2_wgrad_out, go, dim3(256), 0, st, j.S, j.slices, dP, j.Ca, Cb);
+    return hipGetLastError() == hipSuccess ? PG_OK : PG_ELAUNCH;
+}
+
+int pg_wino_wgrad(const float* small, int ld_small, const float* big, int ld_big, float* dP, int N, int Hb, int Wb, int Hs,
+                  int Ws, int Ca, int Cb, void* ws, hipStream_t st, hipEvent_t ev0, hipEvent_t ev1, const float* Vpre, int s3) {
+    WgradGemm j;
+    int rc = wino_wgrad_prep(small, ld_small, big, ld_big, N, Hb, Wb, Hs, Ws, Ca, Cb, ws, st, Vpre, s3, &j);
+    if (rc != PG_OK) return rc;
     if (ev0) (void)hipEventRecord(ev0, st);
-    if (pg_wino_wgrad_tile64(Ca, Cb, s3)) {
-        const int tilesA = (Ca + 63) / 64, tilesB = (Cb + 63) / 64;
-        if (s3)
-            hipLaunchKernelGGL((k_wino_wgrad_gemm_s3<1, 1, 2, 2, 2, 3>), dim3(tilesA * tilesB * X * slices), dim3(256), 0, st, DY, V, S, (int)T,
-                               Ca, Cb, cps, tilesA, tilesB, X, (int)((long)X * T * Ca * 4), (int)((long)X * T * Cb * 4));
-        else
-            hipLaunchKernelGGL((k_wino_wgrad_gemm<1, 1, 2, 2>), dim3(tilesA * tilesB * X * slices), dim3(256), 0, st, DY, V, S, (int)T, Ca,
-                               Cb, cps, tilesA, tilesB, X, (int)((long)X * T * Ca * 4), (int)((long)X * T * Cb * 4));
-    } else {
-        const int tilesA = (Ca + 127) / 128, tilesB = (Cb + 127) / 128;
-        if (s3)
-            hipLaunchKernelGGL((k_wino_wgrad_gemm_s3<2, 2, 2, 2, 1, 2>), dim3(tilesA * tilesB * X * slices), dim3(256), 0, st, DY, V, S, (int)T,
-                               Ca, Cb, cps, tilesA, tilesB, X, (int)((long)X * T * Ca * 4), (int)((long)X * T * Cb * 4));
-        else
-            hipLaunchKernelGGL((k_wino_wgrad_gemm<2, 2, 2, 2>), dim3(tilesA * tilesB * X * slices), dim3(256), 0, st, DY, V, S, (int)T, Ca,
-                               Cb, cps, tilesA, tilesB, X, (int)((long)X * T * Ca * 4), (int)((long)X * T * Cb * 4));
-    }
+    rc = wgrad_gemm(j, st);
     if (ev1) (void)hipEventRecord(ev1, st);
-    if (hipGetLastError() != hipSuccess) return PG_ELAUNCH;
-    const dim3 go((unsigned)(((long)Ca * Cb + 255) / 256));
-    if (R == 3)
-        hipLaunchKernelGGL(k_wino_wgrad_out<3>, go, dim3(256), 0, st, S, slices, dP, Ca, Cb);
-    else
-        hipLaunchKernelGGL(k_wino_wgrad_out<2>, go, dim3(256), 0, st, S, slices, dP, Ca, Cb);
-    return hipGetLastError() == hipSuccess ? PG_OK : PG_ELAUNCH;
+    if (rc != PG_OK) return rc;
+    return wgrad_finish(j, dP, Cb, st);
 }
 
 static void bgemm_s3_launch(int big_rows, dim3 grid, hipStream_t st, const float* A, const float* B, float* C, int Mrows, int Ncols, int K,
@@ -2513,8 +2606,8 @@
     return align256((size_t)16 * T * 4 * Cb * 4) + align256((size_t)16 * T * Ca * 4) + align256((size_t)sl * 16 * Ca * 4 * Cb * 4);
 }
 
-int pg_wino2_wgrad(const float* small, int ld_small, const float* big, int ld_big, float* dP, int N, int Hb, int Wb, int Hs,
-                   int Ws, int Ca, int Cb, void* ws, hipStream_t st, hipEvent_t ev0, hipEvent_t ev1, const float* Vpre, int s3) {
+static int wino2_wgrad_prep(const float* small, int ld_small, const float* big, int ld_big, int N, int Hb, int Wb, int Hs, int Ws, int Ca,
+                            int Cb, void* ws, hipStream_t st, const float* Vpre, int s3, WgradGemm* j) {
     const int TH = (Hs + 2) / 3, TW = (Ws + 2) / 3, K = 4 * Cb;
     const long T = (long)N * TH * TW;
     float* Vown = (float*)ws;
@@ -2529,31 +2622,61 @@
     hipLaunchKernelGGL(k_wino2_dy, dim3((unsigned)((T * (Ca / 4) + 255) / 256)), dim3(256), 0, st, small, ld_small, DY, N, Hs, Ws,
                        Ca, TH, TW);
     if (hipGetLastError() != hipSuccess) return PG_ELAUNCH;
-    const int slices = pg_wino2_wgrad_slices(N, Hs, Ws, Ca, Cb, s3);
-    const int nchunks = (int)((T + KC - 1) / KC);
-    const int cps = (nchunks + slices - 1) / slices;
+    *j = WgradGemm{DY, V, S, T, Ca, K, 16, 0, 0, 0, 0, 0, false, false};
+    wgrad_split(*j, pg_wino2_wgrad_slices(N, Hs, Ws, Ca, Cb, s3), pg_wino2_wgrad_tile64(Ca, Cb, s3), s3);
+    return PG_OK;
+}
+
+int pg_wino2_wgrad(const float* small, int ld_small, const float* big, int ld_big, float* dP, int N, int Hb, int Wb, int Hs,
+                   int Ws, int Ca, int Cb, void* ws, hipStream_t st, hipEvent_t ev0, hipEvent_t ev1, const float* Vpre, int s3) {
+    WgradGemm j;
+    int rc = wino2_wgrad_prep(small, ld_small, big, ld_big, N, Hb, Wb, Hs, Ws, Ca, Cb, ws, st, Vpre, s3, &j);
+    if (rc != PG_OK) return rc;
     if (ev0) (void)hipEventRecord(ev0, st);
-    if (pg_wino2_wgrad_tile64(Ca, Cb, s3)) {
-        const int tilesA = (Ca + 63) / 64, tilesB = (K + 63) / 64;
-        if (s3)
-            hipLaunchKernelGGL((k_wino_wgrad_gemm_s3<1, 1, 2, 2, 2, 3>), dim3(tilesA * tilesB * 16 * slices), dim3(256), 0, st, DY, V, S, (int)T,
-                               Ca, K, cps, tilesA, tilesB, 16, (int)(16L * T * Ca * 4), (int)(16L * T * K * 4));
-        else
-            hipLaunchKernelGGL((k_wino_wgrad_gemm<1, 1, 2, 2>), dim3(tilesA * tilesB * 16 * slices), dim3(256), 0, st, DY, V, S, (int)T, Ca,
-                               K, cps, tilesA, tilesB, 16, (int)(16L * T * Ca * 4), (int)(16L * T * K * 4));
-    } else {
-        const int tilesA = (Ca + 127) / 128, tilesB = (K + 127) / 128;
-        if (s3)
-            hipLaunchKernelGGL((k_wino_wgrad_gemm_s3<2, 2, 2, 2, 1, 2>), dim3(tilesA * tilesB * 16 * slices), dim3(256), 0, st, DY, V, S, (int)T,
-                               Ca, K, cps, tilesA, tilesB, 16, (int)(16L * T * Ca * 4), (int)(16L * T * K * 4));
-        else
-            hipLaunchKernelGGL((k_wino_wgrad_gemm<2, 2, 2, 2>), dim3(tilesA * tilesB * 16 * slices), dim3(256), 0, st, DY, V, S, (int)T, Ca,
-                               K, cps, tilesA, tilesB, 16, (int)(16L * T * Ca * 4), (int)(16L * T * K * 4));
-    }
+    rc = wgrad_gemm(j, st);
     if (ev1) (void)hipEventRecord(ev1, st);
-    if (hipGetLastError() != hipSuccess) return PG_ELAUNCH;
-    hipLaunchKernelGGL(k_wino2_wgrad_out, dim3((unsigned)(((long)Ca * Cb + 255) / 256)), dim3(256), 0, st, S, slices, dP, Ca, Cb);
-    return hipGetLastError() == hipSuccess ? PG_OK : PG_ELAUNCH;
+    if (rc != PG_OK) return rc;
+    return wgrad_finish(j, dP, Cb, st);
+}
+
+int pg_wino_wgrad_group(int n, const pg_wino_wgrad_item* it, hipStream_t st) {
+    if (n < 1 || n > PG_WINO_WGRAD_GROUP_MAX || !it) return PG_EINVAL;
+    WgradGemm j[PG_WINO_WGRAD_GROUP_MAX];
+    for (int i = 0; i < n; ++i) {
+        const pg_wino_wgrad_item& t = it[i];
+        const int rc = (t.polyphase ? wino2_wgrad_prep : wino_wgrad_prep)(t.small, t.ld_small, t.big, t.ld_big, t.N, t.Hb, t.Wb, t.Hs, t.Ws, t.Ca, t.Cb,
+                                                                           t.ws, st, t.Vpre, t.s3, &j[i]);
+        if (rc != PG_OK) return rc;
+    }
+    WinoWgradGroup g{};
+    long units = 0;
+    for (int i = 0; i < n; ++i)
+        if (j[i].groupable()) {
+            g.m[g.n++] = WinoWgradMember{j[i].DY, j[i].V, j[i].S, (int)j[i].T, j[i].Ca, j[i].K, j[i].cps, j[i].tilesA, j[i].tilesB, j[i].X,
+                                         (int)((long)j[i].X * j[i].T * j[i].Ca * 4), (int)((long)j[i].X * j[i].T * j[i].K * 4), j[i].wgs()};
+            units += (j[i].wgs() + 7) / 8;
+        }
+    const bool grouped = g.n >= 2;
+    if (grouped) {
+        hipLaunchKernelGGL((k_wino_wgrad_gemm_s3_group<2, 2, 2, 2, 1, 2>), dim3((unsigned)(8 * units)), dim3(256), 0, st, g);
+        if (hipGetLastError() != hipSuccess) return PG_ELAUNCH;
+    }
+    for (int i = 0; i < n; ++i)
+        if (!(grouped && j[i].groupable())) {
+            const int rc = wgrad_gemm(j[i], st);
+            if (rc != PG_OK) return rc;
+        }
+    for (int i = 0; i < n; ++i) {
+        const int rc = wgrad_finish(j[i], it[i].dP, it[i].Cb, st);
+        if (rc != PG_OK) return rc;
+    }
+    return PG_OK;
+}
+
+long pg_wino_wgrad_group_wgs(int polyphase, int N, int Hs, int Ws, int Ca, int Cb, int s3) {
+    if (!s3 || (polyphase ? pg_wino2_wgrad_tile64(Ca, Cb, s3) : pg_wino_wgrad_tile64(Ca, Cb, s3))) return 0;
+    const long X = polyphase ? 16 : wgrad_nxi(N, Hs, Ws), K = polyphase ? 4L * Cb : Cb;
+    return X * ((Ca + 127) / 128) * ((K + 127) / 128) * (polyphase ? pg_wino2_wgrad_slices(N, Hs, Ws, Ca, Cb, s3) : pg_wino_wgrad_slices(N, Hs, Ws, Ca, Cb, s3));
 }
 
 int pg_wino2_b2s_zb(int N, int Hs, int Ws, int Ca) {
diff --git a/patchgan_amd/engine.py b/patchgan_amd/engine.py
--- a/patchgan_amd/engine.py
+++ b/patchgan_amd/engine.py
@@ -122,6 +122,7 @@
         self.enabled = self.allow = self.inside = self.pending = False
         self.stream = None
         self.keep = []
+        self.held = []
         self.keep_ptrs = set()
         self.keep_bytes = 0
         self.ws = {}
@@ -153,6 +154,7 @@
         if self.stream is not None and (self.keep or self.pending):
             torch.cuda.current_stream(self.device).wait_stream(self.stream)
         self.keep.clear()
+        self.held = []
         self.keep_ptrs.clear()
         self.keep_bytes = 0
         self.pending = self.allow = self.inside = False
@@ -303,6 +305,57 @@
 _MAX_TENSOR_BYTES = None
 
 
+def _to_side(ex, operands, go):
+    if not ex.allow:
+        return False
+    side = ex.side_stream()
+    side.wait_stream(torch.cuda.current_stream())
+    for held in operands:
+        ex.keep.append(held)
+        for t in held[:3]:
+            if t is not None and t.data_ptr() not in ex.keep_ptrs:
+                ex.keep_ptrs.add(t.data_ptr())
+                ex.keep_bytes += t.numel() * t.element_size()
+    was, ex.inside = ex.inside, True
+    try:
+        with torch.cuda.stream(side):
+            go()
+    finally:
+        ex.inside = was
+    if ex.keep_bytes > KEEP_LIMIT_BYTES:
+        torch.cuda.current_stream().wait_stream(side)
+        ex.keep.clear()
+        ex.keep_ptrs.clear()
+        ex.keep_bytes = 0
+    return True
+
+
+def _wgrad(op, nxt, small, big, dP, p_off, dbias=None, b_off=0, v_pre=None, done=None):
+    ex = cur_exec(dP.device)
+    call = (op, small, big, dP, p_off, dbias, b_off, v_pre)
+    if ex.held:
+        held, ex.held = ex.held, []
+        ConvOp.wgrad_group([h[0] for h in held] + [call])
+        for h in held:
+            h[1]()
+    elif (WGRAD_GROUP and PROFILER is None and nxt is not None and not small.bf and not big.bf
+          and op.groups_with(v_pre is not None, *nxt)):
+        ex.held = [(call, done if done is not None else (lambda: None))]
+        return
+    else:
+        op.wgrad(small, big, dP, p_off, dbias, b_off, v_pre=v_pre)
+    if done is not None:
+        done()
+
+
+def _wgrad_flush(launch=True):
+    ex = cur_exec()
+    held, ex.held = ex.held, []
+    for (op, small, big, dP, p_off, dbias, b_off, v_pre), done in (held if launch else []):
+        op.wgrad(small, big, dP, p_off, dbias, b_off, v_pre=v_pre)
+        done()
+
+
 class ConvOp:
 
     def __init__(self, N, Hb, Wb, Ca, Cb, stride, algo=L.ALGO_AUTO):
@@ -457,40 +510,46 @@
     def wgrad(self, small, big, dP, p_off, dbias=None, b_off=0, v_pre=None):
         assert (big.N, big.H, big.W, big.C) == (self.N, self.Hb, self.Wb, self.Cb), 'big view mismatch'
         assert (small.N, small.H, small.W, small.C) == (self.N, self.Hs, self.Ws, self.Ca), 'small view mismatch'
-        wp, wn = self._ws(dP.device)
-        args = (small.ptr(), small.ld, big.ptr(), big.ld, L.ptr(dP, p_off), L.ptr(dbias, b_off) if dbias is not None else None,
-                ctypes.byref(self.g), self.algo | self._io(big, small), wp, wn, _stream())
         x = self._extras(v_pre=v_pre)
 
         def go():
+            wp, wn = self._ws(dP.device)
+            args = (small.ptr(), small.ld, big.ptr(), big.ld, L.ptr(dP, p_off), L.ptr(dbias, b_off) if dbias is not None else None,
+                    ctypes.byref(self.g), self.algo | self._io(big, small), wp, wn, _stream())
             if x is None:
                 L.check(L.load().pg_conv4x4_wgrad(*args), 'pg_conv4x4_wgrad')
             else:
                 L.check(L.load().pg_conv4x4_wgrad_x(*args, ctypes.byref(x)), 'pg_conv4x4_wgrad_x')
-        ex = cur_exec(dP.device)
-        if ex.allow:
-            side = ex.side_stream()
-            side.wait_stream(torch.cuda.current_stream())
-            ex.keep.append((small.t, big.t, v_pre, dP))
-            for t in (small.t, big.t, v_pre):
-                if t is not None and t.data_ptr() not in ex.keep_ptrs:
-                    ex.keep_ptrs.add(t.data_ptr())
-                    ex.keep_bytes += t.numel() * t.element_size()
-            was, ex.inside = ex.inside, True
-            try:
-                with torch.cuda.stream(side):
-                    wp2, wn2 = self._ws(dP.device)
-                    args = args[:8] + (wp2, wn2, _stream())
-                    go()
-            finally:
-                ex.inside = was
-            if ex.keep_bytes > KEEP_LIMIT_BYTES:
-                torch.cuda.current_stream().wait_stream(side)
-                ex.keep.clear()
-                ex.keep_ptrs.clear()
-                ex.keep_bytes = 0
+        if _to_side(cur_exec(dP.device), [(small.t, big.t, v_pre, dP)], go):
             return
         PROFILER.launch(self, 2, go, self._io(big, small)) if PROFILER is not None else go()
+
+    def groups_with(self, has_v, other, other_has_v):
+        def ask():
+            pr = (L.WgradProblem * 2)(*[L.WgradProblem(None, 0, None, 0, None, None, o.g, o.algo, o.ws_arg, 16 if v else None)
+                                        for o, v in ((self, has_v), (other, other_has_v))])
+            pays = ctypes.c_int(0)
+            L.load().pg_conv4x4_wgrad_group_plan(2, pr, None, ctypes.byref(pays))
+            return pays.value
+        return bool(self._query(('group', has_v, other.g.key(), other.algo, other.ws_arg, other_has_v), ask))
+
+    @staticmethod
+    def wgrad_group(calls):
+        dev = calls[0][3].device
+        pr = (L.WgradProblem * len(calls))()
+        total = 0
+        for k, (op, small, big, dP, p_off, dbias, b_off, v_pre) in enumerate(calls):
+            assert (big.N, big.H, big.W, big.C) == (op.N, op.Hb, op.Wb, op.Cb), 'big view mismatch'
+            assert (small.N, small.H, small.W, small.C) == (op.N, op.Hs, op.Ws, op.Ca), 'small view mismatch'
+            pr[k] = L.WgradProblem(small.ptr(), small.ld, big.ptr(), big.ld, L.ptr(dP, p_off), L.ptr(dbias, b_off) if dbias is not None else None,
+                                   op.g, op.algo | op._io(big, small), op.ws_arg, v_pre.data_ptr() if v_pre is not None else None)
+            total += (op.ws_arg + 255) & ~255
+
+        def go():
+            ws = _workspace(total, dev)
+            L.check(L.load().pg_conv4x4_wgrad_group(len(calls), pr, ws.data_ptr(), total, _stream()), 'pg_conv4x4_wgrad_group')
+        if not _to_side(cur_exec(dev), [(small.t, big.t, v_pre, dP) for _, small, big, dP, _, _, _, v_pre in calls], go):
+            go()
 
     def bwd_big(self, small, big, P, dP, p_off, dsmall, u_cache=None, u_valid=False):
         assert (big.N, big.H, big.W, big.C) == (self.N, self.Hb, self.Wb, self.Cb), 'big view mismatch'
@@ -718,6 +777,7 @@
 WGRAD_SIDE = _exp_env('PATCHGAN_WGRAD_SIDE') != '0'
 BF16_WGRAD_SIDE = _exp_env('PATCHGAN_BF16_WGRAD_SIDE') != '0'
 SHARE_DY_V = _exp_env('PATCHGAN_SHARE_DY_V') != '0'
+WGRAD_GROUP = _exp_env('PATCHGAN_WGRAD_GROUP') != '0'
 SPLIT_BWD_BIG = _exp_env('PATCHGAN_SPLIT_BWD_BIG') != '0'
 
 
@@ -1556,9 +1616,11 @@
         ok = False
         try:
             r = self._backward(flat, gflat, c, g1, g2, need_dx, done, ucache)
+            _wgrad_flush()
             ok = True
             return r
         finally:
+            _wgrad_flush(False)
             if not (ok and defer_join):
                 _side_join()
             else:
@@ -1595,15 +1657,18 @@
             u, uv = _ucache(ucache, ('d', i), 0, op, dev, dy, dsrc, l.p_off)
             if (u is not None and bf) or (SPLIT_BWD_BIG and cur_exec().allow):
                 vk = op.keep_v(SHARE_DY_V and not bf, dy, dsrc, src)
+                nxt = (dec_ops[i - 1], SHARE_DY_V and KEEP_V and not bf and dec_ops[i - 1].v_bytes() > 0) if (i > 0 and not bf) else None
+                fin = functools.partial(done, l)
                 if vk is not None:
                     op.big2small(dy, flat, l.p_off, None, 0, dsrc, u_cache=u, u_valid=uv, v_keep=vk)
-                    op.wgrad(src, dy, gflat, l.p_off, v_pre=vk)
+                    _wgrad(op, nxt, src, dy, gflat, l.p_off, v_pre=vk, done=fin)
                 else:
-                    op.wgrad(src, dy, gflat, l.p_off)
+                    _wgrad(op, nxt, src, dy, gflat, l.p_off, done=fin)
                     op.big2small(dy, flat, l.p_off, None, 0, dsrc, u_cache=u, u_valid=uv)
             else:
+                _wgrad_flush()
                 op.bwd_big(src, dy, flat, gflat, l.p_off, dsrc, u_cache=u, u_valid=uv)
-            done(l)
+                done(l)
             dcat = dsrc
         g_main = dcat
         dx = None
@@ -1612,8 +1677,8 @@
             dy = View.alloc(N, op.Hs, op.Ws, l.a, dev, bf=bf and (j > 0 or c.seam8))
             c.norm.backward(l, gflat, g_main, dskip[j] if j < 6 else None, c.y[j], c.stats[j], dy, act, key=(1, j))
             src = (c.xin8 if c.seam8 else c.xin) if j == 0 else c.enc_out[j - 1]
-            op.wgrad(dy, src, gflat, l.p_off, v_pre=c.v[j] if ConvOp._aligned(dy, src) else None)
-            done(l)
+            _wgrad(op, (enc_ops[j - 1], c.v[j - 1] is not None) if j > 0 else None, dy, src, gflat, l.p_off,
+                   v_pre=c.v[j] if ConvOp._aligned(dy, src) else None, done=functools.partial(done, l))
             if j > 0 or need_dx:
                 dsrc = View.alloc(N, op.Hb, op.Wb, l.b, dev, bf=bf and j > 0)
                 u, uv = _ucache(ucache, ('e', j), 1, op, dev, dy, dsrc, l.p_off)
@@ -1779,8 +1844,11 @@
     def backward(self, flat, gflat, c, gout, need_wgrad=True, need_dx=False, ucache=None):
         _side_begin(need_wgrad and (not self.act_bf or BF16_WGRAD_SIDE))
         try:
-            return self._backward(flat, gflat, c, gout, need_wgrad, need_dx, ucache)
+            r = self._backward(flat, gflat, c, gout, need_wgrad, need_dx, ucache)
+            _wgrad_flush()
+            return r
         finally:
+            _wgrad_flush(False)
             _side_join()
 
     def _backward(self, flat, gflat, c, gout, need_wgrad, need_dx, ucache):
@@ -1808,8 +1876,8 @@
                     act_bwd(g, None, c.t[li], dy, L.ACT_CODES[l.act])
             src = c.src[li]
             if need_wgrad:
-                op.wgrad(dy, src, gflat, l.p_off, gflat if l.bias_key is not None else None, l.b_off,
-                         v_pre=c.v[li] if ConvOp._aligned(dy, src) else None)
+                _wgrad(op, (ops[li - 1], c.v[li - 1] is not None) if li > 0 else None, dy, src, gflat, l.p_off,
+                       gflat if l.bias_key is not None else None, l.b_off, v_pre=c.v[li] if ConvOp._aligned(dy, src) else None)
             if li > 0 or need_dx:
                 below = self.layers[li - 1] if li > 0 else None
                 dsrc = None
```

Measured after the change: 2209 images/sec. 0.987x the previous value.
